# ZJU-DAILY/HC-SpMM

Measured on AMD Instinct MI355X. Metric: GNN-aggregation SpMM edges*dim/s (A*X, fp32), higher is better.
Workload: dtype f32

## Files before the change

### hc-spmm_amd/csrc/capi.hip

```cpp
#include <hip/hip_runtime.h>
#include <stdint.h>
#include <stdlib.h>

#include "fingerprint.h"
#include "hcspmm.h"
#include "spmm_kernels.h"

namespace {
thread_local int g_last_hip_error = 0;

int fail_hip(hipError_t e) {
  g_last_hip_error = (int)e;
  return HCSPMM_EHIP;
}

inline bool aligned(const void* p, size_t a) { return (reinterpret_cast<uintptr_t>(p) & (a - 1)) == 0; }

constexpr int kDtypeF8 = HCSPMM_DTYPE_BF16 + 1;

inline int elem_bytes(int dtype) { return dtype == HCSPMM_DTYPE_F32 ? 4 : dtype == kDtypeF8 ? 1 : 2; }

int pick_vec(int dtype, int D, int64_t ldx, int64_t ldz, const void* X, const void* Z, const void* ws) {
  if (dtype == HCSPMM_DTYPE_F32) return D >= 4 ? 4 : D >= 2 ? 2 : 1;
  const bool dword_rows = ((D | ldx | ldz) & 1) == 0 && aligned(X, 4) && aligned(Z, 4) && (!ws || aligned(ws, 4));
// ... 69 lines not shown
  }
  int n_wide = 0;
  return wide_choice(h, D, dtype, &n_wide);
}

extern "C" int32_t hcspmm_wide_threshold_fp8(const hcspmm_plan_header* h, int D) {
  if (D <= 0 || D % 4 != 0) return INT32_MAX;
  if (!h) return (D + nominal_vec(kDtypeF8, D) - 1) / nominal_vec(kDtypeF8, D) > 32 ? INT32_MAX : 64;
  int n_wide = 0;
  return wide_choice(h, D, kDtypeF8, &n_wide);
}

extern "C" int32_t hcspmm_wide_threshold(const hcspmm_plan_header* h, int D) {
  return hcspmm_wide_threshold_typed(h, D, HCSPMM_DTYPE_F32);
}

extern "C" int32_t hcspmm_own_tiny_launch(const hcspmm_plan_header* h, int fused) {
  return h && hcspmm::plan_own_tiny_launch(h->n_tiny, fused) ? 1 : 0;
}

extern "C" int hcspmm_abi_version(void) { return HCSPMM_ABI_VERSION; }

namespace {
__global__ __launch_bounds__(256) void fingerprint_kernel(const int32_t* __restrict__ rowptr, const int32_t* __restrict__ col,
                                                          long long N, long long E, unsigned long long* out) {
  const long long stride = (long long)gridDim.x * blockDim.x;
  const long long i0 = (long long)blockIdx.x * blockDim.x + threadIdx.x;
  unsigned long long acc = (i0 == 0) ? hcspmm::fp_seed(N, E) : 0ull;
  for (long long r = i0; r <= N; r += stride) acc += hcspmm::fp_term_rowptr((uint64_t)r, rowptr[r]);
  for (long long e = i0; e < E; e += stride) acc += hcspmm::fp_term_col((uint64_t)e, col[e]);
  for (int off = 32; off > 0; off >>= 1) acc += __shfl_xor(acc, off, 64);
  if ((threadIdx.x & 63) == 0) atomicAdd(out, acc);
}
}

namespace {
__global__ __launch_bounds__(256) void edge_to_row_kernel(const int32_t* __restrict__ rowptr, int N, long long E,
                                                          int32_t* __restrict__ e2r) {
  const long long stride = (long long)gridDim.x * blockDim.x;
  for (long long e = (long long)blockIdx.x * blockDim.x + threadIdx.x; e < E; e += stride) {
    int lo = 0, hi = N;
    while (hi - lo > 1) {
      const int mid = lo + ((hi - lo) >> 1);
      if ((long long)rowptr[mid] <= e) lo = mid;
      else hi = mid;
    }
    e2r[e] = lo;
  }
}
}

extern "C" int hcspmm_edge_to_row_device(const int32_t* rowptr, int64_t N, int64_t E, int32_t* e2r, void* stream_v) {
  if (N < 0 || E < 0 || !rowptr || (E > 0 && !e2r)) return HCSPMM_EINVAL;
  if (N > INT32_MAX - 16 || E > INT32_MAX) return HCSPMM_ERANGE;
  if (E == 0) return HCSPMM_OK;
  long long blocks = (E + 255) / 256;
  if (blocks > 65536) blocks = 65536;
  hipLaunchKernelGGL(edge_to_row_kernel, dim3((unsigned)blocks), dim3(256), 0, reinterpret_cast<hipStream_t>(stream_v), rowptr,
                     (int)N, (long long)E, e2r);
  const hipError_t e = hipGetLastError();
  return e == hipSuccess ? HCSPMM_OK : fail_hip(e);
}

extern "C" int hcspmm_graph_fingerprint_device(const int32_t* rowptr, const int32_t* col, int64_t N, int64_t E,
                                               uint64_t* out_d, void* stream_v) {
  if (!rowptr || !out_d || N < 0 || E < 0 || (E > 0 && !col)) return HCSPMM_EINVAL;
  if (N > INT32_MAX - 16 || E > INT32_MAX) return HCSPMM_ERANGE;
  hipStream_t stream = reinterpret_cast<hipStream_t>(stream_v);
  hipError_t e = hipMemsetAsync(out_d, 0, sizeof(uint64_t), stream);
  if (e != hipSuccess) return fail_hip(e);
  long long blocks = (N + 1 + E + 256 * 16 - 1) / (256 * 16);
  if (blocks < 1) blocks = 1;
  if (blocks > 4096) blocks = 4096;
  hipLaunchKernelGGL(fingerprint_kernel, dim3((unsigned)blocks), dim3(256), 0, stream, rowptr, col, (long long)N, (long long)E,
                     reinterpret_cast<unsigned long long*>(out_d));
  e = hipGetLastError();
  return e == hipSuccess ? HCSPMM_OK : fail_hip(e);
}
extern "C" int hcspmm_last_hip_error(void) { return g_last_hip_error; }

namespace {
struct FusedOperands {
  const float* W;
  long long ldr, ldc;
  float* out;
  int H;
  int mode;
};

void fill_plan_args(hcspmm::PlanArgs& a, const int32_t* plan_d, const hcspmm_plan_header* ph, int64_t N, int D, int dtype) {
  a = hcspmm::PlanArgs{};
  a.plan = plan_d;
  a.off_tasks = ph->off_tasks;
  a.n_tasks = ph->n_tasks;
  a.n_tiny = ph->n_tiny;
  a.off_slice_table = ph->off_slice_table;
  a.off_slice_tasks = ph->off_slice_tasks;
  a.n_slices = ph->n_slices;
  a.slice_xcd_tasks = ph->slice_xcd_tasks;
  a.off_dense_index = ph->off_dense_index;
  a.off_dense_pack = ph->off_dense_pack;
  a.n_dense = ph->n_dense;
  a.off_dense_compact = ph->off_dense_compact;
  a.n_dense_compact = ph->n_dense_compact;
  a.off_dense_compact2 = ph->off_dense_compact2;
  a.n_dense_compact2 = ph->n_dense_compact2;
  a.off_fixups = ph->off_fixups;
  a.n_split_rows = ph->n_split_rows;
  wide_choice(ph, D, dtype, &a.n_wide, &a.panel_cols);
  a.N = (int)N;
  a.D = D;
}

int forward_impl(const void* X, int64_t x_rows, int64_t ldx, void* Z, int64_t ldz, int dtype, const int32_t* rowptr,
                 const int32_t* col, const int32_t* blockPartition, const int32_t* edgeToColumn,
                 const int32_t* edgeToRow, const int32_t* hybrid_type, const int32_t* plan_d,
                 const hcspmm_plan_header* ph, int64_t N, int64_t E, int D, void* workspace,
                 size_t workspace_bytes, void* stream_v, const FusedOperands* fused, const float* values = nullptr,
                 int heads = 0, const int32_t* vindex = nullptr, int64_t num_values = 0) {
  if (dtype < HCSPMM_DTYPE_F32 || dtype > HCSPMM_DTYPE_BF16) return HCSPMM_EINVAL;
  if (N < 0 || E < 0 || D <= 0 || ldx < D || ldz < D) return HCSPMM_EINVAL;
  if (heads > 0 && (dtype != HCSPMM_DTYPE_F32 || !values || fused || D % heads != 0 ||
                    ((D / heads) % 4 != 0 && !(vindex && heads == 1))))
    return HCSPMM_EINVAL;
  if (N == 0) return HCSPMM_OK;
  if (!X || !Z || !rowptr || (E > 0 && !col)) return HCSPMM_EINVAL;
  if (N > INT32_MAX - 16 || E > INT32_MAX) return HCSPMM_ERANGE;
  hipStream_t stream = reinterpret_cast<hipStream_t>(stream_v);
  hipError_t e;
  if (plan_d && ph) {
    const int rc = hcspmm_plan_check(ph, N, E, 0);
    if (rc != HCSPMM_OK) return rc;
    if (x_rows < ph->num_columns) return HCSPMM_EINVAL;
    const size_t need = hcspmm_workspace_bytes(ph, D);
    if (need > 0 && (!workspace || workspace_bytes < need)) return HCSPMM_EWORKSPACE;
    hcspmm::PlanArgs a;
    fill_plan_args(a, plan_d, ph, N, D, dtype);
    a.X = X;
    a.Z = Z;
    a.ldx = (size_t)ldx;
    a.ldz = (size_t)ldz;
    a.partial = need ? reinterpret_cast<float*>(workspace) : nullptr;
    a.col = col;
    if (fused) {
      a.fused = fused->mode;
      a.H = fused->H;
      a.W = fused->W;
      a.w_ldr = fused->ldr;
      a.w_ldc = fused->ldc;
      a.out = fused->out;
    }
    const int vec = pick_vec(dtype, D, ldx, ldz, X, Z, need ? workspace : nullptr);
    if (fused && (vec != 4 || dtype != HCSPMM_DTYPE_F32)) return HCSPMM_EINVAL;
    if (fused && (fused->mode & 2)) {
      e = hcspmm::launch_fused_tiles(a, stream);
      if (e != hipSuccess) return fail_hip(e);
    }
    if (values) {
      if (fused) return HCSPMM_EINVAL;
      const hcspmm::WPlanArgs wa{a, values, rowptr, ph->segment_len};
      if (vindex) e = hcspmm::launch_plan_wi_f32(hcspmm::WHPlanArgs{wa, (long long)num_values, D / heads, vindex}, vec, stream);
      else if (heads > 0) e = hcspmm::launch_plan_wh_f32(hcspmm::WHPlanArgs{wa, (long long)E, D / heads, nullptr}, vec, stream);
      else e = dtype == HCSPMM_DTYPE_F32 ? hcspmm::launch_plan_w_f32(wa, vec, stream)
          : dtype == HCSPMM_DTYPE_F16 ? hcspmm::launch_plan_w_f16(wa, vec, stream)
                                      : hcspmm::launch_plan_w_bf16(wa, vec, stream);
    } else {
      e = dtype == HCSPMM_DTYPE_F32 ? hcspmm::launch_plan_f32(a, vec, stream)
          : dtype == HCSPMM_DTYPE_F16 ? hcspmm::launch_plan_f16(a, vec, stream)
                                      : hcspmm::launch_plan_bf16(a, vec, stream);
    }
  } else {
    if (fused) return HCSPMM_EINVAL;
    if (plan_d || ph) return HCSPMM_EINVAL;
    if (!blockPartition || !hybrid_type || (E > 0 && (!edgeToColumn || !edgeToRow))) return HCSPMM_EINVAL;
    hcspmm::WindowArgs a;
    a.X = X;
    a.Z = Z;
    a.ldx = (size_t)ldx;
    a.ldz = (size_t)ldz;
    a.rowptr = rowptr;
    a.col = col;
    a.blockPartition = blockPartition;
    a.edgeToColumn = edgeToColumn;
    a.edgeToRow = edgeToRow;
    a.hybrid_type = hybrid_type;
    a.N = (int)N;
    a.D = D;
    const int vec = pick_vec(dtype, D, ldx, ldz, X, Z, nullptr);
    if (values) {
      const hcspmm::WWindowArgs wa{a, values};
      if (vindex) e = hcspmm::launch_window_wi_f32(hcspmm::WHWindowArgs{wa, (long long)num_values, D / heads, vindex}, vec, stream);
      else if (heads > 0) e = hcspmm::launch_window_wh_f32(hcspmm::WHWindowArgs{wa, (long long)E, D / heads, nullptr}, vec, stream);
      else e = dtype == HCSPMM_DTYPE_F32 ? hcspmm::launch_window_w_f32(wa, vec, stream)
          : dtype == HCSPMM_DTYPE_F16 ? hcspmm::launch_window_w_f16(wa, vec, stream)
                                      : hcspmm::launch_window_w_bf16(wa, vec, stream);
    } else {
      e = dtype == HCSPMM_DTYPE_F32 ? hcspmm::launch_window_f32(a, vec, stream)
          : dtype == HCSPMM_DTYPE_F16 ? hcspmm::launch_window_f16(a, vec, stream)
                                      : hcspmm::launch_window_bf16(a, vec, stream);
    }
  }
  return e == hipSuccess ? HCSPMM_OK : fail_hip(e);
}
}

extern "C" int hcspmm_forward_typed(const void* X, int64_t x_rows, int64_t ldx, void* Z, int64_t ldz, int dtype, const int32_t* rowptr,
                                    const int32_t* col, const int32_t* blockPartition, const int32_t* edgeToColumn,
                                    const int32_t* edgeToRow, const int32_t* hybrid_type, const int32_t* plan_d,
                                    const hcspmm_plan_header* ph, int64_t N, int64_t E, int D, void* workspace,
                                    size_t workspace_bytes, void* stream_v) {
  return forward_impl(X, x_rows, ldx, Z, ldz, dtype, rowptr, col, blockPartition, edgeToColumn, edgeToRow, hybrid_type,
                      plan_d, ph, N, E, D, workspace, workspace_bytes, stream_v, nullptr);
}

extern "C" int hcspmm_forward_weighted(const void* X, int64_t x_rows, int64_t ldx, void* Z, int64_t ldz, int dtype,
                                       const int32_t* rowptr, const int32_t* col, const int32_t* blockPartition,
                                       const int32_t* edgeToColumn, const int32_t* edgeToRow, const int32_t* hybrid_type,
                                       const int32_t* plan_d, const hcspmm_plan_header* ph, int64_t N, int64_t E, int D,
                                       void* workspace, size_t workspace_bytes, void* stream_v, const float* values) {
  if (!values) return HCSPMM_EINVAL;
  return forward_impl(X, x_rows, ldx, Z, ldz, dtype, rowptr, col, blockPartition, edgeToColumn, edgeToRow, hybrid_type,
                      plan_d, ph, N, E, D, workspace, workspace_bytes, stream_v, nullptr, values);
}

extern "C" int hcspmm_forward_weighted_heads(const void* X, int64_t x_rows, int64_t ldx, void* Z, int64_t ldz, int dtype,
                                             const int32_t* rowptr, const int32_t* col, const int32_t* blockPartition,
                                             const int32_t* edgeToColumn, const int32_t* edgeToRow, const int32_t* hybrid_type,
                                             const int32_t* plan_d, const hcspmm_plan_header* ph, int64_t N, int64_t E, int D,
                                             void* workspace, size_t workspace_bytes, void* stream_v, const float* values,
                                             int heads) {
  if (!values || heads <= 0) return HCSPMM_EINVAL;
  if ((long long)E * heads > INT64_MAX / 4) return HCSPMM_ERANGE;
  return forward_impl(X, x_rows, ldx, Z, ldz, dtype, rowptr, col, blockPartition, edgeToColumn, edgeToRow, hybrid_type,
                      plan_d, ph, N, E, D, workspace, workspace_bytes, stream_v, nullptr, values, heads);
}

extern "C" int hcspmm_forward_weighted_indexed(const void* X, int64_t x_rows, int64_t ldx, void* Z, int64_t ldz, int dtype,
                                               const int32_t* rowptr, const int32_t* col, const int32_t* blockPartition,
                                               const int32_t* edgeToColumn, const int32_t* edgeToRow, const int32_t* hybrid_type,
                                               const int32_t* plan_d, const hcspmm_plan_header* ph, int64_t N, int64_t E, int D,
                                               void* workspace, size_t workspace_bytes, void* stream_v, const float* values,
                                               int heads, const int32_t* value_index, int64_t num_values) {
  if (!values || heads <= 0 || num_values < 0 || (E > 0 && (!value_index || num_values == 0))) return HCSPMM_EINVAL;
  if (num_values > INT32_MAX || num_values > INT64_MAX / 4 / heads) return HCSPMM_ERANGE;
  static const int32_t no_entries = 0;
  return forward_impl(X, x_rows, ldx, Z, ldz, dtype, rowptr, col, blockPartition, edgeToColumn, edgeToRow, hybrid_type, plan_d,
                      ph, N, E, D, workspace, workspace_bytes, stream_v, nullptr, values, heads,
                      value_index ? value_index : &no_entries, num_values);
}

extern "C" int hcspmm_quantize_fp8(const float* X, int64_t rows, int64_t ldx, int D, int format, const float* scale_in, void* Xq,
                                   int64_t ldq, float* scale_out, void* stream_v) {
  if (format != HCSPMM_FP8_E4M3) return HCSPMM_EINVAL;
  if (rows < 0 || D <= 0 || D % 4 != 0 || ldx < D || ldq < D || ldq % 4 != 0) return HCSPMM_EINVAL;
  if (rows == 0) return HCSPMM_OK;
  if (!X || !Xq || (!scale_out && !scale_in) || !aligned(Xq, 4)) return HCSPMM_EINVAL;
  const hipError_t e = hcspmm::launch_quantize_fp8(X, (long long)rows, (long long)ldx, D, scale_in, reinterpret_cast<unsigned char*>(Xq),
                                                   (long long)ldq, scale_out, reinterpret_cast<hipStream_t>(stream_v));
  return e == hipSuccess ? HCSPMM_OK : fail_hip(e);
}

extern "C" int hcspmm_forward_fp8(const void* Xq, int64_t x_rows, int64_t ldx, int format, const float* row_scale,
                                  const float* values, float* Z, int64_t ldz, const int32_t* rowptr, const int32_t* col,
                                  const int32_t* blockPartition, const int32_t* edgeToColumn, const int32_t* edgeToRow,
                                  const int32_t* hybrid_type, const int32_t* plan_d, const hcspmm_plan_header* ph, int64_t N,
                                  int64_t E, int D, void* workspace, size_t workspace_bytes, void* stream_v) {
  if (format != HCSPMM_FP8_E4M3) return HCSPMM_EINVAL;
  if (N < 0 || E < 0 || x_rows < 0 || D <= 0 || ldx < D || ldz < D) return HCSPMM_EINVAL;
  if (D % 4 != 0 || ldx % 4 != 0) return HCSPMM_EINVAL;
  if (N == 0) return HCSPMM_OK;
  if (!Xq || !Z || !rowptr || (E > 0 && !col) || !aligned(Xq, 4) || !aligned(Z, 4)) return HCSPMM_EINVAL;
  if (N > INT32_MAX - 16 || E > INT32_MAX) return HCSPMM_ERANGE;
  hipStream_t stream = reinterpret_cast<hipStream_t>(stream_v);
  const int vec = nominal_vec(kDtypeF8, D);
  const bool binary = !values && !row_scale;
  hipError_t e;
  if (plan_d && ph) {
    const int rc = hcspmm_plan_check(ph, N, E, 0);
    if (rc != HCSPMM_OK) return rc;
    if (x_rows < ph->num_columns) return HCSPMM_EINVAL;
    const size_t need = hcspmm_workspace_bytes(ph, D);
    if (need > 0 && (!workspace || workspace_bytes < need)) return HCSPMM_EWORKSPACE;
    if (need > 0 && !aligned(workspace, 4)) return HCSPMM_EINVAL;
    hcspmm::PlanArgs a;
    fill_plan_args(a, plan_d, ph, N, D, kDtypeF8);
    a.X = Xq;
    a.Z = Z;
    a.ldx = (size_t)ldx;
    a.ldz = (size_t)ldz;
    a.partial = need ? reinterpret_cast<float*>(workspace) : nullptr;
    a.col = col;
    if (binary) {
      e = hcspmm::launch_plan_f8(a, vec, stream);
    } else {
      a.row_scale = row_scale;
      e = hcspmm::launch_plan_w_f8(hcspmm::WPlanArgs{a, values, rowptr, ph->segment_len}, vec, stream);
    }
  } else {
    if (plan_d || ph) return HCSPMM_EINVAL;
    if (!blockPartition || !hybrid_type || (E > 0 && (!edgeToColumn || !edgeToRow))) return HCSPMM_EINVAL;
    hcspmm::WindowArgs a;
    a.X = Xq;
    a.Z = Z;
    a.ldx = (size_t)ldx;
    a.ldz = (size_t)ldz;
    a.rowptr = rowptr;
// ... 475 lines not shown
```

### hc-spmm_amd/csrc/plan_host.cpp

```cpp
#include <algorithm>
#include <atomic>
#include <chrono>
#include <condition_variable>
#include <cstdint>
#include <cstdio>
#include <cstdlib>
#include <cstring>
#include <mutex>
#include <thread>
#include <vector>

#include "fingerprint.h"
#include "hcspmm.h"
#include "host_util.h"

namespace {

constexpr int kSliceAuto = 0, kSliceOn = 1, kSliceOff = -1;
constexpr int32_t kSliceAutoThreshold = 256;
constexpr int64_t kSliceAutoMinColumns = 65536;
constexpr int64_t kSliceAutoAlwaysColumns = 250000;
constexpr int64_t kSliceAutoMinEntries = 3000000;
constexpr int kSliceSample = 4;
constexpr int kSlicePad = 64;

struct Resolved {
  int32_t split_threshold, segment_len, fuse_in_launch;
  int32_t slice_mode, slice_threshold, n_slices, panel_cols;
};

int env_int(const char* name, int dflt) {
  const char* e = std::getenv(name);
  return e && *e ? std::atoi(e) : dflt;
}

Resolved resolve(const hcspmm_plan_params* p) {
  Resolved r{512, 256, 0, kSliceAuto, kSliceAutoThreshold, 8, 0};
  if (p) {
    if (p->split_threshold > 0) r.split_threshold = p->split_threshold;
    if (p->segment_len > 0) r.segment_len = p->segment_len;
    r.fuse_in_launch = p->fuse_in_launch < 0 ? -1 : (p->fuse_in_launch > 2 ? 2 : p->fuse_in_launch);
  }
  if (r.segment_len > r.split_threshold) r.segment_len = r.split_threshold;
  int thr = p ? p->slice_threshold : 0, ns = p ? p->n_slices : 0;
  if (thr == 0) thr = env_int("HCSPMM_SLICE_THRESHOLD", 0);
  if (ns == 0) ns = env_int("HCSPMM_SLICES", 0);
  if (thr > 0) { r.slice_mode = kSliceOn; r.slice_threshold = thr; }
  else if (thr < 0) r.slice_mode = kSliceOff;
  if (ns > 0) r.n_slices = std::min(64, (ns + 7) / 8 * 8);
  if (p && p->panel_cols != 0) r.panel_cols = p->panel_cols < 0 ? -1 : std::min(1 << 20, (p->panel_cols + 15) / 16 * 16);
  return r;
}

inline int64_t pieces_bound(int64_t d, const Resolved& rp) {
  return std::min<int64_t>(d, rp.n_slices - 1 + (d + rp.segment_len - 1) / rp.segment_len);
}

inline void slice_cuts(const int32_t* col, int32_t e0, int64_t d, const int32_t* bounds, int S, int32_t* cuts) {
  const int32_t* first = col + e0;
  int64_t lo = 0;
  cuts[0] = 0;
  for (int s = 0; s < S; ++s) {
    const int64_t hi = (s == S - 1) ? d : std::lower_bound(first + lo, first + d, bounds[s]) - first;
    cuts[s + 1] = (int32_t)hi;
    lo = hi;
  }
}

template <typename F>
inline void for_each_piece(const int32_t* cuts, int32_t e0, int S, int32_t seg, F fn) {
  for (int s = 0; s < S; ++s)
    for (int64_t b = cuts[s]; b < cuts[s + 1]; b += seg) fn(s, (int32_t)(e0 + b), (int32_t)std::min<int64_t>(seg, cuts[s + 1] - b));
}

inline int64_t align4(int64_t x) { return (x + 3) & ~int64_t(3); }

struct Layout {
  int64_t n_tasks = 0, n_dense = 0, n_compact = 0, n_compact2 = 0, n_split_rows = 0, n_partials = 0;
  int64_t dense_pack_words = 0;
  int64_t nnz_sparse = 0, nnz_dense = 0, dense_k_sum = 0;
  int32_t max_dense_k = 0;
  int64_t n_sparse_windows = 0;
  int64_t n_slice_tasks = 0, n_sliced_rows = 0, nnz_sliced = 0;
  int64_t off_tasks = 0, off_dense_index = 0, off_dense_pack = 0, off_compact2 = 0, off_compact = 0, off_fixups = 0,
          off_sparse_windows = 0, off_slice_table = 0, off_slice_tasks = 0, total = 0;
};

class PassPool {
 public:
  explicit PassPool(int T) : T_(T) {
    for (int t = 1; t < T_; ++t) th_.emplace_back([this, t] { work(t); });
  }
  ~PassPool() {
    fn_ = nullptr;
    post();
    for (auto& x : th_) x.join();
  }
  int size() const { return T_; }
  template <typename F> void run(F& fn) {
    fn_ = [](void* f, int t) { (*static_cast<F*>(f))(t); };
    arg_ = &fn;
    done_.store(0, std::memory_order_relaxed);
    post();
    fn(0);
    for (int spin = 0; done_.load(std::memory_order_acquire) != T_ - 1; ++spin)
      if (spin > 256) std::this_thread::yield();
  }

 private:
  void post() {
    {
      std::lock_guard<std::mutex> lk(m_);
      gen_.fetch_add(1, std::memory_order_release);
    }
    cv_.notify_all();
  }
  void work(int t) {
    uint64_t seen = 0;
    for (;;) {
      for (int spin = 0; spin < 4000 && gen_.load(std::memory_order_acquire) == seen; ++spin) {
      }
      if (gen_.load(std::memory_order_acquire) == seen) {
        std::unique_lock<std::mutex> lk(m_);
        cv_.wait(lk, [&] { return gen_.load(std::memory_order_acquire) != seen; });
      }
      ++seen;
      if (!fn_) return;
      fn_(arg_, t);
      done_.fetch_add(1, std::memory_order_release);
    }
  }
  const int T_;
  std::vector<std::thread> th_;
  void (*fn_)(void*, int) = nullptr;
  void* arg_ = nullptr;
  std::atomic<uint64_t> gen_{0};
  std::atomic<int> done_{0};
  std::mutex m_;
  std::condition_variable cv_;
};
thread_local PassPool* tl_pool = nullptr;
struct PoolScope {
  PassPool pool;
  explicit PoolScope(int T) : pool(T) { tl_pool = T > 1 ? &pool : nullptr; }
  ~PoolScope() { tl_pool = nullptr; }
};

template <typename F> void parallel_for(int T, F fn) {
  if (T <= 1) { fn(0); return; }
  if (tl_pool && tl_pool->size() == T) { tl_pool->run(fn); return; }
  std::vector<std::thread> th;
  th.reserve((size_t)T);
  for (int t = 0; t < T; ++t) th.emplace_back(fn, t);
  for (auto& x : th) x.join();
}

int plan_threads(int64_t W) { return W < 4096 ? 1 : std::min(hcspmm::host_threads(), 16); }

int compute_layout(const int32_t* rowptr, int64_t N, const int32_t* bp, const int32_t* ht, const Resolved& rp,
                   bool slicing, Layout* out) {
  const int64_t W = (N + HCSPMM_BLK_H - 1) / HCSPMM_BLK_H;
  const int T = plan_threads(W);
  std::vector<Layout> part((size_t)T);
  std::vector<int> bad((size_t)T, 0);
  parallel_for(T, [&](int t) {
    Layout L;
    for (int64_t w = W * t / T; w < W * (t + 1) / T; ++w) {
      const int64_t r0 = w * HCSPMM_BLK_H, r1 = std::min<int64_t>(r0 + HCSPMM_BLK_H, N);
      const int64_t nnz = (int64_t)rowptr[r1] - rowptr[r0];
      if (ht[w] != 0 && nnz > 0) {
        if (bp[w] <= 0) { bad[(size_t)t] = 1; return; }
        L.n_dense++;
        const int64_t K = (int64_t)bp[w] * HCSPMM_BLK_W;
        if (K <= HCSPMM_COMPACT_K) L.n_compact++;
        else if (K <= HCSPMM_COMPACT2_K) L.n_compact2++;
        else L.dense_pack_words += K + (K / 4) * 2;
        L.nnz_dense += nnz;
        L.dense_k_sum += K;
        L.max_dense_k = std::max<int32_t>(L.max_dense_k, (int32_t)K);
      } else {
        L.n_sparse_windows++;
        for (int64_t r = r0; r < r1; ++r) {
          const int64_t d = (int64_t)rowptr[r + 1] - rowptr[r];
          if (slicing && d > rp.slice_threshold) {
            const int64_t pcs = pieces_bound(d, rp);
            L.n_slice_tasks += pcs;
            L.n_partials += pcs;
            L.n_split_rows++;
            L.n_sliced_rows++;
            L.nnz_sliced += d;
          } else if (d > rp.split_threshold) {
            const int64_t segs = (d + rp.segment_len - 1) / rp.segment_len;
            L.n_tasks += segs;
            L.n_partials += segs;
            L.n_split_rows++;
          } else {
            L.n_tasks++;
          }
        }
        L.nnz_sparse += nnz;
      }
    }
    part[(size_t)t] = L;
  });
  Layout L;
  for (int t = 0; t < T; ++t) {
    if (bad[(size_t)t]) return HCSPMM_EINVAL;
    const Layout& p = part[(size_t)t];
    L.n_tasks += p.n_tasks; L.n_dense += p.n_dense; L.n_compact += p.n_compact; L.n_compact2 += p.n_compact2;
    L.n_split_rows += p.n_split_rows; L.n_partials += p.n_partials; L.dense_pack_words += p.dense_pack_words;
    L.nnz_sparse += p.nnz_sparse; L.nnz_dense += p.nnz_dense; L.dense_k_sum += p.dense_k_sum;
    L.n_sparse_windows += p.n_sparse_windows;
    L.n_slice_tasks += p.n_slice_tasks; L.n_sliced_rows += p.n_sliced_rows; L.nnz_sliced += p.nnz_sliced;
    L.max_dense_k = std::max(L.max_dense_k, p.max_dense_k);
  }
  if (slicing) L.n_slice_tasks += (int64_t)kSlicePad * rp.n_slices;
  L.off_tasks = HCSPMM_PLAN_HEADER_WORDS;
  L.off_dense_index = align4(L.off_tasks + 4 * L.n_tasks);
  L.off_dense_pack = align4(L.off_dense_index + 4 * L.n_dense);
  L.off_compact2 = (L.off_dense_pack + L.dense_pack_words + 63) & ~int64_t(63);
  L.off_compact = L.off_compact2 + HCSPMM_COMPACT2_WORDS * L.n_compact2;
  L.off_fixups = align4(L.off_compact + HCSPMM_COMPACT_WORDS * L.n_compact);
  L.off_sparse_windows = align4(L.off_fixups + 4 * L.n_split_rows);
  L.off_slice_table = align4(L.off_sparse_windows + L.n_sparse_windows);
  L.off_slice_tasks = slicing ? align4(L.off_slice_table + rp.n_slices + 1) : L.off_slice_table;
  L.total = align4(L.off_slice_tasks + 4 * (slicing ? L.n_slice_tasks : 0));
  if (L.total > INT32_MAX) return HCSPMM_ERANGE;
  *out = L;
  return HCSPMM_OK;
}

}

extern "C" int hcspmm_plan_words(const int32_t* rowptr, int64_t N, int64_t E, const int32_t* bp, const int32_t* ht,
                                 const hcspmm_plan_params* params, int64_t* words_out) {
  if (!rowptr || !words_out || N < 0 || E < 0) return HCSPMM_EINVAL;
  if (N > 0 && (!bp || !ht)) return HCSPMM_EINVAL;
  const Resolved rp = resolve(params);
  PoolScope scope(plan_threads((N + HCSPMM_BLK_H - 1) / HCSPMM_BLK_H));
  Layout L, Ls;
  int rc = HCSPMM_OK;
  int64_t total = 0;
  if (rp.slice_mode != kSliceOn) {
    rc = compute_layout(rowptr, N, bp, ht, rp, false, &L);
    if (rc != HCSPMM_OK) return rc;
    total = L.total;
  }
  if (rp.slice_mode != kSliceOff) {
    rc = compute_layout(rowptr, N, bp, ht, rp, true, &Ls);
    if (rc != HCSPMM_OK) return rc;
    total = std::max(total, Ls.total);
  }
  *words_out = total;
  return HCSPMM_OK;
}

static inline int length_class(int32_t len) { return len <= 1 ? (len > 0 ? 1 : 0) : 33 - __builtin_clz((uint32_t)len - 1u); }

static int fingerprint_and_check(const int32_t* rowptr, const int32_t* col, int64_t N, int64_t E, int64_t M, uint64_t* out) {
  if (rowptr[0] != 0 || rowptr[N] != E) return HCSPMM_EINVAL;
  const int T = (N + E < (1 << 18)) ? 1 : plan_threads(1 << 20);
  std::vector<uint64_t> part((size_t)T, 0);
  std::vector<int> bad((size_t)T, 0);
  parallel_for(T, [&](int t) {
    uint64_t acc = 0;
    uint32_t over = 0;
    for (int64_t r = (N + 1) * t / T; r < (N + 1) * (t + 1) / T; ++r) acc += hcspmm::fp_term_rowptr((uint64_t)r, rowptr[r]);
    for (int64_t r = std::max<int64_t>(1, (N + 1) * t / T); r < (N + 1) * (t + 1) / T; ++r) over |= (uint32_t)(rowptr[r] < rowptr[r - 1]);
    for (int64_t e = E * t / T; e < E * (t + 1) / T; ++e) {
      acc += hcspmm::fp_term_col((uint64_t)e, col[e]);
      over |= (uint32_t)((uint32_t)col[e] >= (uint32_t)M);
    }
    part[(size_t)t] = acc;
    bad[(size_t)t] = over != 0;
  });
  uint64_t f = hcspmm::fp_seed(N, E);
  for (int t = 0; t < T; ++t) {
    if (bad[(size_t)t]) return HCSPMM_EINVAL;
    f += part[(size_t)t];
  }
  *out = f;
  return HCSPMM_OK;
}

extern "C" int hcspmm_graph_fingerprint_host(const int32_t* rowptr, const int32_t* col, int64_t N, int64_t E, uint64_t* out) {
  if (!rowptr || !out || N < 0 || E < 0 || (E > 0 && !col)) return HCSPMM_EINVAL;
  if (N > INT32_MAX - 16 || E > INT32_MAX) return HCSPMM_ERANGE;
  return fingerprint_and_check(rowptr, col, N, E, (int64_t)INT32_MAX + 1, out);
}

extern "C" int hcspmm_plan_build(const int32_t* rowptr, const int32_t* col, int64_t N, int64_t E, int64_t M,
                                 const int32_t* bp, const int32_t* e2c, const int32_t* ht,
                                 const hcspmm_plan_params* params, int32_t* plan, int64_t words) {
  if (!rowptr || !plan || N < 0 || E < 0) return HCSPMM_EINVAL;
  if (N > 0 && (!bp || !ht)) return HCSPMM_EINVAL;
  if (E > 0 && (!col || !e2c)) return HCSPMM_EINVAL;
  if (N > INT32_MAX - 16 || E > INT32_MAX) return HCSPMM_ERANGE;
  if (M <= 0) M = N;
  if (M > INT32_MAX) return HCSPMM_ERANGE;
  PoolScope scope(plan_threads((N + HCSPMM_BLK_H - 1) / HCSPMM_BLK_H));
  static const bool dbg = std::getenv("HCSPMM_PLAN_DEBUG") != nullptr;
  auto now = [] { return std::chrono::duration<double, std::milli>(std::chrono::steady_clock::now().time_since_epoch()).count(); };
  double tp[8] = {now(), 0, 0, 0, 0, 0, 0, 0};
  uint64_t fingerprint = 0;
  {
    const int frc = fingerprint_and_check(rowptr, col, N, E, M, &fingerprint);
    if (frc != HCSPMM_OK) return frc;
  }
  tp[1] = now();
  const Resolved rp = resolve(params);
  Layout L;
  int rc = HCSPMM_OK;
  bool slicing = rp.slice_mode == kSliceOn;
  if (rp.slice_mode != kSliceOff) {
    rc = compute_layout(rowptr, N, bp, ht, rp, true, &L);
    if (rc != HCSPMM_OK) return rc;
    if (rp.slice_mode == kSliceAuto)
      slicing = M >= kSliceAutoMinColumns && L.nnz_sliced * 20 >= L.nnz_sparse && L.nnz_sliced > 0 &&
                (M >= kSliceAutoAlwaysColumns || L.nnz_sparse >= kSliceAutoMinEntries);
    if (L.n_sliced_rows == 0) slicing = false;
  }
  if (!slicing) {
    rc = compute_layout(rowptr, N, bp, ht, rp, false, &L);
    if (rc != HCSPMM_OK) return rc;
  }
  if (words < L.total) return HCSPMM_EINVAL;
  const int64_t W = (N + HCSPMM_BLK_H - 1) / HCSPMM_BLK_H;
  const int S = slicing ? rp.n_slices : 0;
  tp[2] = now();

  const int T = plan_threads(W);
  std::vector<int64_t> cut((size_t)T + 1);
  for (int t = 0; t <= T; ++t) cut[(size_t)t] = W * t / T;
  {
    const int64_t z0 = L.off_dense_index, zn = L.total - z0;
    std::vector<int64_t> zc((size_t)T + 1);
    for (int t = 0; t <= T; ++t) zc[(size_t)t] = z0 + zn * t / T;
    parallel_for(T, [&](int t) {
      std::memset(plan + zc[(size_t)t], 0, sizeof(int32_t) * (size_t)(zc[(size_t)t + 1] - zc[(size_t)t]));
    });
  }

  std::vector<int32_t> bounds((size_t)std::max(S - 1, 0), 0);
  if (slicing) {
    int shift = 0;
    while (((M - 1) >> shift) >= 65536) ++shift;
    const int64_t nb = ((M - 1) >> shift) + 1;
    std::vector<std::vector<int64_t>> hist((size_t)T, std::vector<int64_t>((size_t)nb, 0));
    parallel_for(T, [&](int t) {
      int64_t* h = hist[(size_t)t].data();
      for (int64_t w = cut[(size_t)t]; w < cut[(size_t)t + 1]; ++w) {
        const int64_t r0 = w * HCSPMM_BLK_H, r1 = std::min<int64_t>(r0 + HCSPMM_BLK_H, N);
        if (ht[w] != 0 && rowptr[r1] > rowptr[r0]) continue;
        for (int64_t r = r0; r < r1; ++r) {
          if ((int64_t)rowptr[r + 1] - rowptr[r] <= rp.slice_threshold) continue;
          for (int64_t e = rowptr[r]; e < rowptr[r + 1]; e += kSliceSample) h[col[e] >> shift]++;
        }
      }
    });
    int64_t total = 0;
    for (int64_t b = 0; b < nb; ++b) {
      for (int t = 1; t < T; ++t) hist[0][(size_t)b] += hist[(size_t)t][(size_t)b];
      total += hist[0][(size_t)b];
    }
    int64_t run = 0, b = 0;
    for (int sidx = 0; sidx < S - 1; ++sidx) {
      const int64_t want = (total * (sidx + 1) + S - 1) / S;
      while (b < nb && run + hist[0][(size_t)b] <= want) run += hist[0][(size_t)b++];
      bounds[(size_t)sidx] = (int32_t)std::min<int64_t>(M, b << shift);
    }
  }

  tp[3] = now();
  const int n_cls = length_class(rp.split_threshold) + 1;
  struct Counts {
    std::vector<int64_t> cls;
    std::vector<int64_t> slice_cls;
    std::vector<int32_t> cuts;
    int64_t n_fix = 0, n_slots = 0, n_dense = 0, n_sparse_w = 0;
  };
  std::vector<Counts> cnt((size_t)T);
  auto walk = [&](int t, bool first_pass, auto&& on_task, auto&& on_fix, auto&& on_dense, auto&& on_sparse_window, auto&& on_piece) {
    std::vector<int32_t>& row_cuts = cnt[(size_t)t].cuts;
    if (first_pass) row_cuts.clear();
    size_t next_cuts = 0;
    for (int64_t w = cut[(size_t)t]; w < cut[(size_t)t + 1]; ++w) {
      const int64_t r0 = w * HCSPMM_BLK_H, r1 = std::min<int64_t>(r0 + HCSPMM_BLK_H, N);
      const int64_t nnz = (int64_t)rowptr[r1] - rowptr[r0];
      if (ht[w] != 0 && nnz > 0) {
        on_dense(w);
        continue;
      }
      on_sparse_window(w);
      for (int64_t r = r0; r < r1; ++r) {
        const int32_t e0 = rowptr[r];
        const int64_t d = (int64_t)rowptr[r + 1] - e0;
        if (slicing && d > rp.slice_threshold) {
          if (first_pass) {
            row_cuts.resize(next_cuts + (size_t)S + 1);
            slice_cuts(col, e0, d, bounds.data(), S, row_cuts.data() + next_cuts);
          }
          const int32_t* cuts = row_cuts.data() + next_cuts;
          next_cuts += (size_t)S + 1;
          int64_t pcs = 0, k = 0;
          for (int sl = 0; sl < S; ++sl) pcs += ((int64_t)cuts[sl + 1] - cuts[sl] + rp.segment_len - 1) / rp.segment_len;
          const int64_t slot0 = pcs > 1 ? on_fix(r, pcs) : -1;
          for_each_piece(cuts, e0, S, rp.segment_len, [&](int sl, int32_t first, int32_t len) {
            on_piece(sl, (int32_t)r, first, len, (int32_t)(pcs > 1 ? slot0 + k : -1));
            ++k;
          });
        } else if (d > rp.split_threshold) {
          const int64_t segs = (d + rp.segment_len - 1) / rp.segment_len;
          const int64_t slot0 = on_fix(r, segs);
          for (int64_t sgm = 0; sgm < segs; ++sgm) {
            const int64_t b = sgm * rp.segment_len;
            on_task((int32_t)r, (int32_t)(e0 + b), (int32_t)std::min<int64_t>(rp.segment_len, d - b), (int32_t)(slot0 + sgm));
          }
        } else {
          on_task((int32_t)r, e0, (int32_t)d, -1);
        }
      }
    }
  };
  parallel_for(T, [&](int t) {
    std::vector<int64_t> cls((size_t)n_cls, 0), slice_cls((size_t)S * (size_t)n_cls, 0);
    int64_t n_fix = 0, n_slots = 0, n_dense = 0, n_sparse_w = 0;
    walk(t, true, [&](int32_t, int32_t, int32_t len, int32_t) { cls[(size_t)length_class(len)]++; },
         [&](int64_t, int64_t segs) { n_fix++; n_slots += segs; return (int64_t)0; },
         [&](int64_t) { n_dense++; }, [&](int64_t) { n_sparse_w++; },
         [&](int sl, int32_t, int32_t, int32_t len, int32_t) { slice_cls[(size_t)sl * (size_t)n_cls + (size_t)length_class(len)]++; });
    Counts& c = cnt[(size_t)t];
    c.cls.swap(cls);
    c.slice_cls.swap(slice_cls);
    c.n_fix = n_fix;
    c.n_slots = n_slots;
    c.n_dense = n_dense;
    c.n_sparse_w = n_sparse_w;
  });
  std::vector<int64_t> start((size_t)n_cls + 1, 0);
  for (int c = 0; c < n_cls; ++c) {
    int64_t tot = 0;
    for (int t = 0; t < T; ++t) tot += cnt[(size_t)t].cls[(size_t)c];
    start[(size_t)(n_cls - 1 - c) + 1] = tot;
  }
  for (size_t i = 1; i < start.size(); ++i) start[i] += start[i - 1];
  int32_t len_gt[5] = {0, 0, 0, 0, 0};
  for (int b = 0; b < 5; ++b) {
    const int c = length_class((16 << b) + 1);
    len_gt[b] = c >= n_cls ? 0 : (int32_t)start[(size_t)(n_cls - c)];
  }
  int64_t n_tiny = 0;
  for (int c = 0; c <= length_class(HCSPMM_TINY_LEN) && c < n_cls; ++c)
    for (int t = 0; t < T; ++t) n_tiny += cnt[(size_t)t].cls[(size_t)c];
  std::vector<std::vector<int64_t>> pos((size_t)T, std::vector<int64_t>((size_t)n_cls));
  std::vector<int64_t> fix_at((size_t)T + 1, 0), slot_at((size_t)T + 1, 0), dense_at((size_t)T + 1, 0), sparse_w_at((size_t)T + 1, 0);
  {
    std::vector<int64_t> run(start.begin(), start.end() - 1);
    for (int t = 0; t < T; ++t) {
      for (int c = 0; c < n_cls; ++c) {
        pos[(size_t)t][(size_t)c] = run[(size_t)(n_cls - 1 - c)];
        run[(size_t)(n_cls - 1 - c)] += cnt[(size_t)t].cls[(size_t)c];
      }
      fix_at[(size_t)t + 1] = fix_at[(size_t)t] + cnt[(size_t)t].n_fix;
      slot_at[(size_t)t + 1] = slot_at[(size_t)t] + cnt[(size_t)t].n_slots;
      dense_at[(size_t)t + 1] = dense_at[(size_t)t] + cnt[(size_t)t].n_dense;
      sparse_w_at[(size_t)t + 1] = sparse_w_at[(size_t)t] + cnt[(size_t)t].n_sparse_w;
    }
  }
  if (slicing ? (fix_at[(size_t)T] > L.n_split_rows || slot_at[(size_t)T] > L.n_partials)
              : (fix_at[(size_t)T] != L.n_split_rows || slot_at[(size_t)T] != L.n_partials))
    return HCSPMM_EINVAL;
  if (dense_at[(size_t)T] != L.n_dense || start.back() != L.n_tasks || sparse_w_at[(size_t)T] != L.n_sparse_windows)
    return HCSPMM_EINVAL;
  std::vector<int64_t> table((size_t)S + 1, 0);
  std::vector<std::vector<int64_t>> spos((size_t)T, std::vector<int64_t>((size_t)S * (size_t)n_cls, 0));
  int64_t slice_xcd_tasks = 0;
  if (slicing) {
    int64_t xcd[8] = {0, 0, 0, 0, 0, 0, 0, 0};
    for (int sl = 0; sl < S; ++sl) {
      int64_t run = table[(size_t)sl];
      for (int c = n_cls - 1; c >= 0; --c)
        for (int t = 0; t < T; ++t) {
          spos[(size_t)t][(size_t)sl * (size_t)n_cls + (size_t)c] = run;
          run += cnt[(size_t)t].slice_cls[(size_t)sl * (size_t)n_cls + (size_t)c];
        }
      const int64_t padded = (run - table[(size_t)sl] + kSlicePad - 1) / kSlicePad * kSlicePad;
      int32_t* pad = plan + L.off_slice_tasks;
      for (int64_t q = run; q < table[(size_t)sl] + padded; ++q) {
        if (q >= L.n_slice_tasks) return HCSPMM_EINVAL;
        pad[4 * q + 0] = -1; pad[4 * q + 1] = 0; pad[4 * q + 2] = 0; pad[4 * q + 3] = -1;
      }
      table[(size_t)sl + 1] = table[(size_t)sl] + padded;
      xcd[sl & 7] += padded;
    }
    if (table[(size_t)S] > L.n_slice_tasks) return HCSPMM_EINVAL;
    for (int x = 0; x < 8; ++x) slice_xcd_tasks = std::max(slice_xcd_tasks, xcd[x]);
    for (int sl = 0; sl <= S; ++sl) plan[L.off_slice_table + sl] = (int32_t)table[(size_t)sl];
  }
  tp[4] = now();
  struct DenseRef { int32_t w, K; };
  std::vector<DenseRef> dense((size_t)L.n_dense);
  int32_t* out = plan + L.off_tasks;
  int32_t* fix = plan + L.off_fixups;
  int32_t* sparse_w = plan + L.off_sparse_windows;
  int32_t* sout = plan + L.off_slice_tasks;
  parallel_for(T, [&](int t) {
    std::vector<int64_t> p = pos[(size_t)t];
    std::vector<int64_t> sp = spos[(size_t)t];
    int64_t n_fix = fix_at[(size_t)t], slot = slot_at[(size_t)t], nd = dense_at[(size_t)t], nsw = sparse_w_at[(size_t)t];
    walk(t, false,
         [&](int32_t row, int32_t e0, int32_t len, int32_t slot_id) {
           const int64_t q = p[(size_t)length_class(len)]++;
           if (len <= HCSPMM_TINY_LEN) {
             out[4 * q + 0] = slot_id < 0 ? row : -(slot_id + 1);
             out[4 * q + 1] = len >= 1 ? col[e0] : -1;
             out[4 * q + 2] = len;
             out[4 * q + 3] = len >= 2 ? col[e0 + 1] : -1;
           } else {
             out[4 * q + 0] = row;
             out[4 * q + 1] = e0;
             out[4 * q + 2] = len;
             out[4 * q + 3] = slot_id;
           }
         },
         [&](int64_t r, int64_t segs) {
           fix[4 * n_fix + 0] = (int32_t)r;
           fix[4 * n_fix + 1] = (int32_t)slot;
           fix[4 * n_fix + 2] = (int32_t)segs;
           ++n_fix;
           const int64_t s0 = slot;
           slot += segs;
           return s0;
         },
         [&](int64_t w) { dense[(size_t)nd++] = DenseRef{(int32_t)w, bp[w] * HCSPMM_BLK_W}; },
         [&](int64_t w) { sparse_w[nsw++] = (int32_t)w; },
         [&](int sl, int32_t row, int32_t first, int32_t len, int32_t slot_id) {
           const int64_t q = sp[(size_t)sl * (size_t)n_cls + (size_t)length_class(len)]++;
           sout[4 * q + 0] = row;
           sout[4 * q + 1] = first;
           sout[4 * q + 2] = len;
           sout[4 * q + 3] = slot_id;
         });
  });

  tp[5] = now();
  std::stable_sort(dense.begin(), dense.end(), [](const DenseRef& a, const DenseRef& b) { return a.K > b.K; });
  int32_t* dindex = plan + L.off_dense_index;
  int32_t* dpack = plan + L.off_dense_pack;
  const int64_t n_reg = L.n_dense - L.n_compact - L.n_compact2, n_c2 = L.n_compact2;
  std::vector<int64_t> pack_at((size_t)n_reg + 1, 0);
  for (int64_t i = 0; i < n_reg; ++i) pack_at[(size_t)i + 1] = pack_at[(size_t)i] + dense[(size_t)i].K + (dense[(size_t)i].K / 4) * 2;
  std::vector<int64_t> uniq_part((size_t)T, 0);
  std::vector<int> bad((size_t)T, 0);
  parallel_for(T, [&](int t) {
    int64_t uniq_total = 0;
    for (int64_t i = L.n_dense * t / T; i < L.n_dense * (t + 1) / T; ++i) {
      const int64_t w = dense[(size_t)i].w;
      const int32_t K = dense[(size_t)i].K, K4 = K / 4;
      const int64_t r0 = w * HCSPMM_BLK_H, r1 = std::min<int64_t>(r0 + HCSPMM_BLK_H, N);
      const int kind = i < n_reg ? 0 : (i < n_reg + n_c2 ? 2 : 1);
      if (kind != (K <= HCSPMM_COMPACT_K ? 1 : (K <= HCSPMM_COMPACT2_K ? 2 : 0))) { bad[(size_t)t] = 1; return; }
      const int32_t kmax = kind == 1 ? HCSPMM_COMPACT_K : (kind == 2 ? HCSPMM_COMPACT2_K : K);
      const int64_t off = kind == 1 ? HCSPMM_COMPACT_WORDS * (i - n_reg - n_c2)
                                    : (kind == 2 ? HCSPMM_COMPACT2_WORDS * (i - n_reg) : pack_at[(size_t)i]);
      int32_t* rec = plan + (kind == 1 ? L.off_compact : L.off_compact2) + off;
      int32_t* U = kind ? rec + 2 : dpack + off;
      uint32_t* masks = reinterpret_cast<uint32_t*>(U + kmax);
      if (kind) {
        rec[0] = (int32_t)w;
        rec[1] = K4;
      }
      for (int32_t k = 0; k < kmax; ++k) U[k] = -1;
      for (int64_t r = r0; r < r1; ++r) {
        for (int64_t e = rowptr[r]; e < rowptr[r + 1]; ++e) {
          const int32_t c = e2c[e];
          if (c < 0 || c >= K) { bad[(size_t)t] = 1; return; }
          U[c] = col[e];
          const int lane = 16 * (c & 3) + (int)(r - r0);
          masks[(c >> 2) * 2 + (lane >> 5)] |= 1u << (lane & 31);
        }
      }
      for (int32_t k = 0; k < K; ++k) uniq_total += U[k] >= 0;
      dindex[4 * i + 0] = (int32_t)w;
      dindex[4 * i + 1] = (int32_t)off;
      dindex[4 * i + 2] = K4;
      dindex[4 * i + 3] = kind;
    }
    uniq_part[(size_t)t] = uniq_total;
  });
  int64_t uniq_total = 0;
  for (int t = 0; t < T; ++t) {
    if (bad[(size_t)t]) return HCSPMM_EINVAL;
    uniq_total += uniq_part[(size_t)t];
  }

  hcspmm_plan_header h;
  std::memset(&h, 0, sizeof(h));
  h.magic = HCSPMM_PLAN_MAGIC;
  h.version = HCSPMM_PLAN_VERSION;
  h.total_words = (int32_t)L.total;
  h.num_nodes = (int32_t)N;
  h.num_edges = (int32_t)E;
  h.num_windows = (int32_t)W;
  h.split_threshold = rp.split_threshold;
  h.segment_len = rp.segment_len;
  h.n_tasks = (int32_t)L.n_tasks;
  h.n_dense = (int32_t)L.n_dense;
  h.n_split_rows = (int32_t)fix_at[(size_t)T];
  h.n_partials = (int32_t)slot_at[(size_t)T];
  h.off_tasks = (int32_t)L.off_tasks;
  h.off_dense_index = (int32_t)L.off_dense_index;
  h.off_dense_pack = (int32_t)L.off_dense_pack;
  h.off_fixups = (int32_t)L.off_fixups;
  h.nnz_sparse = (int32_t)L.nnz_sparse;
  h.nnz_dense = (int32_t)L.nnz_dense;
  h.uniq_dense = (int32_t)uniq_total;
  h.max_dense_k = L.max_dense_k;
  for (int b = 0; b < 5; ++b) h.n_len_gt[b] = len_gt[b];
  h.n_tiny = (int32_t)n_tiny;
  h.n_dense_compact = (int32_t)L.n_compact;
  h.off_dense_compact = (int32_t)L.off_compact;
  h.n_dense_compact2 = (int32_t)L.n_compact2;
  h.off_dense_compact2 = (int32_t)L.off_compact2;
  h.num_columns = (int32_t)M;
  h.n_sparse_windows = (int32_t)L.n_sparse_windows;
  h.off_sparse_windows = (int32_t)L.off_sparse_windows;
  h.fingerprint_lo = (uint32_t)(fingerprint & 0xffffffffull);
  h.fingerprint_hi = (uint32_t)(fingerprint >> 32);
  h.dense_k_sum = (int32_t)std::min<int64_t>(L.dense_k_sum, INT32_MAX);
  h.flags = rp.fuse_in_launch < 0 ? HCSPMM_PLAN_FUSE_NEVER : (rp.fuse_in_launch >= 2 ? HCSPMM_PLAN_FUSE_ROWS : (rp.fuse_in_launch == 1 ? HCSPMM_PLAN_FUSE_IN_LAUNCH : 0));
  h.n_slices = S;
  h.slice_threshold = slicing ? rp.slice_threshold : 0;
  h.off_slice_table = (int32_t)L.off_slice_table;
  h.off_slice_tasks = (int32_t)L.off_slice_tasks;
  h.n_slice_tasks = slicing ? (int32_t)table[(size_t)S] : 0;
  h.slice_xcd_tasks = (int32_t)slice_xcd_tasks;
  h.nnz_sliced = slicing ? (int32_t)L.nnz_sliced : 0;
  h.n_sliced_rows = slicing ? (int32_t)L.n_sliced_rows : 0;
  h.panel_cols = rp.panel_cols;
  static_assert(sizeof(hcspmm_plan_header) == HCSPMM_PLAN_HEADER_WORDS * 4, "header size");
  std::memcpy(plan, &h, sizeof(h));
  if (dbg) {
    tp[6] = now();
    std::fprintf(stderr, "plan_build: T=%d: fingerprint + range check %.2f | layout %.2f | clear + slice boundaries %.2f | task pass 1 (count) %.2f | "
                         "task pass 2 (write) %.2f | dense packs %.2f | total %.2f ms\n",
                 T, tp[1] - tp[0], tp[2] - tp[1], tp[3] - tp[2], tp[4] - tp[3], tp[5] - tp[4], tp[6] - tp[5], tp[6] - tp[0]);
  }
  return HCSPMM_OK;
}

extern "C" int hcspmm_plan_check(const hcspmm_plan_header* h, int64_t N, int64_t E, int64_t words_available) {
  if (!h) return HCSPMM_EINVAL;
  if (h->magic != HCSPMM_PLAN_MAGIC || h->version != HCSPMM_PLAN_VERSION) return HCSPMM_EPLAN;
  if (h->num_nodes != N || h->num_edges != E) return HCSPMM_EPLAN;
  if (h->num_windows != (N + HCSPMM_BLK_H - 1) / HCSPMM_BLK_H) return HCSPMM_EPLAN;
  if (h->num_columns < 0 || (h->num_columns == 0 && N > 0)) return HCSPMM_EPLAN;
  if (h->n_tasks < 0 || h->n_dense < 0 || h->n_split_rows < 0 || h->n_partials < 0) return HCSPMM_EPLAN;
  if (h->n_tiny < 0 || h->n_tiny > h->n_tasks) return HCSPMM_EPLAN;
  if (h->n_dense_compact < 0 || h->n_dense_compact2 < 0 ||
      (int64_t)h->n_dense_compact + h->n_dense_compact2 > h->n_dense)
    return HCSPMM_EPLAN;
  if (h->n_sparse_windows < 0 || (int64_t)h->n_sparse_windows + h->n_dense != h->num_windows) return HCSPMM_EPLAN;
  if (h->n_partials < 2 * (int64_t)h->n_split_rows || h->split_threshold <= 0 || h->segment_len <= 0) return HCSPMM_EPLAN;
  for (int b = 0; b < 5; ++b) {
    if (h->n_len_gt[b] < 0 || h->n_len_gt[b] > h->n_tasks - h->n_tiny) return HCSPMM_EPLAN;
    if (b > 0 && h->n_len_gt[b] > h->n_len_gt[b - 1]) return HCSPMM_EPLAN;
  }
  const int64_t n_reg = (int64_t)h->n_dense - h->n_dense_compact - h->n_dense_compact2;
  if (h->off_tasks != HCSPMM_PLAN_HEADER_WORDS) return HCSPMM_EPLAN;
  if (h->off_dense_index < h->off_tasks + 4 * (int64_t)h->n_tasks || (h->off_dense_index & 3)) return HCSPMM_EPLAN;
  if (h->off_dense_pack < h->off_dense_index + 4 * (int64_t)h->n_dense || (h->off_dense_pack & 3)) return HCSPMM_EPLAN;
  if (h->off_dense_compact2 < h->off_dense_pack + 132 * n_reg || (h->off_dense_compact2 & 63)) return HCSPMM_EPLAN;
  if (h->off_dense_compact != h->off_dense_compact2 + (int64_t)HCSPMM_COMPACT2_WORDS * h->n_dense_compact2) return HCSPMM_EPLAN;
  if (h->off_fixups < h->off_dense_compact + (int64_t)HCSPMM_COMPACT_WORDS * h->n_dense_compact || (h->off_fixups & 3))
    return HCSPMM_EPLAN;
  if (h->off_sparse_windows < h->off_fixups + 4 * (int64_t)h->n_split_rows || (h->off_sparse_windows & 3)) return HCSPMM_EPLAN;
  if (h->total_words < h->off_sparse_windows + (int64_t)h->n_sparse_windows) return HCSPMM_EPLAN;
  if (h->n_slices < 0 || h->n_slices > 64 || (h->n_slices & 7) || h->n_slice_tasks < 0 || h->slice_xcd_tasks < 0) return HCSPMM_EPLAN;
  if (h->n_slices > 0) {
    if (h->slice_threshold <= 0 || (h->n_slice_tasks % 64) || (h->slice_xcd_tasks % 64) || h->slice_xcd_tasks > h->n_slice_tasks)
      return HCSPMM_EPLAN;
    if (h->off_slice_table < h->off_sparse_windows + (int64_t)h->n_sparse_windows || (h->off_slice_table & 3)) return HCSPMM_EPLAN;
    if (h->off_slice_tasks < h->off_slice_table + (int64_t)h->n_slices + 1 || (h->off_slice_tasks & 3)) return HCSPMM_EPLAN;
    if (h->total_words < h->off_slice_tasks + 4 * (int64_t)h->n_slice_tasks) return HCSPMM_EPLAN;
    if (h->nnz_sliced < 0 || h->nnz_sliced > h->nnz_sparse) return HCSPMM_EPLAN;
  } else if (h->n_slice_tasks != 0 || h->slice_xcd_tasks != 0) {
    return HCSPMM_EPLAN;
  }
  if (words_available > 0 && h->total_words > words_available) return HCSPMM_EPLAN;
  if ((int64_t)h->nnz_sparse + h->nnz_dense != E) return HCSPMM_EPLAN;
  return HCSPMM_OK;
}

extern "C" size_t hcspmm_workspace_bytes(const hcspmm_plan_header* h, int D) {
  if (!h || D <= 0) return 0;
  return (size_t)h->n_partials * (size_t)D * sizeof(float);
}
```

### hc-spmm_amd/csrc/spmm_impl.h

```cpp
#pragma once
#include <hip/hip_runtime.h>
#include <stdint.h>
#include <stdlib.h>

#include "hcspmm.h"
#include "spmm_kernels.h"
#include "plan_layout.h"

namespace hcspmm {

struct F32 { typedef float T; typedef float Z; };
struct F16 { typedef unsigned short T; typedef unsigned short Z; };
struct BF16 { typedef unsigned short T; typedef unsigned short Z; };
struct F8 { typedef unsigned char T; typedef float Z; };

typedef float f32x4 __attribute__((ext_vector_type(4)));
typedef unsigned int u32x4 __attribute__((ext_vector_type(4)));
typedef unsigned int u32x2 __attribute__((ext_vector_type(2)));

template <int VEC> struct AccT { typedef float type __attribute__((ext_vector_type(VEC))); };
template <> struct AccT<1> { typedef float type; };
__device__ __forceinline__ float aget(const float& v, int) { return v; }
__device__ __forceinline__ void aset(float& v, int, float x) { v = x; }
template <typename V> __device__ __forceinline__ float aget(const V& v, int i) { return v[i]; }
template <typename V> __device__ __forceinline__ void aset(V& v, int i, float x) { v[i] = x; }
template <int VEC> __device__ __forceinline__ typename AccT<VEC>::type azero() {
  typename AccT<VEC>::type z;
#pragma unroll
  for (int q = 0; q < VEC; ++q) aset(z, q, 0.f);
  return z;
}

template <typename E, int VEC> struct RawT { typedef typename AccT<VEC>::type type; };
template <> struct RawT<F16, 8> { typedef u32x4 type; };
template <> struct RawT<F16, 4> { typedef u32x2 type; };
template <> struct RawT<F16, 2> { typedef unsigned int type; };
template <> struct RawT<F16, 1> { typedef unsigned short type; };
template <> struct RawT<BF16, 8> { typedef u32x4 type; };
template <> struct RawT<BF16, 4> { typedef u32x2 type; };
template <> struct RawT<BF16, 2> { typedef unsigned int type; };
template <> struct RawT<BF16, 1> { typedef unsigned short type; };
template <> struct RawT<F8, 8> { typedef u32x2 type; };
template <> struct RawT<F8, 4> { typedef unsigned int type; };
template <> struct RawT<F8, 2> { typedef unsigned short type; };
template <> struct RawT<F8, 1> { typedef unsigned char type; };

template <typename E> __device__ __forceinline__ float widen(unsigned short h);
template <> __device__ __forceinline__ float widen<F16>(unsigned short h) { return (float)__builtin_bit_cast(_Float16, h); }
template <> __device__ __forceinline__ float widen<BF16>(unsigned short h) { return __uint_as_float((unsigned)h << 16); }
template <typename E> __device__ __forceinline__ unsigned short narrow(float f);
template <> __device__ __forceinline__ unsigned short narrow<F16>(float f) { return __builtin_bit_cast(unsigned short, (_Float16)f); }
template <> __device__ __forceinline__ unsigned short narrow<BF16>(float f) {
  unsigned u = __float_as_uint(f);
  if ((u & 0x7fffffffu) > 0x7f800000u) return (unsigned short)((u >> 16) | 0x40u);
  u += 0x7fffu + ((u >> 16) & 1u);
  return (unsigned short)(u >> 16);
}

__device__ __forceinline__ unsigned rword(const u32x4& v, int i) { return v[i]; }
__device__ __forceinline__ unsigned rword(const u32x2& v, int i) { return v[i]; }
__device__ __forceinline__ unsigned rword(const unsigned& v, int) { return v; }
__device__ __forceinline__ unsigned rword(const unsigned short& v, int) { return v; }
__device__ __forceinline__ unsigned rword(const unsigned char& v, int) { return v; }
__device__ __forceinline__ float widen_f8(unsigned w, int q) {
  typedef float f32x2 __attribute__((ext_vector_type(2)));
  const f32x2 lo = __builtin_amdgcn_cvt_pk_f32_fp8((int)w, false), hi = __builtin_amdgcn_cvt_pk_f32_fp8((int)w, true);
  return (q & 2) ? hi[q & 1] : lo[q & 1];
}
__device__ __forceinline__ void rset(u32x4& v, int i, unsigned w) { v[i] = w; }
__device__ __forceinline__ void rset(u32x2& v, int i, unsigned w) { v[i] = w; }
__device__ __forceinline__ void rset(unsigned& v, int, unsigned w) { v = w; }

template <int VEC> struct MemF32 { typedef float type __attribute__((ext_vector_type(VEC), aligned(4))); };
template <> struct MemF32<1> { typedef float type; };

template <int WORDS> struct MemU32 { typedef unsigned int type __attribute__((ext_vector_type(WORDS), aligned(4))); };
template <> struct MemU32<1> { typedef unsigned int type; };


template <int VEC> __device__ __forceinline__ int lane_col(int c, int cend) { return VEC == 1 ? c : min(c, cend - VEC); }

template <typename E, int VEC> struct Lane {
  typedef typename E::T T;
  typedef typename E::Z ZT;
  typedef typename RawT<E, VEC>::type raw_t;
  typedef typename AccT<VEC>::type acc_t;
  static __device__ __forceinline__ raw_t zero() {
    raw_t z;
    __builtin_memset(&z, 0, sizeof(z));
    return z;
  }
  static __device__ __forceinline__ raw_t load(const T* p) {
    if constexpr (sizeof(T) == 4) return *reinterpret_cast<const typename MemF32<VEC>::type*>(p);
    else if constexpr (sizeof(T) == 1 && VEC >= 4) return *reinterpret_cast<const typename MemU32<VEC / 4>::type*>(p);
    else if constexpr (sizeof(T) == 1) return *reinterpret_cast<const raw_t*>(p);
    else if constexpr (VEC >= 2) return *reinterpret_cast<const typename MemU32<VEC / 2>::type*>(p);
    else return *reinterpret_cast<const raw_t*>(p);
  }
  static __device__ __forceinline__ acc_t load_partial(const float* p) { return *reinterpret_cast<const typename MemF32<VEC>::type*>(p); }
  static __device__ __forceinline__ float elem(const raw_t& v, int q) {
    if constexpr (sizeof(T) == 4) return aget(v, q);
    else if constexpr (sizeof(T) == 1) return widen_f8(rword(v, q >> 2), q & 3);
    else if constexpr (VEC == 1) return widen<E>(v);
    else {
      const unsigned w = rword(v, q >> 1);
      return widen<E>((unsigned short)((q & 1) ? (w >> 16) : (w & 0xffffu)));
    }
  }
  static __device__ __forceinline__ void add(acc_t& acc, const raw_t& v) {
    if constexpr (sizeof(T) == 4) acc += v;
    else {
#pragma unroll
      for (int q = 0; q < VEC; ++q) aset(acc, q, aget(acc, q) + elem(v, q));
    }
  }
  static __device__ __forceinline__ raw_t pack(const acc_t& acc) {
    if constexpr (sizeof(T) == 4) return acc;
    else if constexpr (VEC == 1) return narrow<E>(acc);
    else {
      raw_t r;
#pragma unroll
      for (int w = 0; w < VEC / 2; ++w)
        rset(r, w, (unsigned)narrow<E>(aget(acc, 2 * w)) | ((unsigned)narrow<E>(aget(acc, 2 * w + 1)) << 16));
      return r;
    }
  }
  static __device__ __forceinline__ void store(ZT* p, const acc_t& acc) {
    if constexpr (sizeof(T) == 1) store_partial(p, acc);
    else if constexpr (sizeof(T) == 4) __builtin_nontemporal_store(pack(acc), reinterpret_cast<typename MemF32<VEC>::type*>(p));
    else if constexpr (VEC >= 2) __builtin_nontemporal_store(pack(acc), reinterpret_cast<typename MemU32<VEC / 2>::type*>(p));
    else __builtin_nontemporal_store(pack(acc), reinterpret_cast<raw_t*>(p));
  }
  static __device__ __forceinline__ void store_partial(float* p, const acc_t& acc) {
    __builtin_nontemporal_store(acc, reinterpret_cast<typename MemF32<VEC>::type*>(p));
  }
};

#define HCSPMM_CONST_AS __attribute__((address_space(4)))
typedef const HCSPMM_CONST_AS int* cint_p;
typedef const HCSPMM_CONST_AS unsigned long long* cu64_p;

#ifndef HCSPMM_SPARSE_U
#define HCSPMM_SPARSE_U 8
#endif
#ifndef HCSPMM_DENSE_B
#define HCSPMM_DENSE_B 8
#endif
#ifndef HCSPMM_TINY_PER_WAVE
#define HCSPMM_TINY_PER_WAVE 8
#endif
template <int L> struct TinyT {
  static constexpr int per_group = HCSPMM_TINY_PER_WAVE / (64 / L);
  static constexpr int value = per_group < 2 ? 2 : (per_group > 4 ? 4 : per_group);
};
#ifndef HCSPMM_MIN_WAVES_H16
#define HCSPMM_MIN_WAVES_H16 4
// ... 554 lines not shown
  const int lane = threadIdx.x & 63;
  const int fi = (int)blockIdx.x * kWaves + (threadIdx.x >> 6);
  if (fi >= a.n_split_rows) return;
  const int4 f = reinterpret_cast<const int4*>(a.plan + a.off_fixups)[fi];
  const int row = f.x, s0 = f.y, ns = f.z;
  const int slots = (a.D + VEC - 1) / VEC;
  int L = 1;
  while (L < slots && L < 64) L <<= 1;
  const int R = 64 / L, g = lane / L, sl = lane & (L - 1);
  for (int c0 = 0; c0 < a.D; c0 += L * VEC) {
    const bool cok = c0 + sl * VEC < a.D;
    const int c = cok ? lane_col<VEC>(c0 + sl * VEC, a.D) : 0;
    const float* p = a.partial + (size_t)s0 * (size_t)a.D + c;
    acc_t acc = azero<VEC>();
    int s = g;
    for (; s + 7 * R < ns; s += 8 * R) {
      acc_t v[8];
#pragma unroll
      for (int u = 0; u < 8; ++u) v[u] = Lane<F32, VEC>::load_partial(p + (size_t)(s + u * R) * (size_t)a.D);
#pragma unroll
      for (int u = 0; u < 8; ++u) acc += v[u];
    }
    for (; s < ns; s += R) acc += Lane<F32, VEC>::load_partial(p + (size_t)s * (size_t)a.D);
    for (int off = L; off < 64; off <<= 1) {
#pragma unroll
      for (int q = 0; q < VEC; ++q) aset(acc, q, aget(acc, q) + __shfl_xor(aget(acc, q), off, 64));
    }
    if (cok && g == 0) Ln::store(Z + (size_t)row * a.ldz + c, acc);
  }
}

constexpr int kChunkK = 512;
constexpr int kPlanFreeWide = 64;

template <typename E, int L, int VEC>
__global__ __launch_bounds__(kThreads) void hybrid_window_kernel(WindowArgs a) {
  typedef Lane<E, VEC> Ln;
  typedef typename E::T elem_t;
  const elem_t* X = reinterpret_cast<const elem_t*>(a.X);
  typename E::Z* Z = reinterpret_cast<typename E::Z*>(a.Z);
  __shared__ int s_U[kChunkK];
  __shared__ unsigned int s_mask[kChunkK / 4 * 2];
  const int lane = threadIdx.x & 63;
  const int wave = __builtin_amdgcn_readfirstlane(threadIdx.x >> 6);
  const int nthreads = (int)blockDim.x, nwaves = nthreads >> 6;
  const int w = blockIdx.x;
  const int r0 = w * 16, r1 = min(r0 + 16, a.N);
  if (a.hybrid_type[w] == 0) {
    constexpr int R = 64 / L;
    const int G = R * nwaves;
    const int gi = wave * R + lane / L;
    for (int rb = r0; rb < r1; rb += G) {
      const int r = rb + gi;
      int e0 = 0, n = 0;
      typename E::Z* dst = nullptr;
      if (r < r1) {
        e0 = a.rowptr[r];
        n = a.rowptr[r + 1] - e0;
        dst = Z + (size_t)r * a.ldz;
        if (R > 1 && n > kPlanFreeWide) {
          n = 0;
          dst = nullptr;
        }
      }
      sparse_task<E, L, VEC, false>(X, dst, nullptr, a.col, e0, n, a.ldx, 0, a.D, lane);
    }
    if (R > 1) {
      int k = 0;
      for (int r = r0; r < r1; ++r) {
        const int e0 = a.rowptr[r];
        const int n = a.rowptr[r + 1] - e0;
        if (n > kPlanFreeWide) {
          if (k % nwaves == wave)
            sparse_task<E, L, VEC, true>(X, Z + (size_t)r * a.ldz, nullptr, a.col, e0, n, a.ldx, 0, a.D, lane);
          ++k;
        }
      }
    }
    return;
  }
  const int lo = a.rowptr[r0], hi = a.rowptr[r1];
  const int K = a.blockPartition[w] * 8;
  const int n_panels = (a.D + 16 * VEC - 1) / (16 * VEC);
  const int kq = lane >> 4, j = lane & 15;
  for (int pb = 0; pb < n_panels; pb += nwaves) {
    const int panel = pb + wave;
    const bool cok = panel < n_panels && panel * 16 * VEC + j * VEC < a.D;
    const int c = cok ? lane_col<VEC>(panel * 16 * VEC + j * VEC, a.D) : 0;
    f32x4 acc[VEC];
#pragma unroll
    for (int q = 0; q < VEC; ++q) acc[q] = f32x4{0.f, 0.f, 0.f, 0.f};
    for (int k0 = 0; k0 < K; k0 += kChunkK) {
      const int kc = min(kChunkK, K - k0);
      __syncthreads();
      for (int i = threadIdx.x; i < kChunkK; i += nthreads) s_U[i] = -1;
      for (int i = threadIdx.x; i < kChunkK / 2; i += nthreads) s_mask[i] = 0u;
      __syncthreads();
      for (int e = lo + (int)threadIdx.x; e < hi; e += nthreads) {
        const int cc = a.edgeToColumn[e] - k0;
        if (cc >= 0 && cc < kc) {
          const int rl = a.edgeToRow[e] - r0;
          const int bit = 16 * (cc & 3) + rl;
          atomicOr(&s_mask[(cc >> 2) * 2 + (bit >> 5)], 1u << (bit & 31));
          s_U[cc] = a.col[e];
        }
      }
      __syncthreads();
      const int steps = (kc + 3) / 4;
      for (int t0 = 0; t0 < steps; t0 += 4) {
        typename Ln::raw_t x[4];
        float av[4];
#pragma unroll
        for (int u = 0; u < 4; ++u) {
          const int t = t0 + u;
          const bool tv = t < steps;
          const int idx = tv ? s_U[min(4 * t + kq, kChunkK - 1)] : -1;
          const unsigned int mw = tv ? s_mask[t * 2 + (lane >> 5)] : 0u;
          av[u] = ((mw >> (lane & 31)) & 1u) ? 1.0f : 0.0f;
          x[u] = Ln::zero();
          if (cok && idx >= 0) x[u] = Ln::load(X + (size_t)idx * a.ldx + c);
        }
#pragma unroll
        for (int u = 0; u < 4; ++u) {
#pragma unroll
          for (int q = 0; q < VEC; ++q)
            acc[q] = __builtin_amdgcn_mfma_f32_16x16x4f32(av[u], Ln::elem(x[u], q), acc[q], 0, 0, 0);
        }
      }
    }
    if (cok) dense_store<E, VEC>(Z, acc, w, kq, c, a.N, a.ldz);
  }
}

template <typename E, int L, int VEC>
static hipError_t launch_plan_LV(const PlanArgs& a, hipStream_t stream) {
  PlanArgs b = a;
  const bool dense_fused = (a.fused & 1) != 0;
  const int n_col_panels =
      plan_launch_layout(b, L, VEC, DenseV<VEC>::mid, TinyT<L>::value, own_tiny_launch(a.n_tiny, a.fused), a.fused);
  constexpr bool kCanFuse = sizeof(typename E::T) == 4 && VEC == 4;
  constexpr int kMinWaves = sizeof(typename E::T) == 4 ? HCSPMM_MIN_WAVES_PER_SIMD : HCSPMM_MIN_WAVES_H16;
  if (dense_fused && !kCanFuse) return hipErrorInvalidValue;
  const long long dense_units = (long long)b.n_dense * (dense_fused ? 1 : b.n_panels);
  long long dense_wgs = (dense_units + kWaves - 1) / kWaves;
  if (dense_fused) {
    static const long long cap = [] {
      const char* e = getenv("HCSPMM_FUSED_DENSE_WGS");
      const long long v = e ? atoll(e) : 0;
      return v > 0 ? v : 2048LL;
    }();
    if (dense_wgs > cap) dense_wgs = cap;
  }
  b.fused_dense_wgs = (int)dense_wgs;
  const long long grid = (long long)b.sparse_wgs + dense_wgs;
  if (grid > 0x7fffffffLL) return hipErrorInvalidValue;
  if (grid > 0) {
    if constexpr (kCanFuse) {
      if (dense_fused) {
        const size_t lds = (size_t)b.n_panels * 16 * b.dense_vec * fused_row_stride(a.H, b.dense_vec) * sizeof(float);
        hipLaunchKernelGGL((hybrid_plan_kernel<E, L, VEC, HCSPMM_SPARSE_U, HCSPMM_FUSED_MIN_WAVES, true>),
                           dim3((unsigned)grid), dim3(kThreads), lds, stream, b);
      } else {
        hipLaunchKernelGGL((hybrid_plan_kernel<E, L, VEC, HCSPMM_SPARSE_U, kMinWaves>), dim3((unsigned)grid),
                           dim3(kThreads), 0, stream, b);
      }
    } else {
      hipLaunchKernelGGL((hybrid_plan_kernel<E, L, VEC, HCSPMM_SPARSE_U, kMinWaves>), dim3((unsigned)grid),
                         dim3(kThreads), 0, stream, b);
    }
  }
  hipError_t e = hipGetLastError();
  if (e != hipSuccess) return e;
  if (b.tiny_kernel_wgs > 0) {
    hipLaunchKernelGGL((tiny_kernel<E, L, VEC>), dim3((unsigned)(b.tiny_kernel_wgs * n_col_panels)), dim3(kThreads), 0, stream, b);
    e = hipGetLastError();
    if (e != hipSuccess) return e;
  }
  if (a.n_split_rows > 0) {
    const int fg = (a.n_split_rows + kWaves - 1) / kWaves;
    hipLaunchKernelGGL((fixup_kernel<E, VEC>), dim3(fg), dim3(kThreads), 0, stream, b);
    e = hipGetLastError();
  }
  return e;
}

template <typename E, int L, int VEC>
static hipError_t launch_window_LV(const WindowArgs& a, hipStream_t stream) {
  const int W = (a.N + 15) / 16;
  const int n_panels = (a.D + 16 * VEC - 1) / (16 * VEC);
  int waves = (16 * L + 63) / 64;
  if (n_panels > waves) waves = n_panels;
  if (waves > kWaves) waves = kWaves;
  if (W > 0) hipLaunchKernelGGL((hybrid_window_kernel<E, L, VEC>), dim3(W), dim3(waves * 64), 0, stream, a);
  return hipGetLastError();
}

static inline int pick_L(int D, int VEC) {
  const int slots = (D + VEC - 1) / VEC;
  int L = 4;
  while (L < slots && L < 64) L <<= 1;
  return L;
}

#define HCSPMM_DISPATCH_L(FN, E, VEC, WIDTH, ARGS, STREAM)  \
  switch (pick_L((WIDTH), VEC)) {                           \
    case 4:  return FN<E, 4, VEC>(ARGS, STREAM);            \
    case 8:  return FN<E, 8, VEC>(ARGS, STREAM);            \
    case 16: return FN<E, 16, VEC>(ARGS, STREAM);           \
    case 32: return FN<E, 32, VEC>(ARGS, STREAM);           \
    default: return FN<E, 64, VEC>(ARGS, STREAM);           \
  }

}
```

### hc-spmm_amd/csrc/spmm_kernels.h

```cpp
#pragma once
#include <hip/hip_runtime.h>
#include <stdint.h>

namespace hcspmm {

struct PlanArgs {
  const void* X;
  void* Z;
  float* partial;
  const int* col;
  const int* plan;
  size_t ldx, ldz;
  int off_tasks, n_tasks;
  int off_dense_index, off_dense_pack, n_dense;
  int off_dense_compact, n_dense_compact;
  int off_dense_compact2, n_dense_compact2;
  int off_fixups, n_split_rows;
  int N, D;
  int n_wide;
  int n_tiny;
  int panel_cols;
  int sparse_wgs_pp, dense_vec;
  int wide_wgs, sparse_wgs, n_panels;
  int tiny_wgs;
  int tiny_kernel_wgs;
  int off_slice_table, off_slice_tasks, n_slices, slice_xcd_tasks;
  int slice_wgs;
  int free_wgs_pp;
  int fused, H;
  int fused_dense_wgs;
  union {
    const float* W;
    const float* row_scale;
  };
  long long w_ldr, w_ldc;
  float* out;
};

struct TilesArgs {
  PlanArgs p;
  int n_ord_tiles, n_tiny_tiles;
  int chunk, tile_stride;
};

struct WindowArgs {
  const void* X;
  void* Z;
  const int* rowptr;
  const int* col;
  const int* blockPartition;
  const int* edgeToColumn;
  const int* edgeToRow;
  const int* hybrid_type;
  size_t ldx, ldz;
  int N, D;
};

struct WPlanArgs {
  PlanArgs p;
  const float* values;
  const int* rowptr;
  int segment_len;
};
struct WWindowArgs {
  WindowArgs w;
  const float* values;
  const float* row_scale;
};

hipError_t launch_plan_f32(const PlanArgs& a, int vec, hipStream_t stream);
bool plan_own_tiny_launch(int n_tiny, int fused);
hipError_t launch_window_f32(const WindowArgs& a, int vec, hipStream_t stream);
hipError_t launch_plan_f16(const PlanArgs& a, int vec, hipStream_t stream);
hipError_t launch_window_f16(const WindowArgs& a, int vec, hipStream_t stream);
hipError_t launch_plan_bf16(const PlanArgs& a, int vec, hipStream_t stream);
hipError_t launch_window_bf16(const WindowArgs& a, int vec, hipStream_t stream);
hipError_t launch_plan_w_f32(const WPlanArgs& a, int vec, hipStream_t stream);
hipError_t launch_window_w_f32(const WWindowArgs& a, int vec, hipStream_t stream);
hipError_t launch_plan_w_f16(const WPlanArgs& a, int vec, hipStream_t stream);
hipError_t launch_window_w_f16(const WWindowArgs& a, int vec, hipStream_t stream);
hipError_t launch_plan_w_bf16(const WPlanArgs& a, int vec, hipStream_t stream);
hipError_t launch_window_w_bf16(const WWindowArgs& a, int vec, hipStream_t stream);
hipError_t launch_plan_f8(const PlanArgs& a, int vec, hipStream_t stream);
hipError_t launch_window_f8(const WindowArgs& a, int vec, hipStream_t stream);
hipError_t launch_plan_w_f8(const WPlanArgs& a, int vec, hipStream_t stream);
hipError_t launch_window_w_f8(const WWindowArgs& a, int vec, hipStream_t stream);
hipError_t launch_quantize_fp8(const float* X, long long rows, long long ldx, int D, const float* scale_in, unsigned char* Xq,
                               long long ldq, float* scale_out, hipStream_t stream);
struct WHPlanArgs {
  WPlanArgs w;
  long long E;
  int dh;
  const int* vindex;
};
struct WHWindowArgs {
  WWindowArgs w;
  long long E;
  int dh;
  const int* vindex;
};
hipError_t launch_plan_wh_f32(const WHPlanArgs& a, int vec, hipStream_t stream);
hipError_t launch_window_wh_f32(const WHWindowArgs& a, int vec, hipStream_t stream);
hipError_t launch_plan_wi_f32(const WHPlanArgs& a, int vec, hipStream_t stream);
hipError_t launch_window_wi_f32(const WHWindowArgs& a, int vec, hipStream_t stream);
hipError_t launch_edge_norm(const int* rowptr, const int* col, int N, long long E, int kind, float* values, hipStream_t stream);

bool weight_grad_supported(int D, int H);
int weight_grad_groups(long long N);
hipError_t launch_weight_grad(const float* A, long long lda, const float* B, long long ldb, float* out, float* partial,
                              long long N, int D, int H, hipStream_t stream);

hipError_t launch_dense_update(const float* in, const float* W, long long ldr, long long ldc, float* out, int N,
                               int D, int H, const int* tile_list, int n_tiles, hipStream_t stream);
bool fused_tiles_supported(int D, int H);
hipError_t launch_fused_tiles(const PlanArgs& a, hipStream_t stream);
hipError_t launch_dense_update_leftover(const float* in, const float* W, long long ldr, long long ldc, float* out, int N,
                                        int D, int H, const int* plan, int off_tasks, int n_wide, int off_fixups,
                                        int n_split_rows, int off_slice_tasks, int n_slice_tasks, hipStream_t stream);
bool dense_update_streams(const float* in, const float* out, int D, int H);

struct SddmmArgs {
  const void* A;
  const void* B;
  size_t lda, ldb;
  const int* rowptr;
  const int* col;
  float* out;
  int N, D;
  long long E;
};
hipError_t launch_sddmm_f32(const SddmmArgs& a, int vec, hipStream_t stream);
hipError_t launch_sddmm_f16(const SddmmArgs& a, int vec, hipStream_t stream);
hipError_t launch_sddmm_bf16(const SddmmArgs& a, int vec, hipStream_t stream);
hipError_t launch_sddmm_heads_f32(const SddmmArgs& a, int heads, int vec, hipStream_t stream);
struct SoftmaxArgs {
  const float* x;
  const float* y;
  float* out;
  const int* rowptr;
  int N, heads;
  long long E;
};
hipError_t launch_edge_softmax(const SoftmaxArgs& a, bool backward, hipStream_t stream);

struct GatArgs {
  const float* s_dst;
  const float* s_src;
  const float* alpha;
  const float* grad_alpha;
  const int* rowptr;
  const int* col;
  const int* perm;
  float* out;
  float* grad_s_dst;
  float* grad_s_src;
  float slope;
  int N, heads;
  long long E;
  const int* rowptr_t;
  int n_t;
};
hipError_t launch_gat_attention(const GatArgs& a, hipStream_t stream);
hipError_t launch_gat_attention_backward(const GatArgs& a, hipStream_t stream);

struct Gatv2Args {
  const float* H_dst;
  const float* H_src;
  const float* att;
  const float* g;
  const int* rowptr;
  const int* col;
  const int* perm;
  float* out;
  float* grad_dst;
  float* grad_src;
  float* grad_att;
  float* partial;
  size_t ld_dst, ld_src, ld_gdst, ld_gsrc;
  float slope;
  int N, D, heads;
  long long E;
  const int* rowptr_t;
  const int* col_t;
  int n_t;
};
long long gatv2_grad_blocks(long long N, int D);
hipError_t launch_gatv2_scores(const Gatv2Args& a, hipStream_t stream);
hipError_t launch_gatv2_backward(const Gatv2Args& a, hipStream_t stream);

struct XArgs {
  PlanArgs p;
  const int* rowptr;
  int segment_len;
  unsigned flip;
  int* arg;
  int* ppos;
  const int* garg;
  const int* perm;
  size_t ldarg;
};
hipError_t launch_extremum_f32(const XArgs& a, int vec, hipStream_t stream);
hipError_t launch_extremum_backward_f32(const XArgs& a, int vec, hipStream_t stream);

struct EdgeMsgArgs {
  PlanArgs p;
  const int* rowptr;
  int segment_len;
  int op;
  const float* F;
  size_t ldf;
  const int* findex;
};
hipError_t launch_edge_messages_f32(const EdgeMsgArgs& a, int vec, hipStream_t stream);
struct EdgeMsgGradArgs {
  const float* gZ;
  const float* X;
  const float* F;
  float* gF;
  size_t ldg, ldx, ldf, ldgf;
  const int* rowptr;
  const int* col;
  int N, D, op;
  long long E;
// ... 6 lines not shown
```

### hc-spmm_amd/hcspmm/__init__.py

```python
import collections
import ctypes
import os
import threading
import weakref

import torch

from .capi import (EPLAN, Header, PlanParams, RULE_AS_SHIPPED, RULE_INTENDED, RULE_INTENDED_GUARD, RULE_MI355X,
                   RULE_MI355X_WIDE, check, lib)

__all__ = [
    "preprocess", "forward", "forward_more", "forward_fixed32", "forward_fixed64", "forward_fixed32_fused",
    "forward_fixed64_fused", "forward_final_fused", "forward_final_fused_64", "forward_GIN_final_fused", "backward",
    "backward_fixed32", "backward_fixed32_fused", "backward_final_fused", "backward_fixed64",
    "backward_fixed64_fused", "backward_final_fused_64", "backward_GIN_final_fused", "loi_reorder",
    "apply_permutation", "weight_grad", "update", "plan_header", "forward_rect", "forward_into", "sddmm", "edge_softmax", "edge_softmax_backward",
    "gat_attention", "gat_attention_backward", "forward_weighted_heads", "sddmm_heads",
    "gatv2_scores", "gatv2_scores_backward",
    "transpose_graph", "forward_weighted_indexed", "gat_attention_backward_directed", "gatv2_scores_backward_directed",
    "forward_max", "forward_min", "forward_extremum_backward",
    "forward_edge_messages", "edge_messages_grad", "EDGE_OPS",
    "quantize_fp8", "forward_fp8", "forward_weighted_fp8", "wide_threshold_fp8",
    "wide_threshold", "workspace_bytes", "fused_in_launch", "own_tiny_launch", "build_plan", "set_default_rule", "default_rule", "RULE_INTENDED", "RULE_INTENDED_GUARD",
    "RULE_AS_SHIPPED", "RULE_MI355X", "RULE_MI355X_WIDE", "mi355x_rule", "tune_plan",
# ... 50 lines not shown
    return e


def _entry(row_nzr, num_nodes=None, num_edges=None):
    if row_nzr is None or row_nzr.numel() < Header.WORDS or row_nzr.dtype != torch.int32:
        return None
    key = row_nzr.data_ptr()
    with _REG_LOCK:
        e = _REG.get(key)
        if e is not None:
            if e.ref() is not None:
                _REG.move_to_end(key)
                return e
            del _REG[key]
    host = row_nzr[:Header.WORDS].cpu().contiguous()
    h = Header.from_buffer_copy(host.numpy().tobytes())
    if h.magic != Header.MAGIC:
        return None
    if num_nodes is not None and check(lib().hcspmm_plan_check(ctypes.byref(h), num_nodes, num_edges, row_nzr.numel()),
                                       soft=True) != 0:
        return None
    return _register(row_nzr, h)


def plan_header(row_nzr, num_nodes=None, num_edges=None):
    e = _entry(row_nzr, num_nodes, num_edges)
    return e.header if e is not None else None


def _verify_graph(e, row_pointers, column_index):
    key = (row_pointers.data_ptr(), column_index.data_ptr())
    hit = e.graphs.get(key)
    if hit is not None and hit[0]() is not None and hit[1]() is not None:
        return
    L = lib()
    out = torch.empty(1, dtype=torch.int64, device=row_pointers.device)
    stream = torch.cuda.current_stream(row_pointers.device)
    with torch.cuda.device(row_pointers.device):
        check(L.hcspmm_graph_fingerprint_device(_ptr(row_pointers), _ptr(column_index), row_pointers.numel() - 1,
                                                column_index.numel(), _ptr(out), ctypes.c_void_p(stream.cuda_stream)))
    got = int(out.item()) & 0xFFFFFFFFFFFFFFFF
    if got != e.header.fingerprint:
        raise RuntimeError("hcspmm: plan does not match this graph (row_pointers / column_index differ from the ones "
                           "the plan was built from) [code %d]" % EPLAN)
    while len(e.graphs) >= _GRAPHS_MAX:
        e.graphs.popitem(last=False)
    e.graphs[key] = (weakref.ref(row_pointers), weakref.ref(column_index))


def wide_threshold(row_nzr, embedding_dim, dtype=torch.float32):
    h = plan_header(row_nzr)
    return int(lib().hcspmm_wide_threshold_typed(ctypes.byref(h) if h is not None else None, int(embedding_dim),
                                                 _DTYPES[dtype]))


def wide_threshold_fp8(row_nzr, embedding_dim):
    h = plan_header(row_nzr)
    return int(lib().hcspmm_wide_threshold_fp8(ctypes.byref(h) if h is not None else None, int(embedding_dim)))


def workspace_bytes(row_nzr, embedding_dim):
    h = plan_header(row_nzr)
    return int(lib().hcspmm_workspace_bytes(ctypes.byref(h), int(embedding_dim))) if h is not None else 0


def fused_in_launch(row_nzr, embedding_dim, hidden_dim):
    h = plan_header(row_nzr)
    return int(lib().hcspmm_fused_in_launch(ctypes.byref(h), int(embedding_dim), int(hidden_dim))) if h is not None else 0


def own_tiny_launch(row_nzr, fused=False):
    h = plan_header(row_nzr)
    return bool(lib().hcspmm_own_tiny_launch(ctypes.byref(h), int(bool(fused)))) if h is not None else False


def _ptr(t):
    return ctypes.c_void_p(t.data_ptr() if t is not None and t.numel() > 0 else 0)


class _on_device:
    __slots__ = ("ctx",)

    def __init__(self, device):
        self.ctx = None if device.index is None or device.index == torch.cuda.current_device() else torch.cuda.device(device)

    def __enter__(self):
        if self.ctx is not None:
            self.ctx.__enter__()

    def __exit__(self, *a):
        if self.ctx is not None:
            self.ctx.__exit__(*a)


def _i32_host(t):
    t = t.detach()
    if t.is_cuda and t.dtype == torch.int32 and t.is_contiguous() and t.numel() > (1 << 16):
        host = torch.empty(t.shape, dtype=torch.int32, pin_memory=True)
        host.copy_(t, non_blocking=True)
        torch.cuda.current_stream(t.device).synchronize()
        return host
    return t.to(device="cpu", dtype=torch.int32).contiguous()


def preprocess(column_index, row_pointers, num_nodes, num_edges, num_row_windows, rule=None, dim=None, num_columns=None):
    L = lib()
    dev = column_index.device
    col_h = _i32_host(column_index)
    rp_h = _i32_host(row_pointers)
    N = int(rp_h.numel()) - 1
    E = int(col_h.numel())
    if int(num_nodes) != N:
        raise RuntimeError("preprocess: num_nodes (%d) != row_pointers.size(0)-1 (%d)" % (num_nodes, N))
    W = (N + 15) // 16
    if int(num_row_windows) != W:
        raise RuntimeError("preprocess: num_row_windows (%d) != ceil(N/16) (%d)" % (num_row_windows, W))
    on_gpu = dev.type == "cuda"
    bp = torch.empty(W, dtype=torch.int32, pin_memory=on_gpu)
    ht = torch.empty(W, dtype=torch.int32, pin_memory=on_gpu)
    e2c = torch.empty(E, dtype=torch.int32, pin_memory=on_gpu)
    e2r = None
    if on_gpu:
        e2r = torch.empty(E, dtype=torch.int32, device=dev)
        rp_dev = row_pointers.to(device=dev, dtype=torch.int32).contiguous()
        with torch.cuda.device(dev):
            check(L.hcspmm_edge_to_row_device(_ptr(rp_dev), N, E, _ptr(e2r),
                                              ctypes.c_void_p(torch.cuda.current_stream(dev).cuda_stream)))
    e2r_h = None if on_gpu else torch.empty(E, dtype=torch.int32)
    if rule == "mi355x":
        if dim is None:
            raise RuntimeError('preprocess: rule="mi355x" needs dim= (the embedding width)')
        rule = mi355x_rule(dim)
    r = _DEFAULT_RULE if rule is None else int(rule)
    M = N if num_columns is None else int(num_columns)
    check(L.hcspmm_preprocess_host(_ptr(rp_h), _ptr(col_h), N, E, M, r, 0, _ptr(bp), _ptr(e2c), _ptr(e2r_h), _ptr(ht)))
    if not on_gpu:
        e2r = e2r_h
    up = [t.to(dev, non_blocking=True) for t in (bp, e2c, e2r, ht)]
    words = ctypes.c_int64(0)
    check(L.hcspmm_plan_words(_ptr(rp_h), N, E, _ptr(bp), _ptr(ht), ctypes.byref(_PLAN_PARAMS), ctypes.byref(words)))
    plan = torch.empty(max(int(words.value), Header.WORDS), dtype=torch.int32, pin_memory=on_gpu)
    check(L.hcspmm_plan_build(_ptr(rp_h), _ptr(col_h), N, E, M, _ptr(bp), _ptr(e2c), _ptr(ht),
                              ctypes.byref(_PLAN_PARAMS), _ptr(plan), plan.numel()))
    h = Header.from_buffer_copy(plan[:Header.WORDS].numpy().tobytes())
    plan = plan[:h.total_words]
    outs = up + [plan.to(dev, non_blocking=True)]
    _register(outs[4], h, row_pointers, column_index)
    col_nzr = torch.zeros(1, dtype=torch.int32, device=dev)
    return [outs[0], outs[1], outs[2], outs[3], outs[4], col_nzr]


def build_plan(row_pointers, column_index, blockPartition, edgeToColumn, hybrid_type, device=None,
               split_threshold=0, segment_len=0, num_columns=None, fuse_in_launch=False, slice_threshold=0, n_slices=0,
               panel_cols=0):
    L = lib()
    rp_h, col_h = _i32_host(row_pointers), _i32_host(column_index)
    bp_h, e2c_h, ht_h = _i32_host(blockPartition), _i32_host(edgeToColumn), _i32_host(hybrid_type)
    N, E = rp_h.numel() - 1, col_h.numel()
    params = PlanParams(int(split_threshold), int(segment_len), int(fuse_in_launch), int(slice_threshold), int(n_slices),
                        int(panel_cols)) \
        if (split_threshold or segment_len or fuse_in_launch or slice_threshold or n_slices or panel_cols) else _PLAN_PARAMS
    words = ctypes.c_int64(0)
    check(L.hcspmm_plan_words(_ptr(rp_h), N, E, _ptr(bp_h), _ptr(ht_h), ctypes.byref(params), ctypes.byref(words)))
    plan = torch.empty(max(int(words.value), Header.WORDS), dtype=torch.int32)
    check(L.hcspmm_plan_build(_ptr(rp_h), _ptr(col_h), N, E, N if num_columns is None else int(num_columns), _ptr(bp_h),
                              _ptr(e2c_h), _ptr(ht_h), ctypes.byref(params), _ptr(plan), plan.numel()))
    h = Header.from_buffer_copy(plan[:Header.WORDS].numpy().tobytes())
    plan = plan[:h.total_words]
    dev = torch.device(device) if device is not None else row_pointers.device
    plan_d = plan.to(dev)
    _register(plan_d, h, row_pointers, column_index)
    return plan_d


def tune_plan(row_pointers, column_index, blockPartition, edgeToColumn, edgeToRow, hybrid_type, embedding_dim,
              dtype=torch.float32, num_columns=None, candidates=None, steps=20, fuse_in_launch=False):
    dev = row_pointers.device
    if not row_pointers.is_cuda:
        raise RuntimeError("tune_plan measures on the GPU: graph tensors must be CUDA tensors")
    D = int(embedding_dim)
    N = row_pointers.size(0) - 1
    M = N if num_columns is None else int(num_columns)
    if candidates is None:
        panels = [0, 32, 64, -1] if D >= 64 else [0]
        candidates = [dict(slice_threshold=s, panel_cols=p) for s in (0, -1, 256) for p in panels]
    X = torch.randn(M, D, device=dev).to(dtype)
    Z = torch.empty(N, D, dtype=dtype, device=dev)
    col_nzr = torch.zeros(1, dtype=torch.int32, device=dev)
    report, best, seen = [], None, set()
    for kw in candidates:
        plan = build_plan(row_pointers, column_index, blockPartition, edgeToColumn, hybrid_type, num_columns=M,
                          fuse_in_launch=fuse_in_launch, **kw)
        h = plan_header(plan)
        key = (h.n_slices, h.slice_threshold, h.panel_cols, h.n_slice_tasks)
        if key in seen:
            continue
        seen.add(key)
        ws = torch.empty(max(workspace_bytes(plan, D) // 4, 1), dtype=torch.float32, device=dev)
        a = (row_pointers, column_index, blockPartition, edgeToColumn, edgeToRow, hybrid_type, plan, col_nzr)
        for _ in range(3):
            forward_into(X, Z, *a, workspace=ws)
        s, e = torch.cuda.Event(enable_timing=True), torch.cuda.Event(enable_timing=True)
        s.record()
        for _ in range(steps):
            forward_into(X, Z, *a, workspace=ws)
        e.record()
        e.synchronize()
        ms = s.elapsed_time(e) / steps
        report.append(dict(kw, ms=ms, n_slices=h.n_slices))
        if best is None or ms < best[0]:
            best = (ms, plan)
    return best[1], sorted(report, key=lambda r: r["ms"])


def _check_input(t, name):
    if not t.is_cuda:
        raise RuntimeError("%s must be a CUDA tensor" % name)
    if not t.is_contiguous():
        raise RuntimeError("%s must be contiguous" % name)


_DTYPES = {torch.float32: 0, torch.float16: 1, torch.bfloat16: 2}


def _graph_args(X, row_pointers, column_index, blockPartition, edgeToColumn, edgeToRow, hybrid_type, row_nzr,
                rect=False, dtypes=(torch.float32,)):
    for t, n in ((X, "input"), (row_pointers, "nodePointer"), (column_index, "edgeList"),
                 (blockPartition, "blockPartition"), (edgeToColumn, "edgeToColumn"), (edgeToRow, "edgeToRow")):
        _check_input(t, n)
    if X.dtype not in dtypes or X.dim() != 2:
        raise RuntimeError("input must be a 2-D %s tensor" % " / ".join(str(d).replace("torch.", "") for d in dtypes))
    N = row_pointers.size(0) - 1
    E = column_index.size(0)
    D = X.size(1)
    if X.size(0) != N and not rect:
        raise RuntimeError("input has %d rows but the graph has %d nodes" % (X.size(0), N))
    h = _checked_header(row_nzr, row_pointers, column_index, N, E, X.size(0))
    return N, E, D, h


def _checked_header(row_nzr, row_pointers, column_index, N, E, x_rows):
    e = _entry(row_nzr, N, E) if (row_nzr is not None and row_nzr.is_cuda) else None
    if e is None:
        return None
    if e.checked != (N, E, row_nzr.numel()):
        check(lib().hcspmm_plan_check(ctypes.byref(e.header), N, E, row_nzr.numel()))
        e.checked = (N, E, row_nzr.numel())
    if x_rows < e.header.num_columns:
        raise RuntimeError("input has %d rows but the plan gathers from %d" % (x_rows, e.header.num_columns))
    _verify_graph(e, row_pointers, column_index)
    return e.header


def _spmm(X, row_pointers, column_index, blockPartition, edgeToColumn, edgeToRow, hybrid_type, row_nzr, col_nzr,
          Z=None, rect=False):
    L = lib()
    N, E, D, h = _graph_args(X, row_pointers, column_index, blockPartition, edgeToColumn, edgeToRow, hybrid_type,
                             row_nzr, rect, dtypes=tuple(_DTYPES))
    if Z is None:
        Z = torch.empty((N, D), dtype=X.dtype, device=X.device)
    ws, ws_bytes = None, 0
    if h is not None:
        ws_bytes = int(L.hcspmm_workspace_bytes(ctypes.byref(h), D))
        if ws_bytes:
            ws = torch.empty(ws_bytes // 4, dtype=torch.float32, device=X.device)
    stream = ctypes.c_void_p(torch.cuda.current_stream(X.device).cuda_stream)
    with _on_device(X.device):
        check(L.hcspmm_forward_typed(_ptr(X), X.size(0), D, _ptr(Z), D, _DTYPES[X.dtype], _ptr(row_pointers), _ptr(column_index),
                                     _ptr(blockPartition), _ptr(edgeToColumn), _ptr(edgeToRow), _ptr(hybrid_type),
                                     _ptr(row_nzr) if h is not None else ctypes.c_void_p(0),
                                     ctypes.byref(h) if h is not None else None, N, E, D, _ptr(ws), ws_bytes, stream))
    return Z


def forward(X, row_pointers, column_index, blockPartition, edgeToColumn, edgeToRow, hybrid_type, row_nzr, col_nzr):
    return [_spmm(X, row_pointers, column_index, blockPartition, edgeToColumn, edgeToRow, hybrid_type, row_nzr, col_nzr)]


def forward_rect(X_full, row_pointers, column_index, blockPartition, edgeToColumn, edgeToRow, hybrid_type, row_nzr,
                 col_nzr):
    return [_spmm(X_full, row_pointers, column_index, blockPartition, edgeToColumn, edgeToRow, hybrid_type, row_nzr,
                  col_nzr, rect=True)]


def forward_into(X, Z, row_pointers, column_index, blockPartition, edgeToColumn, edgeToRow, hybrid_type, row_nzr,
                 col_nzr, workspace=None):
    L = lib()
    for t, n in ((row_pointers, "nodePointer"), (column_index, "edgeList"), (blockPartition, "blockPartition"),
                 (edgeToColumn, "edgeToColumn"), (edgeToRow, "edgeToRow")):
        _check_input(t, n)
    for t, n in ((X, "input"), (Z, "output")):
        if not t.is_cuda:
            raise RuntimeError("%s must be a CUDA tensor" % n)
        if t.dtype not in _DTYPES or t.dtype != X.dtype or t.dim() != 2 or t.stride(1) != 1 or t.stride(0) < t.size(1):
            raise RuntimeError("%s must be a 2-D float32 / float16 / bfloat16 view with unit inner stride" % n)
    N, E, D = row_pointers.size(0) - 1, column_index.size(0), X.size(1)
    if Z.size(0) != N or Z.size(1) != D:
        raise RuntimeError("output must be [num_nodes, embedding_dim]")
    h = _checked_header(row_nzr, row_pointers, column_index, N, E, X.size(0))
    ws, ws_bytes = None, 0
    if h is not None:
        ws_bytes = int(L.hcspmm_workspace_bytes(ctypes.byref(h), D))
        if ws_bytes:
            if workspace is not None and workspace.numel() * workspace.element_size() >= ws_bytes:
                ws = workspace
            else:
                ws = torch.empty(ws_bytes // 4, dtype=torch.float32, device=X.device)
    stream = ctypes.c_void_p(torch.cuda.current_stream(X.device).cuda_stream)
    with _on_device(X.device):
        check(L.hcspmm_forward_typed(_ptr(X), X.size(0), X.stride(0), _ptr(Z), Z.stride(0), _DTYPES[X.dtype], _ptr(row_pointers),
                                     _ptr(column_index), _ptr(blockPartition), _ptr(edgeToColumn), _ptr(edgeToRow),
                                     _ptr(hybrid_type), _ptr(row_nzr) if h is not None else ctypes.c_void_p(0),
                                     ctypes.byref(h) if h is not None else None, N, E, D, _ptr(ws), ws_bytes, stream))
    return Z
# ... 790 lines not shown
```

### hc-spmm_amd/hcspmm/capi.py

```python
import ctypes
import os

_HERE = os.path.dirname(os.path.abspath(__file__))
LIB_PATH = os.environ.get("HCSPMM_LIB") or os.path.normpath(os.path.join(_HERE, "..", "csrc", "libhcspmm.so"))

RULE_INTENDED = 0
RULE_INTENDED_GUARD = 1
RULE_AS_SHIPPED = 2
RULE_MI355X = 3
RULE_MI355X_WIDE = 4

OK, EINVAL, ENOMEM, EPLAN, EHIP, EWORKSPACE, ERANGE = 0, -1, -2, -3, -4, -5, -6


class Header(ctypes.Structure):
    WORDS = 64
    MAGIC = 0x48435350
    _fields_ = [(n, ctypes.c_int32) for n in (
        "magic", "version", "total_words", "num_nodes", "num_edges", "num_windows", "split_threshold", "segment_len",
        "n_tasks", "n_dense", "n_split_rows", "n_partials", "off_tasks", "off_dense_index", "off_dense_pack",
        "off_fixups", "nnz_sparse", "nnz_dense", "uniq_dense", "max_dense_k")] + [("n_len_gt", ctypes.c_int32 * 5),
                                                                                  ("n_tiny", ctypes.c_int32), ("n_dense_compact", ctypes.c_int32),
                                                                                  ("off_dense_compact", ctypes.c_int32), ("n_dense_compact2", ctypes.c_int32),
                                                                                  ("off_dense_compact2", ctypes.c_int32), ("num_columns", ctypes.c_int32),
                                                                                  ("n_sparse_windows", ctypes.c_int32), ("off_sparse_windows", ctypes.c_int32),
                                                                                  ("fingerprint_lo", ctypes.c_uint32), ("fingerprint_hi", ctypes.c_uint32),
                                                                                  ("dense_k_sum", ctypes.c_int32), ("flags", ctypes.c_int32),
                                                                                  ("n_slices", ctypes.c_int32), ("slice_threshold", ctypes.c_int32),
                                                                                  ("off_slice_table", ctypes.c_int32), ("off_slice_tasks", ctypes.c_int32),
                                                                                  ("n_slice_tasks", ctypes.c_int32), ("slice_xcd_tasks", ctypes.c_int32),
                                                                                  ("nnz_sliced", ctypes.c_int32), ("n_sliced_rows", ctypes.c_int32),
                                                                                  ("panel_cols", ctypes.c_int32), ("reserved", ctypes.c_int32 * 18)]

    @property
    def fingerprint(self):
        return (int(self.fingerprint_hi) << 32) | int(self.fingerprint_lo)


class PlanParams(ctypes.Structure):
    _fields_ = [("split_threshold", ctypes.c_int32), ("segment_len", ctypes.c_int32), ("fuse_in_launch", ctypes.c_int32),
                ("slice_threshold", ctypes.c_int32), ("n_slices", ctypes.c_int32), ("panel_cols", ctypes.c_int32)]


_vp, _i64, _int, _sz = ctypes.c_void_p, ctypes.c_int64, ctypes.c_int, ctypes.c_size_t
_hp, _pp = ctypes.POINTER(Header), ctypes.POINTER(PlanParams)
SYMBOLS = {
    "hcspmm_strerror": (ctypes.c_char_p, [_int]),
    "hcspmm_abi_version": (_int, []),
    "hcspmm_last_hip_error": (_int, []),
    "hcspmm_preprocess_host": (_int, [_vp, _vp, _i64, _i64, _i64, _int, _int, _vp, _vp, _vp, _vp]),
    "hcspmm_edge_to_row_device": (_int, [_vp, _i64, _i64, _vp, _vp]),
    "hcspmm_plan_words": (_int, [_vp, _i64, _i64, _vp, _vp, _pp, ctypes.POINTER(_i64)]),
    "hcspmm_plan_build": (_int, [_vp, _vp, _i64, _i64, _i64, _vp, _vp, _vp, _pp, _vp, _i64]),
    "hcspmm_plan_check": (_int, [_hp, _i64, _i64, _i64]),
    "hcspmm_graph_fingerprint_host": (_int, [_vp, _vp, _i64, _i64, ctypes.POINTER(ctypes.c_uint64)]),
    "hcspmm_graph_fingerprint_device": (_int, [_vp, _vp, _i64, _i64, _vp, _vp]),
    "hcspmm_workspace_bytes": (_sz, [_hp, _int]),
    "hcspmm_wide_threshold": (ctypes.c_int32, [_hp, _int]),
    "hcspmm_wide_threshold_typed": (ctypes.c_int32, [_hp, _int, _int]),
    "hcspmm_own_tiny_launch": (ctypes.c_int32, [_hp, _int]),
    "hcspmm_wide_threshold_fp8": (ctypes.c_int32, [_hp, _int]),
    "hcspmm_quantize_fp8": (_int, [_vp, _i64, _i64, _int, _int, _vp, _vp, _i64, _vp, _vp]),
    "hcspmm_forward_fp8": (_int, [_vp, _i64, _i64, _int, _vp, _vp, _vp, _i64, _vp, _vp, _vp, _vp, _vp, _vp, _vp, _hp, _i64, _i64,
                                  _int, _vp, _sz, _vp]),
    "hcspmm_forward_typed": (_int, [_vp, _i64, _i64, _vp, _i64, _int, _vp, _vp, _vp, _vp, _vp, _vp, _vp, _hp, _i64, _i64, _int, _vp,
                                    _sz, _vp]),
    "hcspmm_forward_weighted": (_int, [_vp, _i64, _i64, _vp, _i64, _int, _vp, _vp, _vp, _vp, _vp, _vp, _vp, _hp, _i64, _i64, _int,
                                       _vp, _sz, _vp, _vp]),
    "hcspmm_forward_weighted_heads": (_int, [_vp, _i64, _i64, _vp, _i64, _int, _vp, _vp, _vp, _vp, _vp, _vp, _vp, _hp, _i64, _i64,
                                             _int, _vp, _sz, _vp, _vp, _int]),
    "hcspmm_forward_weighted_indexed": (_int, [_vp, _i64, _i64, _vp, _i64, _int, _vp, _vp, _vp, _vp, _vp, _vp, _vp, _hp, _i64, _i64,
                                               _int, _vp, _sz, _vp, _vp, _int, _vp, _i64]),
    "hcspmm_extremum_workspace_bytes": (_sz, [_hp, _int]),
    "hcspmm_forward_extremum": (_int, [_vp, _i64, _i64, _vp, _i64, _int, _vp, _vp, _vp, _vp, _vp, _vp, _vp, _hp, _i64, _i64, _int,
                                       _vp, _sz, _vp, _int, _vp, _i64]),
    "hcspmm_forward_extremum_backward": (_int, [_vp, _i64, _vp, _i64, _vp, _i64, _vp, _vp, _vp, _vp, _vp, _vp, _vp, _hp, _i64, _i64,
                                                _int, _vp, _vp, _sz, _vp]),
    "hcspmm_forward_edge_messages": (_int, [_vp, _i64, _i64, _vp, _i64, _i64, _vp, _int, _vp, _i64, _vp, _vp, _vp, _vp, _vp, _vp, _vp,
                                            _hp, _i64, _i64, _int, _vp, _sz, _vp]),
    "hcspmm_edge_messages_grad": (_int, [_vp, _i64, _vp, _i64, _i64, _vp, _i64, _vp, _i64, _int, _vp, _vp, _i64, _i64, _int, _vp]),
    "hcspmm_edge_norm_device": (_int, [_vp, _vp, _i64, _i64, _int, _vp, _vp]),
    "hcspmm_transpose_permutation": (_int, [_vp, _vp, _i64, _i64, _vp]),
    "hcspmm_transpose_graph": (_int, [_vp, _vp, _i64, _i64, _i64, _vp, _vp, _vp]),
    "hcspmm_sddmm": (_int, [_vp, _i64, _vp, _i64, _i64, _int, _vp, _vp, _vp, _vp, _hp, _i64, _i64, _int, _vp]),
    "hcspmm_sddmm_heads": (_int, [_vp, _i64, _vp, _i64, _i64, _int, _vp, _vp, _vp, _vp, _hp, _i64, _i64, _int, _vp, _int]),
    "hcspmm_edge_softmax": (_int, [_vp, _vp, _vp, _i64, _i64, _int, _vp]),
    "hcspmm_edge_softmax_backward": (_int, [_vp, _vp, _vp, _vp, _i64, _i64, _int, _vp]),
    "hcspmm_gat_attention": (_int, [_vp, _vp, _i64, ctypes.c_float, _vp, _vp, _vp, _i64, _i64, _int, _vp]),
    "hcspmm_gat_attention_backward": (_int, [_vp, _vp, _vp, _vp, ctypes.c_float, _vp, _vp, _vp, _i64, _i64, _int, _vp, _vp, _vp,
                                             _vp]),
    "hcspmm_gat_attention_backward_directed": (_int, [_vp, _vp, _vp, _vp, ctypes.c_float, _vp, _vp, _vp, _vp, _i64, _i64, _i64, _int,
                                                      _vp, _vp, _vp, _vp]),
    "hcspmm_gatv2_scores": (_int, [_vp, _i64, _vp, _i64, _i64, _vp, ctypes.c_float, _vp, _vp, _vp, _i64, _i64, _int, _int, _vp]),
    "hcspmm_gatv2_backward_workspace_bytes": (_sz, [_i64, _i64, _int, _int]),
    "hcspmm_gatv2_scores_backward": (_int, [_vp, _vp, _i64, _vp, _i64, _vp, ctypes.c_float, _vp, _vp, _vp, _i64, _i64, _int, _int,
                                            _vp, _i64, _vp, _i64, _vp, _vp, _sz, _vp]),
    "hcspmm_gatv2_scores_backward_directed": (_int, [_vp, _vp, _i64, _vp, _i64, _vp, ctypes.c_float, _vp, _vp, _vp, _vp, _vp, _i64,
                                                     _i64, _i64, _int, _int, _vp, _i64, _vp, _i64, _vp, _vp, _sz, _vp]),
    "hcspmm_forward": (_int, [_vp, _vp, _vp, _vp, _vp, _vp, _vp, _vp, _vp, _hp, _i64, _i64, _int, _vp, _sz, _vp]),
    "hcspmm_forward_strided": (_int, [_vp, _i64, _i64, _vp, _i64, _vp, _vp, _vp, _vp, _vp, _vp, _vp, _hp, _i64, _i64, _int, _vp, _sz,
                                      _vp]),
    "hcspmm_forward_fused": (_int, [_vp, _vp, _vp, _vp, _i64, _i64, _int, _vp, _vp, _vp, _vp, _vp, _vp, _vp, _hp,
                                    _i64, _i64, _int, _vp, _sz, _vp]),
    "hcspmm_fused_in_launch": (_int, [_hp, _int, _int]),
    "hcspmm_dense_update": (_int, [_vp, _vp, _i64, _i64, _vp, _i64, _int, _int, _vp]),
    "hcspmm_weight_grad_workspace": (_sz, [_i64, _int, _int]),
    "hcspmm_weight_grad": (_int, [_vp, _i64, _vp, _i64, _vp, _i64, _int, _int, _vp, _sz, _vp]),
    "hcspmm_loi_reorder": (_int, [_vp, _vp, _i64, _i64, _vp, _vp, ctypes.POINTER(_i64)]),
    "hcspmm_loi_reorder_variant": (_int, [_vp, _vp, _i64, _i64, _int, _vp, _vp, ctypes.POINTER(_i64)]),
    "hcspmm_loi_reorder_fast": (_int, [_vp, _vp, _i64, _i64, _vp, _vp, _vp, ctypes.POINTER(_i64)]),
    "hcspmm_apply_permutation": (_int, [_vp, _vp, _i64, _i64, _vp, _vp, _vp]),
}

_LIB = None


def lib():
    global _LIB
    if _LIB is None:
        if not os.path.exists(LIB_PATH):
            raise RuntimeError("libhcspmm.so not found at %s -- run `python -c 'import __graft_entry__ as g; "
                               "g.build()'` (or make -C hc-spmm_amd/csrc); no fallback path exists" % LIB_PATH)
        L = ctypes.CDLL(LIB_PATH)
        for name, (res, args) in SYMBOLS.items():
            fn = getattr(L, name)
            fn.restype = res
            fn.argtypes = args
        _LIB = L
    return _LIB


def check(rc, soft=False):
    if rc != 0 and not soft:
        L = lib()
        msg = L.hcspmm_strerror(rc).decode()
        if rc == EHIP:
            msg += " (hipError_t %d)" % L.hcspmm_last_hip_error()
        raise RuntimeError("hcspmm: %s [code %d]" % (msg, rc))
    return rc
```

### hc-spmm_amd/hybrid_kernel/hybrid_all.cpp

```cpp
#include <torch/extension.h>

#include <c10/hip/HIPStream.h>

#include <cstring>
#include <mutex>
#include <unordered_map>
#include <vector>

#include "hcspmm.h"

namespace {

#define CHECK_CUDA(x) TORCH_CHECK(x.is_cuda(), #x " must be a CUDA tensor")
#define CHECK_CONTIGUOUS(x) TORCH_CHECK(x.is_contiguous(), #x " must be contiguous")
#define CHECK_INPUT(x) \
  CHECK_CUDA(x);       \
  CHECK_CONTIGUOUS(x)

int g_rule = HCSPMM_RULE_MI355X;
hcspmm_plan_params g_params = {0, 0, 0, 0, 0, 0};

void check_rc(int rc, const char* what) {
  TORCH_CHECK(rc == HCSPMM_OK, "HCSPMM.", what, ": ", hcspmm_strerror(rc), " [code ", rc, ", hipError_t ",
              hcspmm_last_hip_error(), "]");
}

typedef c10::weak_intrusive_ptr<c10::TensorImpl> WeakTensor;
WeakTensor weak_of(const torch::Tensor& t) { return WeakTensor(t.getIntrusivePtr()); }

struct GraphSeen {
  const void *rp, *col;
  WeakTensor rp_ref, col_ref;
};
struct PlanEntry {
  WeakTensor plan;
  hcspmm_plan_header header;
  std::vector<GraphSeen> graphs;
  uint64_t tick;
};
std::mutex g_mu;
std::unordered_map<const void*, PlanEntry> g_plans;
uint64_t g_tick = 0;
constexpr size_t kMaxPlans = 256, kMaxGraphsPerPlan = 8;

void remember(const torch::Tensor& plan, const hcspmm_plan_header& h, const torch::Tensor* rp, const torch::Tensor* col) {
  std::lock_guard<std::mutex> lk(g_mu);
  for (auto it = g_plans.begin(); it != g_plans.end();) it = it->second.plan.expired() ? g_plans.erase(it) : std::next(it);
  while (g_plans.size() >= kMaxPlans) {
    auto lru = g_plans.begin();
    for (auto it = g_plans.begin(); it != g_plans.end(); ++it)
      if (it->second.tick < lru->second.tick) lru = it;
    g_plans.erase(lru);
  }
  PlanEntry e{weak_of(plan), h, {}, ++g_tick};
  if (rp && col && rp->is_cuda()) e.graphs.push_back(GraphSeen{rp->data_ptr(), col->data_ptr(), weak_of(*rp), weak_of(*col)});
  g_plans.insert_or_assign(plan.data_ptr(), std::move(e));
}

bool lookup(const torch::Tensor& row_nzr, const torch::Tensor& nodePointer, const torch::Tensor& edgeList, int64_t N,
            int64_t E, hcspmm_plan_header* h) {
  if (!row_nzr.defined() || !row_nzr.is_cuda() || row_nzr.scalar_type() != torch::kInt ||
      row_nzr.numel() < HCSPMM_PLAN_HEADER_WORDS || !row_nzr.is_contiguous())
    return false;
  bool known = false, graph_ok = false;
  {
    std::lock_guard<std::mutex> lk(g_mu);
    auto it = g_plans.find(row_nzr.data_ptr());
    if (it != g_plans.end() && it->second.plan.expired()) {
      g_plans.erase(it);
      it = g_plans.end();
    }
    if (it != g_plans.end()) {
      known = true;
      it->second.tick = ++g_tick;
      *h = it->second.header;
      for (const GraphSeen& g : it->second.graphs)
        if (g.rp == nodePointer.data_ptr() && g.col == edgeList.data_ptr() && !g.rp_ref.expired() && !g.col_ref.expired())
          graph_ok = true;
    }
  }
  if (!known) {
    auto host = row_nzr.slice(0, 0, HCSPMM_PLAN_HEADER_WORDS).cpu().contiguous();
    std::memcpy(h, host.data_ptr<int>(), sizeof(*h));
    if (h->magic != HCSPMM_PLAN_MAGIC) return false;
  }
  check_rc(hcspmm_plan_check(h, N, E, row_nzr.numel()), "forward(plan check)");
  if (!graph_ok) {
    auto fp = torch::empty({1}, row_nzr.options().dtype(torch::kLong));
    const c10::DeviceGuard guard(row_nzr.device());
    check_rc(hcspmm_graph_fingerprint_device(nodePointer.data_ptr<int>(), edgeList.numel() ? edgeList.data_ptr<int>() : nullptr, N,
                                             E, reinterpret_cast<uint64_t*>(fp.data_ptr<int64_t>()),
                                             (void*)c10::hip::getCurrentHIPStream(row_nzr.device().index()).stream()),
             "forward(graph fingerprint)");
    const uint64_t got = (uint64_t)fp.item<int64_t>();
    const uint64_t want = ((uint64_t)h->fingerprint_hi << 32) | h->fingerprint_lo;
    TORCH_CHECK(got == want, "HCSPMM.forward: plan does not match this graph (nodePointer / edgeList differ from the ones "
                "the plan was built from) [code ", HCSPMM_EPLAN, "]");
    if (!known) remember(row_nzr, *h, &nodePointer, &edgeList);
    else {
      std::lock_guard<std::mutex> lk(g_mu);
      auto it = g_plans.find(row_nzr.data_ptr());
      if (it != g_plans.end()) {
        if (it->second.graphs.size() >= kMaxGraphsPerPlan) it->second.graphs.erase(it->second.graphs.begin());
        it->second.graphs.push_back(GraphSeen{nodePointer.data_ptr(), edgeList.data_ptr(), weak_of(nodePointer), weak_of(edgeList)});
      }
    }
  }
  return true;
}

struct Call {
  int64_t N, E;
  int D;
  bool has_plan;
  hcspmm_plan_header header;
  torch::Tensor workspace;
  void* stream;
};

int feature_dtype(const torch::Tensor& t) {
  switch (t.scalar_type()) {
    case torch::kFloat: return HCSPMM_DTYPE_F32;
    case torch::kHalf: return HCSPMM_DTYPE_F16;
    case torch::kBFloat16: return HCSPMM_DTYPE_BF16;
    default: return -1;
  }
}

Call prepare(const torch::Tensor& input, const torch::Tensor& nodePointer, const torch::Tensor& edgeList,
             const torch::Tensor& blockPartition, const torch::Tensor& edgeToColumn, const torch::Tensor& edgeToRow,
             const torch::Tensor& row_nzr, bool allow_16bit = false, bool rect = false, bool strided = false,
             const torch::Tensor* workspace = nullptr, bool fp8 = false) {
  if (strided) {
    CHECK_CUDA(input);
  } else {
    CHECK_INPUT(input);
  }
  CHECK_INPUT(nodePointer);
  CHECK_INPUT(edgeList);
  CHECK_INPUT(blockPartition);
  CHECK_INPUT(edgeToColumn);
  CHECK_INPUT(edgeToRow);
  if (fp8) {
    TORCH_CHECK(input.dim() == 2 && (input.scalar_type() == torch::kFloat8_e4m3fn || input.scalar_type() == torch::kByte),
                "input must be a 2-D float8_e4m3fn (or uint8) tensor");
  } else {
    TORCH_CHECK(input.dim() == 2 && (allow_16bit ? feature_dtype(input) >= 0 : input.scalar_type() == torch::kFloat),
                allow_16bit ? "input must be a 2-D float32 / float16 / bfloat16 tensor" : "input must be a 2-D float32 tensor");
  }
  TORCH_CHECK(nodePointer.scalar_type() == torch::kInt && edgeList.scalar_type() == torch::kInt,
              "nodePointer / edgeList must be int32");
  Call c;
  c.N = nodePointer.size(0) - 1;
  c.E = edgeList.size(0);
  c.D = (int)input.size(1);
  TORCH_CHECK(rect || input.size(0) == c.N, "input has ", input.size(0), " rows but the graph has ", c.N, " nodes");
  c.has_plan = lookup(row_nzr, nodePointer, edgeList, c.N, c.E, &c.header);
  if (c.has_plan) {
    TORCH_CHECK(input.size(0) >= c.header.num_columns, "input has ", input.size(0), " rows but the plan gathers from ",
                c.header.num_columns);
    const size_t need = hcspmm_workspace_bytes(&c.header, c.D);
    if (need) {
      if (workspace && workspace->defined() && workspace->is_cuda() && (size_t)workspace->nbytes() >= need)
        c.workspace = *workspace;
      else
        c.workspace = torch::empty({(int64_t)(need / 4)}, input.options().dtype(torch::kFloat));
    }
  }
  c.stream = (void*)c10::hip::getCurrentHIPStream(input.device().index()).stream();
  return c;
}

const int* iptr(const torch::Tensor& t) { return (t.defined() && t.numel() > 0) ? t.data_ptr<int>() : nullptr; }
// ... 564 lines not shown
                                                   (void*)c10::hip::getCurrentHIPStream(H_dst.device().index()).stream()),
             "gatv2_scores_backward_directed");
    return {grad_dst, grad_src, grad_att};
  }
  check_rc(hcspmm_gatv2_scores_backward(fptr(grad_logits), fptr(H_dst), H_dst.stride(0), fptr(H_src), H_src.stride(0), fptr(att),
                                        (float)negative_slope, iptr(nodePointer), iptr(edgeList), iptr(perm32), N, E, (int)D,
                                        (int)heads, mfptr(grad_dst), D, mfptr(grad_src), D, mfptr(grad_att), mfptr(ws), ws_bytes,
                                        (void*)c10::hip::getCurrentHIPStream(H_dst.device().index()).stream()),
           "gatv2_scores_backward");
  return {grad_dst, grad_src, grad_att};
}

std::vector<torch::Tensor> gatv2_scores_backward(torch::Tensor grad_logits, torch::Tensor H_dst, torch::Tensor H_src,
                                                 torch::Tensor att, torch::Tensor nodePointer, torch::Tensor edgeList,
                                                 torch::Tensor perm, double negative_slope) {
  return gatv2_scores_backward_any(grad_logits, H_dst, H_src, att, nodePointer, edgeList, torch::Tensor(), torch::Tensor(), perm,
                                   negative_slope);
}

std::vector<torch::Tensor> run_fused(const torch::Tensor& input, const torch::Tensor& nodePointer,
                                     const torch::Tensor& edgeList, const torch::Tensor& blockPartition,
                                     const torch::Tensor& edgeToColumn, const torch::Tensor& edgeToRow,
                                     const torch::Tensor& hybrid_type, const torch::Tensor& row_nzr,
                                     const torch::Tensor& weights, torch::Tensor output) {
  Call c = prepare(input, nodePointer, edgeList, blockPartition, edgeToColumn, edgeToRow, row_nzr);
  TORCH_CHECK(weights.is_cuda() && weights.scalar_type() == torch::kFloat && weights.dim() == 2 &&
                  weights.size(0) == c.D,
              "weights must be a CUDA float32 tensor of shape [embedding_dim, hidden_dim]");
  const int H = (int)weights.size(1);
  if (!output.defined()) {
    output = torch::empty({c.N, (int64_t)H}, input.options());
  } else {
    CHECK_INPUT(output);
    TORCH_CHECK(output.scalar_type() == torch::kFloat && output.numel() == c.N * H,
                "output must be float32 with num_nodes*hidden_dim elements");
  }
  auto output2 = torch::empty({c.N, (int64_t)c.D}, input.options());
  const c10::DeviceGuard guard(input.device());
  const int rc = hcspmm_forward_fused(
      input.data_ptr<float>(), output.data_ptr<float>(), output2.data_ptr<float>(), weights.data_ptr<float>(),
      weights.stride(0), weights.stride(1), H, iptr(nodePointer), iptr(edgeList), iptr(blockPartition),
      iptr(edgeToColumn), iptr(edgeToRow), iptr(hybrid_type), c.has_plan ? iptr(row_nzr) : nullptr,
      c.has_plan ? &c.header : nullptr, c.N, c.E, c.D, c.workspace.defined() ? c.workspace.data_ptr() : nullptr,
      c.workspace.defined() ? (size_t)c.workspace.nbytes() : 0, c.stream);
  check_rc(rc, "forward_fused");
  return {output, output2};
}

torch::Tensor to_host_i32(const torch::Tensor& t) {
  if (t.is_cuda() && t.scalar_type() == torch::kInt && t.is_contiguous() && t.numel() > (1 << 16)) {
    auto host = torch::empty(t.sizes(), torch::TensorOptions().dtype(torch::kInt).pinned_memory(true));
    host.copy_(t, true);
    c10::hip::getCurrentHIPStream(t.device().index()).synchronize();
    return host;
  }
  return t.to(torch::kCPU, torch::kInt).contiguous();
}

}

std::vector<torch::Tensor> preprocess(torch::Tensor edgeList_tensor, torch::Tensor nodePointer_tensor, int num_nodes,
                                      int edge_num, int block_num, int64_t num_columns) {
  (void)edge_num;
  auto dev = edgeList_tensor.device();
  auto col = to_host_i32(edgeList_tensor);
  auto rp = to_host_i32(nodePointer_tensor);
  const int64_t N = rp.numel() - 1, E = col.numel(), W = (N + HCSPMM_BLK_H - 1) / HCSPMM_BLK_H;
  TORCH_CHECK(num_nodes == N, "preprocess: num_nodes (", num_nodes, ") != row_pointers.size(0)-1 (", N, ")");
  TORCH_CHECK(block_num == W, "preprocess: num_row_windows (", block_num, ") != ceil(N/16) (", W, ")");
  const int64_t M = num_columns > 0 ? num_columns : N;
  auto opts = torch::TensorOptions().dtype(torch::kInt);
  auto hopts = opts.pinned_memory(dev.is_cuda());
  auto bp = torch::empty({W}, hopts), ht = torch::empty({W}, hopts), e2c = torch::empty({E}, hopts);
  torch::Tensor e2r;
  if (dev.is_cuda()) {
    e2r = torch::empty({E}, opts.device(dev));
    auto rp_dev = nodePointer_tensor.to(dev, torch::kInt).contiguous();
    const c10::DeviceGuard guard(dev);
    check_rc(hcspmm_edge_to_row_device(rp_dev.data_ptr<int>(), N, E, mptr(e2r),
                                       (void*)c10::hip::getCurrentHIPStream(dev.index()).stream()),
             "preprocess(edgeToRow)");
  } else {
    e2r = torch::empty({E}, opts);
  }
  check_rc(hcspmm_preprocess_host(rp.data_ptr<int>(), iptr(col), N, E, M, g_rule, 0, mptr(bp), mptr(e2c),
                                  dev.is_cuda() ? nullptr : mptr(e2r), mptr(ht)),
           "preprocess");
  auto bp_d = bp.to(dev, true), e2c_d = e2c.to(dev, true), ht_d = ht.to(dev, true);
  int64_t words = 0;
  check_rc(hcspmm_plan_words(rp.data_ptr<int>(), N, E, iptr(bp), iptr(ht), &g_params, &words), "preprocess(plan size)");
  auto plan = torch::empty({std::max<int64_t>(words, HCSPMM_PLAN_HEADER_WORDS)}, hopts);
  check_rc(hcspmm_plan_build(rp.data_ptr<int>(), iptr(col), N, E, M, iptr(bp), iptr(e2c), iptr(ht), &g_params,
                             plan.data_ptr<int>(), plan.numel()),
           "preprocess(plan build)");
  hcspmm_plan_header h;
  std::memcpy(&h, plan.data_ptr<int>(), sizeof(h));
  plan = plan.narrow(0, 0, h.total_words);
  auto plan_d = plan.to(dev, true);
  if (plan_d.is_cuda()) remember(plan_d, h, &nodePointer_tensor, &edgeList_tensor);
  auto col_nzr = torch::zeros({1}, opts).to(dev);
  return {bp_d, e2c_d, e2r.to(dev), ht_d, plan_d, col_nzr};
}

#define HCSPMM_GRAPH_PARAMS                                                                                   \
  torch::Tensor input, torch::Tensor nodePointer, torch::Tensor edgeList, torch::Tensor blockPartition,       \
      torch::Tensor edgeToColumn, torch::Tensor edgeToRow, torch::Tensor hybrid_type, torch::Tensor row_nzr,  \
      torch::Tensor col_nzr

std::vector<torch::Tensor> spmm_forward(HCSPMM_GRAPH_PARAMS) {
  return {run_spmm(input, nodePointer, edgeList, blockPartition, edgeToColumn, edgeToRow, hybrid_type, row_nzr)};
}

std::vector<torch::Tensor> spmm_forward_fused(HCSPMM_GRAPH_PARAMS, torch::Tensor weights) {
  return run_fused(input, nodePointer, edgeList, blockPartition, edgeToColumn, edgeToRow, hybrid_type, row_nzr,
                   weights, torch::Tensor());
}

std::vector<torch::Tensor> spmm_forward_final_fused(HCSPMM_GRAPH_PARAMS, torch::Tensor weights,
                                                    torch::Tensor output) {
  return run_fused(input, nodePointer, edgeList, blockPartition, edgeToColumn, edgeToRow, hybrid_type, row_nzr,
                   weights, output);
}

std::vector<torch::Tensor> spmm_forward_rect(HCSPMM_GRAPH_PARAMS) {
  return {run_spmm(input, nodePointer, edgeList, blockPartition, edgeToColumn, edgeToRow, hybrid_type, row_nzr, true)};
}

torch::Tensor spmm_forward_into(torch::Tensor input, torch::Tensor output, torch::Tensor nodePointer, torch::Tensor edgeList,
                                torch::Tensor blockPartition, torch::Tensor edgeToColumn, torch::Tensor edgeToRow,
                                torch::Tensor hybrid_type, torch::Tensor row_nzr, torch::Tensor col_nzr,
                                c10::optional<torch::Tensor> workspace) {
  (void)col_nzr;
  for (const torch::Tensor* t : {&input, &output}) {
    TORCH_CHECK(t->is_cuda() && feature_dtype(*t) >= 0 && t->scalar_type() == input.scalar_type() && t->dim() == 2 &&
                    t->stride(1) == 1 && t->stride(0) >= t->size(1),
                t == &input ? "input" : "output", " must be a 2-D float32 / float16 / bfloat16 view with unit inner stride");
  }
  torch::Tensor ws = workspace.has_value() ? *workspace : torch::Tensor();
  Call c = prepare(input, nodePointer, edgeList, blockPartition, edgeToColumn, edgeToRow, row_nzr, true, true, true, &ws);
  TORCH_CHECK(output.size(0) == c.N && output.size(1) == c.D, "output must be [num_nodes, embedding_dim]");
  const c10::DeviceGuard guard(input.device());
  const int rc = hcspmm_forward_typed(
      input.data_ptr(), input.size(0), input.stride(0), output.data_ptr(), output.stride(0), feature_dtype(input),
      iptr(nodePointer), iptr(edgeList), iptr(blockPartition), iptr(edgeToColumn), iptr(edgeToRow), iptr(hybrid_type),
      c.has_plan ? iptr(row_nzr) : nullptr, c.has_plan ? &c.header : nullptr, c.N, c.E, c.D,
      c.workspace.defined() ? c.workspace.data_ptr() : nullptr, c.workspace.defined() ? (size_t)c.workspace.nbytes() : 0,
      c.stream);
  check_rc(rc, "forward_into");
  return output;
}

torch::Tensor build_plan(torch::Tensor row_pointers, torch::Tensor column_index, torch::Tensor blockPartition,
                         torch::Tensor edgeToColumn, torch::Tensor hybrid_type, int split_threshold, int segment_len,
                         int64_t num_columns, int fuse_in_launch, int slice_threshold, int n_slices, int panel_cols) {
  auto rp = to_host_i32(row_pointers), col = to_host_i32(column_index), bp = to_host_i32(blockPartition),
       e2c = to_host_i32(edgeToColumn), ht = to_host_i32(hybrid_type);
  const int64_t N = rp.numel() - 1, E = col.numel();
  hcspmm_plan_params pp = (split_threshold || segment_len || fuse_in_launch || slice_threshold || n_slices || panel_cols)
                              ? hcspmm_plan_params{split_threshold, segment_len, fuse_in_launch, slice_threshold, n_slices, panel_cols}
                              : g_params;
  int64_t words = 0;
  check_rc(hcspmm_plan_words(rp.data_ptr<int>(), N, E, iptr(bp), iptr(ht), &pp, &words), "build_plan(plan size)");
  auto plan = torch::empty({std::max<int64_t>(words, HCSPMM_PLAN_HEADER_WORDS)}, torch::TensorOptions().dtype(torch::kInt));
  check_rc(hcspmm_plan_build(rp.data_ptr<int>(), iptr(col), N, E, num_columns > 0 ? num_columns : N, iptr(bp), iptr(e2c),
                             iptr(ht), &pp, plan.data_ptr<int>(), plan.numel()),
           "build_plan");
  hcspmm_plan_header h;
  std::memcpy(&h, plan.data_ptr<int>(), sizeof(h));
  plan = plan.narrow(0, 0, h.total_words);
  auto plan_d = plan.to(row_pointers.device());
  if (plan_d.is_cuda()) remember(plan_d, h, &row_pointers, &column_index);
  return plan_d;
}

PYBIND11_MODULE(TORCH_EXTENSION_NAME, m) {
  m.def("preprocess", &preprocess, "Preprocess step: window condensing + classifier + MI355X launch plan (host)",
        pybind11::arg("column_index"), pybind11::arg("row_pointers"), pybind11::arg("num_nodes"), pybind11::arg("num_edges"),
        pybind11::arg("num_row_windows"), pybind11::arg("num_columns") = -1);
  m.def("forward", &spmm_forward, "HCSPMM SPMM forward (gfx950)");
  m.def("forward_more", &spmm_forward, "HCSPMM SPMM forward more (gfx950)");
  m.def("forward_fixed32", &spmm_forward, "HCSPMM SPMM forward fixed32 (gfx950)");
  m.def("forward_fixed32_fused", &spmm_forward_fused, "HCSPMM SPMM forward fixed32 fused (gfx950)");
  m.def("forward_final_fused", &spmm_forward_final_fused, "HCSPMM SPMM forward final fused (gfx950)");
  m.def("forward_fixed64", &spmm_forward, "HCSPMM SPMM forward fixed64 (gfx950)");
  m.def("forward_fixed64_fused", &spmm_forward_fused, "HCSPMM SPMM forward fixed64 fused (gfx950)");
  m.def("forward_final_fused_64", &spmm_forward_final_fused, "HCSPMM SPMM forward final fused 64 (gfx950)");
  m.def("forward_GIN_final_fused", &spmm_forward_fused, "HCSPMM SPMM forward for GIN final fused (gfx950)");
  m.def("backward", &spmm_forward, "HCSPMM SPMM backward (gfx950)");
  m.def("backward_fixed32", &spmm_forward, "HCSPMM SPMM backward fixed32 (gfx950)");
  m.def("backward_fixed32_fused", &spmm_forward_fused, "HCSPMM SPMM backward fixed32 fused (gfx950)");
  m.def("backward_final_fused", &spmm_forward_final_fused, "HCSPMM SPMM backward final fused (gfx950)");
  m.def("backward_fixed64", &spmm_forward, "HCSPMM SPMM backward fixed 64 (gfx950)");
  m.def("backward_fixed64_fused", &spmm_forward_fused, "HCSPMM SPMM backward fixed 64 fused (gfx950)");
  m.def("backward_final_fused_64", &spmm_forward_final_fused, "HCSPMM SPMM backward final fused 64 (gfx950)");
  m.def("backward_GIN_final_fused", &spmm_forward_fused, "HCSPMM SPMM backward for GIN final fused (gfx950)");
  m.def("forward_rect", &spmm_forward_rect, "A (n x M row block) * X_full (M x D) -> [Z (n x D)]");
  m.def("forward_into", &spmm_forward_into, "Z_view[:, :] = A @ X_view on strided column panels",
        pybind11::arg("input"), pybind11::arg("output"), pybind11::arg("nodePointer"), pybind11::arg("edgeList"),
        pybind11::arg("blockPartition"), pybind11::arg("edgeToColumn"), pybind11::arg("edgeToRow"),
        pybind11::arg("hybrid_type"), pybind11::arg("row_nzr"), pybind11::arg("col_nzr"),
        pybind11::arg("workspace") = pybind11::none());
  m.def("build_plan", &build_plan, "launch plan (row_nzr) for a caller-supplied window classification",
        pybind11::arg("row_pointers"), pybind11::arg("column_index"), pybind11::arg("blockPartition"),
        pybind11::arg("edgeToColumn"), pybind11::arg("hybrid_type"), pybind11::arg("split_threshold") = 0,
        pybind11::arg("segment_len") = 0, pybind11::arg("num_columns") = -1, pybind11::arg("fuse_in_launch") = 0,
        pybind11::arg("slice_threshold") = 0, pybind11::arg("n_slices") = 0, pybind11::arg("panel_cols") = 0);
  m.def("wide_threshold", [](torch::Tensor row_nzr, int embedding_dim, int dtype) {
    hcspmm_plan_header h;
    bool has = false;
    if (row_nzr.defined() && row_nzr.numel() >= HCSPMM_PLAN_HEADER_WORDS && row_nzr.scalar_type() == torch::kInt) {
      auto host = row_nzr.slice(0, 0, HCSPMM_PLAN_HEADER_WORDS).cpu().contiguous();
      std::memcpy(&h, host.data_ptr<int>(), sizeof(h));
      has = h.magic == HCSPMM_PLAN_MAGIC;
    }
    return (int64_t)hcspmm_wide_threshold_typed(has ? &h : nullptr, embedding_dim, dtype);
  }, "rows with more entries than this are summed by a whole wave (hcspmm.h hcspmm_wide_threshold_typed)",
        pybind11::arg("row_nzr"), pybind11::arg("embedding_dim"), pybind11::arg("dtype") = 0);
  m.def("set_rule", [](int rule) {
    TORCH_CHECK(rule >= HCSPMM_RULE_INTENDED && rule <= HCSPMM_RULE_MI355X_WIDE, "unknown rule");
    g_rule = rule;
  }, "3 = MI355X refit, narrow / width-agnostic (default), 4 = MI355X refit for embedding widths of 64 columns and more; the reference's: "
     "0 = intended classifier (hybrid_all_kernel.cu:261), 1 = with the size>32 guard, 2 = as shipped (:262, every window on the sparse-row path)");
  m.def("get_rule", []() { return g_rule; });
  m.def("set_plan_params", [](int split_threshold, int segment_len, int fuse_in_launch, int slice_threshold, int n_slices, int panel_cols) {
    g_params.split_threshold = split_threshold;
    g_params.segment_len = segment_len;
    g_params.fuse_in_launch = fuse_in_launch;
    g_params.slice_threshold = slice_threshold;
    g_params.n_slices = n_slices;
    g_params.panel_cols = panel_cols;
  }, "rows longer than split_threshold are cut into segments of segment_len entries (0 = defaults); fuse_in_launch: 1 = the fused "
     "operators update dense-tile windows inside the hybrid launch, 2 = sparse rows as well (row-tile form); slice_threshold / n_slices: XCD-affine column slices "
     "(hcspmm.h hcspmm_plan_params: 0 = automatic, < 0 = off)",
        pybind11::arg("split_threshold"), pybind11::arg("segment_len"), pybind11::arg("fuse_in_launch") = 0,
        pybind11::arg("slice_threshold") = 0, pybind11::arg("n_slices") = 0, pybind11::arg("panel_cols") = 0);
  m.def("fused_in_launch", [](torch::Tensor row_nzr, int embedding_dim, int hidden_dim) {
    hcspmm_plan_header h;
    if (!row_nzr.defined() || row_nzr.numel() < HCSPMM_PLAN_HEADER_WORDS || row_nzr.scalar_type() != torch::kInt) return 0;
    auto host = row_nzr.slice(0, 0, HCSPMM_PLAN_HEADER_WORDS).cpu().contiguous();
    std::memcpy(&h, host.data_ptr<int>(), sizeof(h));
    return h.magic == HCSPMM_PLAN_MAGIC ? hcspmm_fused_in_launch(&h, embedding_dim, hidden_dim) : 0;
  }, "form forward_*_fused takes with this plan and shape: 0 = two launches, 1 = dense-tile windows update inside the hybrid "
     "launch, 2 = the sparse-row path as well (row-tile form)");
  m.def("forward_weighted", &spmm_forward_weighted, "edge-weighted aggregation [A_w * X] (gfx950)");
  m.def("quantize_fp8", &quantize_fp8,
        "per-row quantiser: float32 [rows, D] -> (float8_e4m3fn codes [rows, D], float32 scale [rows]), code = rne(clamp(x / scale, "
        "-448, 448)), scale = amax / 448 unless given (gfx950)",
        pybind11::arg("input"), pybind11::arg("scale") = c10::optional<torch::Tensor>());
  m.def("forward_fp8", [](torch::Tensor input, c10::optional<torch::Tensor> scale, torch::Tensor nodePointer, torch::Tensor edgeList,
                          torch::Tensor blockPartition, torch::Tensor edgeToColumn, torch::Tensor edgeToRow,
                          torch::Tensor hybrid_type, torch::Tensor row_nzr, torch::Tensor col_nzr) {
    return std::vector<torch::Tensor>{run_spmm_fp8(input, scale, nullptr, nodePointer, edgeList, blockPartition, edgeToColumn,
                                                   edgeToRow, hybrid_type, row_nzr)};
  }, "aggregation of 8-bit features: float32 [A * (scale[:, None] * Xq)], scale float32 [N] or None (gfx950)");
  m.def("forward_weighted_fp8", [](torch::Tensor input, c10::optional<torch::Tensor> scale, torch::Tensor values,
                                   torch::Tensor nodePointer, torch::Tensor edgeList, torch::Tensor blockPartition,
                                   torch::Tensor edgeToColumn, torch::Tensor edgeToRow, torch::Tensor hybrid_type,
                                   torch::Tensor row_nzr, torch::Tensor col_nzr) {
    return std::vector<torch::Tensor>{run_spmm_fp8(input, scale, &values, nodePointer, edgeList, blockPartition, edgeToColumn,
                                                   edgeToRow, hybrid_type, row_nzr)};
  }, "edge-weighted aggregation of 8-bit features: float32 [A_w * (scale[:, None] * Xq)] (gfx950)");
  m.def("wide_threshold_fp8", [](torch::Tensor row_nzr, int embedding_dim) {
    hcspmm_plan_header h;
    bool has = false;
    if (row_nzr.defined() && row_nzr.numel() >= HCSPMM_PLAN_HEADER_WORDS && row_nzr.scalar_type() == torch::kInt) {
      auto host = row_nzr.slice(0, 0, HCSPMM_PLAN_HEADER_WORDS).cpu().contiguous();
      std::memcpy(&h, host.data_ptr<int>(), sizeof(h));
      has = h.magic == HCSPMM_PLAN_MAGIC;
    }
    return (int64_t)hcspmm_wide_threshold_fp8(has ? &h : nullptr, embedding_dim);
  }, "wide_threshold for forward_fp8 / forward_weighted_fp8 (hcspmm.h hcspmm_wide_threshold_fp8)");
  m.def("edge_norm", [](torch::Tensor row_pointers, torch::Tensor column_index, std::string kind) {
    TORCH_CHECK(kind == "sym" || kind == "mean", "kind must be 'sym' or 'mean', got '", kind, "'");
    CHECK_INPUT(row_pointers);
    CHECK_INPUT(column_index);
    TORCH_CHECK(row_pointers.scalar_type() == torch::kInt && column_index.scalar_type() == torch::kInt,
                "nodePointer / edgeList must be int32");
    const int64_t N = row_pointers.numel() - 1, E = column_index.numel();
    auto out = torch::empty({E}, row_pointers.options().dtype(torch::kFloat));
    const c10::DeviceGuard guard(row_pointers.device());
    check_rc(hcspmm_edge_norm_device(iptr(row_pointers), iptr(column_index), N, E, kind == "sym" ? HCSPMM_NORM_SYM : HCSPMM_NORM_MEAN,
                                     E ? out.data_ptr<float>() : nullptr,
                                     (void*)c10::hip::getCurrentHIPStream(row_pointers.device().index()).stream()),
             "edge_norm");
    return out;
  }, "edge values of the 'sym' (1/sqrt(deg_r deg_c)) or 'mean' (1/deg_r) normalisation, on the device");
  m.def("transpose_permutation", [](torch::Tensor row_pointers, torch::Tensor column_index) {
    auto rp = row_pointers.to(torch::kCPU, torch::kInt).contiguous();
    auto col = column_index.to(torch::kCPU, torch::kInt).contiguous();
    const int64_t N = rp.numel() - 1, E = col.numel();
    auto perm = torch::empty({E}, rp.options());
    check_rc(hcspmm_transpose_permutation(rp.data_ptr<int>(), E ? col.data_ptr<int>() : nullptr, N, E,
                                          E ? perm.data_ptr<int>() : nullptr),
             "transpose_permutation");
    return perm.to(row_pointers.device(), torch::kLong);
  }, "perm with values[perm] = the values of A_w^T in A's CSR order (pattern-symmetric graphs)");
  m.def("transpose_graph", [](torch::Tensor row_pointers, torch::Tensor column_index, c10::optional<int64_t> num_cols) {
    auto rp = row_pointers.to(torch::kCPU, torch::kInt).contiguous();
    auto col = column_index.to(torch::kCPU, torch::kInt).contiguous();
    TORCH_CHECK(rp.dim() == 1 && rp.numel() >= 1 && col.dim() == 1, "row_pointers [N + 1] and column_index [E] must be 1-D");
    const int64_t N = rp.numel() - 1, E = col.numel(), M = num_cols.has_value() ? *num_cols : N;
    TORCH_CHECK(M >= 0, "num_cols must not be negative, got ", M);
    auto rp_t = torch::empty({M + 1}, rp.options()), col_t = torch::empty({E}, rp.options()), eid_t = torch::empty({E}, rp.options());
    check_rc(hcspmm_transpose_graph(rp.data_ptr<int>(), E ? col.data_ptr<int>() : nullptr, N, M, E, rp_t.data_ptr<int>(),
                                    E ? col_t.data_ptr<int>() : nullptr, E ? eid_t.data_ptr<int>() : nullptr),
             "transpose_graph");
    const auto dev = row_pointers.device();
    return std::vector<torch::Tensor>{rp_t.to(dev), col_t.to(dev), eid_t.to(dev)};
  }, "A^T of any CSR graph (host counting sort) -> [row_pointers_t, column_index_t, entry_index_t], int32 on the inputs' device; "
     "entry_index_t[e_t] = the CSR position in A of A^T's entry e_t",
        pybind11::arg("row_pointers"), pybind11::arg("column_index"), pybind11::arg("num_cols") = pybind11::none());
  m.def("forward_weighted_indexed", &spmm_forward_weighted_indexed,
        "multi-head edge-weighted aggregation with indexed values [Z]: entry e of head h weighs values[h][value_index[e]]; the "
        "bits of forward_weighted_heads(X, values[:, value_index]) without the gathered copy (gfx950)");
  m.def("gat_attention_backward_directed",
        [](torch::Tensor alpha, torch::Tensor grad_alpha, torch::Tensor s_dst, torch::Tensor s_src, torch::Tensor row_pointers,
           torch::Tensor column_index, torch::Tensor row_pointers_t, torch::Tensor entry_index_t, double negative_slope) {
          TORCH_CHECK(row_pointers_t.defined(), "row_pointers_t is required");
          return gat_attention_backward_any(alpha, grad_alpha, s_dst, s_src, row_pointers, column_index, row_pointers_t,
                                            entry_index_t, negative_slope);
        },
        "backward of gat_attention on any square graph; (row_pointers_t, entry_index_t) from transpose_graph -> [grad_s_dst, "
        "grad_s_src, grad_scores] (gfx950)",
        pybind11::arg("alpha"), pybind11::arg("grad_alpha"), pybind11::arg("s_dst"), pybind11::arg("s_src"),
        pybind11::arg("row_pointers"), pybind11::arg("column_index"), pybind11::arg("row_pointers_t"),
        pybind11::arg("entry_index_t"), pybind11::arg("negative_slope") = 0.2);
  m.def("gatv2_scores_backward_directed",
        [](torch::Tensor grad_logits, torch::Tensor H_dst, torch::Tensor H_src, torch::Tensor att, torch::Tensor row_pointers,
           torch::Tensor column_index, torch::Tensor row_pointers_t, torch::Tensor column_index_t, torch::Tensor entry_index_t,
           double negative_slope) {
          TORCH_CHECK(row_pointers_t.defined() && column_index_t.defined(), "row_pointers_t and column_index_t are required");
          return gatv2_scores_backward_any(grad_logits, H_dst, H_src, att, row_pointers, column_index, row_pointers_t,
                                           column_index_t, entry_index_t, negative_slope);
        },
        "backward of gatv2_scores on any square graph; (row_pointers_t, column_index_t, entry_index_t) from transpose_graph -> "
        "[grad_H_dst, grad_H_src, grad_att] (gfx950)",
        pybind11::arg("grad_logits"), pybind11::arg("H_dst"), pybind11::arg("H_src"), pybind11::arg("att"),
        pybind11::arg("row_pointers"), pybind11::arg("column_index"), pybind11::arg("row_pointers_t"),
        pybind11::arg("column_index_t"), pybind11::arg("entry_index_t"), pybind11::arg("negative_slope") = 0.2);
  m.def("forward_weighted_heads", &spmm_forward_weighted_heads,
        "multi-head edge-weighted aggregation [Z]: values [heads, E], head h weights columns h*Dh ... (h+1)*Dh - 1 (gfx950)");
  m.def("sddmm_heads", &spmm_sddmm_heads,
        "multi-head sampled dense-dense product: float32 [heads, E], one Dh-column slice per head (gfx950)");
  m.def("forward_max", [](torch::Tensor input, torch::Tensor nodePointer, torch::Tensor edgeList, torch::Tensor blockPartition,
                          torch::Tensor edgeToColumn, torch::Tensor edgeToRow, torch::Tensor hybrid_type, torch::Tensor row_nzr,
                          torch::Tensor col_nzr, bool return_arg) {
    return spmm_forward_extremum(input, nodePointer, edgeList, blockPartition, edgeToColumn, edgeToRow, hybrid_type, row_nzr, col_nzr,
                                 return_arg, HCSPMM_REDUCE_MAX);
  }, "max over each row's neighbours -> [Z, arg] ([Z] with return_arg=False); ties to the lowest entry, NaN wins (gfx950)",
        pybind11::arg("input"), pybind11::arg("row_pointers"), pybind11::arg("column_index"), pybind11::arg("blockPartition"),
        pybind11::arg("edgeToColumn"), pybind11::arg("edgeToRow"), pybind11::arg("hybrid_type"), pybind11::arg("row_nzr"),
        pybind11::arg("col_nzr"), pybind11::arg("return_arg") = true);
  m.def("forward_min", [](torch::Tensor input, torch::Tensor nodePointer, torch::Tensor edgeList, torch::Tensor blockPartition,
                          torch::Tensor edgeToColumn, torch::Tensor edgeToRow, torch::Tensor hybrid_type, torch::Tensor row_nzr,
                          torch::Tensor col_nzr, bool return_arg) {
    return spmm_forward_extremum(input, nodePointer, edgeList, blockPartition, edgeToColumn, edgeToRow, hybrid_type, row_nzr, col_nzr,
                                 return_arg, HCSPMM_REDUCE_MIN);
  }, "min over each row's neighbours -> [Z, arg] ([Z] with return_arg=False); ties to the lowest entry, NaN wins (gfx950)",
        pybind11::arg("input"), pybind11::arg("row_pointers"), pybind11::arg("column_index"), pybind11::arg("blockPartition"),
        pybind11::arg("edgeToColumn"), pybind11::arg("edgeToRow"), pybind11::arg("hybrid_type"), pybind11::arg("row_nzr"),
        pybind11::arg("col_nzr"), pybind11::arg("return_arg") = true);
  m.def("forward_extremum_backward", &spmm_forward_extremum_backward,
        "backward of forward_max / forward_min -> grad_X: a square, pattern-symmetric graph with perm = int32 transpose_permutation, "
        "or any square graph's A^T (transpose_graph's tensors and their preprocessing) with perm = entry_index_t (gfx950)");
  m.def("forward_edge_messages", &spmm_forward_edge_messages,
        "edge-feature messages [Z]: Z[r] = sum over the entries e of row r of m(X[col(e)], F[index[e] or e]); op 'mul' x * f, "
        "'add_relu' relu(x + f), 'copy' f (input may be None) (gfx950)",
        pybind11::arg("input"), pybind11::arg("F"), pybind11::arg("row_pointers"), pybind11::arg("column_index"),
        pybind11::arg("blockPartition"), pybind11::arg("edgeToColumn"), pybind11::arg("edgeToRow"), pybind11::arg("hybrid_type"),
        pybind11::arg("row_nzr"), pybind11::arg("col_nzr"), pybind11::arg("op") = "add_relu", pybind11::arg("index") = pybind11::none());
  m.def("edge_messages_grad", &spmm_edge_messages_grad,
        "gradient of forward_edge_messages with respect to F: float32 [E, D] (input / F may be None where the op does not read them) "
        "(gfx950)",
        pybind11::arg("dZ"), pybind11::arg("input"), pybind11::arg("F"), pybind11::arg("row_pointers"), pybind11::arg("column_index"),
        pybind11::arg("op") = "add_relu");
  m.def("sddmm", &spmm_sddmm, "sampled dense-dense product on the stored entries: float32 [E], out[e] = <A[row(e)], B[col(e)]> (gfx950)");
  m.def("edge_softmax", &edge_softmax, "softmax of float32 [E] / [heads, E] logits over each row's stored entries (gfx950)");
  m.def("edge_softmax_backward", &edge_softmax_backward,
        "grad_logits = alpha * (grad_alpha - row sum of alpha * grad_alpha), shapes as edge_softmax (gfx950)");
  m.def("gat_attention", &gat_attention,
        "GAT attention weights: softmax over each row of LeakyReLU(s_dst[row] + s_src[col]), s_* float32 [rows] / [rows, heads] "
        "-> [E] / [heads, E] (gfx950)",
        pybind11::arg("s_dst"), pybind11::arg("s_src"), pybind11::arg("row_pointers"), pybind11::arg("column_index"),
        pybind11::arg("negative_slope") = 0.2);
  m.def("gat_attention_backward", &gat_attention_backward,
        "backward of gat_attention (square, pattern-symmetric graph; perm = transpose_permutation) -> [grad_s_dst, grad_s_src, "
        "grad_scores] (gfx950)",
        pybind11::arg("alpha"), pybind11::arg("grad_alpha"), pybind11::arg("s_dst"), pybind11::arg("s_src"),
        pybind11::arg("row_pointers"), pybind11::arg("column_index"), pybind11::arg("perm"), pybind11::arg("negative_slope") = 0.2);
  m.def("gatv2_scores", &gatv2_scores,
        "GATv2 attention logits: float32 [heads, E], out[h][e] = sum_k att[h][k] * LeakyReLU(H_dst[row(e)][h*Dh + k] + "
        "H_src[col(e)][h*Dh + k]) (gfx950)",
        pybind11::arg("H_dst"), pybind11::arg("H_src"), pybind11::arg("att"), pybind11::arg("row_pointers"),
        pybind11::arg("column_index"), pybind11::arg("negative_slope") = 0.2);
  m.def("gatv2_scores_backward", &gatv2_scores_backward,
        "backward of gatv2_scores (square, pattern-symmetric graph; perm = transpose_permutation) -> [grad_H_dst, grad_H_src, "
        "grad_att] (gfx950)",
        pybind11::arg("grad_logits"), pybind11::arg("H_dst"), pybind11::arg("H_src"), pybind11::arg("att"),
        pybind11::arg("row_pointers"), pybind11::arg("column_index"), pybind11::arg("perm"), pybind11::arg("negative_slope") = 0.2);
  m.def("abi_version", []() { return hcspmm_abi_version(); });
  m.def("loi_reorder", [](torch::Tensor row_pointers, torch::Tensor column_index, int variant) {
    auto rp = row_pointers.to(torch::kCPU, torch::kInt).contiguous();
    auto col = column_index.to(torch::kCPU, torch::kInt).contiguous();
    const int64_t N = rp.numel() - 1, E = col.numel();
    auto perm = torch::empty({N}, torch::kInt), sizes = torch::empty({std::max<int64_t>(N, 1)}, torch::kInt);
    int64_t ng = 0;
    check_rc(hcspmm_loi_reorder_variant(rp.data_ptr<int>(), iptr(col), N, E, variant, mptr(perm), sizes.data_ptr<int>(), &ng),
             "loi_reorder");
    return std::vector<torch::Tensor>{perm, sizes.slice(0, 0, ng).clone()};
  }, "-> [perm (old vertex id at each new position), group sizes]; variant 0 = reorder_plus_new_direct, 1 = reorder_plus_new, "
     "2 / 3 = the windowed reorder_plus_direct / reorder_plus (>= 50 rows, no empty rows)",
        pybind11::arg("row_pointers"), pybind11::arg("column_index"), pybind11::arg("variant") = 0);
  m.def("loi_reorder_fast", [](torch::Tensor row_pointers, torch::Tensor column_index, int batch, int list_cap, int threads) {
    auto rp = row_pointers.to(torch::kCPU, torch::kInt).contiguous();
    auto col = column_index.to(torch::kCPU, torch::kInt).contiguous();
    const int64_t N = rp.numel() - 1, E = col.numel();
    auto perm = torch::empty({N}, torch::kInt), sizes = torch::empty({std::max<int64_t>(N, 1)}, torch::kInt);
    int64_t ng = 0;
    const hcspmm_loi_fast_params params = {batch, list_cap, threads, 0};
    {
      pybind11::gil_scoped_release no_gil;
      check_rc(hcspmm_loi_reorder_fast(rp.data_ptr<int>(), iptr(col), N, E, &params, mptr(perm), sizes.data_ptr<int>(), &ng),
               "loi_reorder_fast");
    }
    return std::vector<torch::Tensor>{perm, sizes.slice(0, 0, ng).clone()};
  }, "the relaxed parallel LOI reorder (hcspmm.h hcspmm_loi_reorder_fast) -> [perm, group sizes]: NOT the reference's permutation "
     "unless batch = 1 and list_cap < 0; deterministic for a given (batch, list_cap) whatever the thread count",
        pybind11::arg("row_pointers"), pybind11::arg("column_index"), pybind11::arg("batch") = 0, pybind11::arg("list_cap") = 0,
        pybind11::arg("threads") = 0);
  m.def("apply_permutation", [](torch::Tensor row_pointers, torch::Tensor column_index, torch::Tensor perm) {
    auto rp = row_pointers.to(torch::kCPU, torch::kInt).contiguous();
    auto col = column_index.to(torch::kCPU, torch::kInt).contiguous();
    auto p = perm.to(torch::kCPU, torch::kInt).contiguous();
    const int64_t N = rp.numel() - 1, E = col.numel();
    TORCH_CHECK(p.numel() == N, "perm must have num_nodes entries");
    auto rp2 = torch::empty({N + 1}, torch::kInt), col2 = torch::empty({E}, torch::kInt);
    check_rc(hcspmm_apply_permutation(rp.data_ptr<int>(), iptr(col), N, E, iptr(p), rp2.data_ptr<int>(), mptr(col2)),
             "apply_permutation");
    return std::vector<torch::Tensor>{rp2, col2};
  }, "relabel a CSR graph with a LOI permutation -> [row_pointers, column_index]");
  m.def("update", [](torch::Tensor X, torch::Tensor W) -> torch::Tensor {
    if (!(X.is_cuda() && W.is_cuda() && X.scalar_type() == torch::kFloat && W.scalar_type() == torch::kFloat && X.dim() == 2 &&
          W.dim() == 2 && X.size(1) == W.size(0) && X.is_contiguous() && X.size(0) > 0 && X.size(1) > 0 && W.size(1) > 0))
      return torch::Tensor();
    auto out = torch::empty({X.size(0), W.size(1)}, X.options());
    const c10::DeviceGuard guard(X.device());
    check_rc(hcspmm_dense_update(X.data_ptr<float>(), W.data_ptr<float>(), W.stride(0), W.stride(1), out.data_ptr<float>(), X.size(0),
                                 (int)X.size(1), (int)W.size(1), (void*)c10::hip::getCurrentHIPStream(X.device().index()).stream()),
             "update");
    return out;
  }, "X * W (the layers' update GEMM; W may be a transposed view); None if the operands are not contiguous fp32 device matrices");
  m.def("weight_grad", [](torch::Tensor A, torch::Tensor B) -> torch::Tensor {
    if (!(A.is_cuda() && B.is_cuda() && A.scalar_type() == torch::kFloat && B.scalar_type() == torch::kFloat &&
          A.dim() == 2 && B.dim() == 2 && A.size(0) == B.size(0) && A.stride(1) == 1 && B.stride(1) == 1 &&
          A.stride(0) >= A.size(1) && B.stride(0) >= B.size(1)))
      return torch::Tensor();
    const int64_t N = A.size(0);
    const int D = (int)A.size(1), H = (int)B.size(1);
    const size_t need = hcspmm_weight_grad_workspace(N, D, H);
    if (need == 0) return torch::Tensor();
    auto ws = torch::empty({(int64_t)(need / 4)}, A.options());
    auto out = torch::empty({(int64_t)D, (int64_t)H}, A.options());
    const c10::DeviceGuard guard(A.device());
    check_rc(hcspmm_weight_grad(A.data_ptr<float>(), A.stride(0), B.data_ptr<float>(), B.stride(0), out.data_ptr<float>(), N,
                                D, H, ws.data_ptr(), need, (void*)c10::hip::getCurrentHIPStream(A.device().index()).stream()),
             "weight_grad");
    return out;
  }, "dW = A^T B for the layers' backward passes (split-K MFMA kernel); None if the shape is unsupported");
  m.def("plan_info", [](torch::Tensor row_nzr) {
    pybind11::dict d;
    hcspmm_plan_header h;
    if (!row_nzr.defined() || row_nzr.numel() < HCSPMM_PLAN_HEADER_WORDS || row_nzr.scalar_type() != torch::kInt) return d;
    auto host = row_nzr.slice(0, 0, HCSPMM_PLAN_HEADER_WORDS).cpu().contiguous();
    std::memcpy(&h, host.data_ptr<int>(), sizeof(h));
    if (h.magic != HCSPMM_PLAN_MAGIC) return d;
    d["n_tasks"] = h.n_tasks; d["n_dense"] = h.n_dense; d["n_split_rows"] = h.n_split_rows;
    d["n_partials"] = h.n_partials; d["nnz_sparse"] = h.nnz_sparse; d["nnz_dense"] = h.nnz_dense;
    d["uniq_dense"] = h.uniq_dense; d["split_threshold"] = h.split_threshold; d["segment_len"] = h.segment_len;
    d["max_dense_k"] = h.max_dense_k; d["n_tiny"] = h.n_tiny; d["n_dense_compact"] = h.n_dense_compact;
    d["n_dense_compact2"] = h.n_dense_compact2; d["num_columns"] = h.num_columns;
    d["panel_cols"] = h.panel_cols; d["n_slices"] = h.n_slices; d["slice_threshold"] = h.slice_threshold; d["n_slice_tasks"] = h.n_slice_tasks;
    d["nnz_sliced"] = h.nnz_sliced; d["n_sliced_rows"] = h.n_sliced_rows; d["total_words"] = h.total_words;
    d["n_sparse_windows"] = h.n_sparse_windows; d["dense_k_sum"] = h.dense_k_sum; d["flags"] = h.flags; d["num_nodes"] = h.num_nodes; d["num_edges"] = h.num_edges;
    d["fingerprint"] = ((uint64_t)h.fingerprint_hi << 32) | h.fingerprint_lo;
    return d;
  }, "fields of the launch plan carried in row_nzr ({} for the reference's [0] placeholder)");
}
```

### include/hcspmm.h

```cpp
#ifndef HCSPMM_H
#define HCSPMM_H

#include <stddef.h>
#include <stdint.h>

#ifdef __cplusplus
extern "C" {
#endif

#define HCSPMM_ABI_VERSION 3

#define HCSPMM_BLK_H 16
#define HCSPMM_BLK_W 8

#define HCSPMM_OK 0
#define HCSPMM_EINVAL (-1)
#define HCSPMM_ENOMEM (-2)
#define HCSPMM_EPLAN (-3)
#define HCSPMM_EHIP (-4)
#define HCSPMM_EWORKSPACE (-5)
#define HCSPMM_ERANGE (-6)

#define HCSPMM_RULE_INTENDED 0
#define HCSPMM_RULE_INTENDED_GUARD 1
#define HCSPMM_RULE_AS_SHIPPED 2
#define HCSPMM_RULE_MI355X 3
#define HCSPMM_RULE_MI355X_WIDE 4

const char* hcspmm_strerror(int code);
int hcspmm_abi_version(void);
int hcspmm_last_hip_error(void);

int hcspmm_preprocess_host(const int32_t* row_pointers_h, const int32_t* column_index_h, int64_t num_nodes,
                           int64_t num_edges, int64_t num_columns, int rule, int num_threads,
                           int32_t* blockPartition_h, int32_t* edgeToColumn_h, int32_t* edgeToRow_h,
                           int32_t* hybrid_type_h);

int hcspmm_edge_to_row_device(const int32_t* row_pointers_d, int64_t num_nodes, int64_t num_edges, int32_t* edgeToRow_d,
                              void* stream);

#define HCSPMM_PLAN_MAGIC 0x48435350
#define HCSPMM_PLAN_VERSION 7
#define HCSPMM_TINY_LEN 2
#define HCSPMM_COMPACT_K 40
#define HCSPMM_COMPACT_WORDS 64
#define HCSPMM_COMPACT2_K 80
#define HCSPMM_COMPACT2_WORDS 128
#define HCSPMM_PLAN_HEADER_WORDS 64

typedef struct hcspmm_plan_header {
  int32_t magic;
  int32_t version;
  int32_t total_words;
  int32_t num_nodes;
  int32_t num_edges;
  int32_t num_windows;
  int32_t split_threshold;
  int32_t segment_len;
  int32_t n_tasks;
  int32_t n_dense;
  int32_t n_split_rows;
  int32_t n_partials;
  int32_t off_tasks;
  int32_t off_dense_index;
  int32_t off_dense_pack;
  int32_t off_fixups;
  int32_t nnz_sparse;
  int32_t nnz_dense;
  int32_t uniq_dense;
  int32_t max_dense_k;
  int32_t n_len_gt[5];
  int32_t n_tiny;
  int32_t n_dense_compact;
  int32_t off_dense_compact;
  int32_t n_dense_compact2;
  int32_t off_dense_compact2;
  int32_t num_columns;
  int32_t n_sparse_windows;
  int32_t off_sparse_windows;
  uint32_t fingerprint_lo;
  uint32_t fingerprint_hi;
  int32_t dense_k_sum;
  int32_t flags;
  int32_t n_slices;
  int32_t slice_threshold;
  int32_t off_slice_table;
  int32_t off_slice_tasks;
  int32_t n_slice_tasks;
  int32_t slice_xcd_tasks;
  int32_t nnz_sliced;
  int32_t n_sliced_rows;
  int32_t panel_cols;
  int32_t reserved[18];
} hcspmm_plan_header;

#define HCSPMM_PLAN_FUSE_IN_LAUNCH 1
#define HCSPMM_PLAN_FUSE_ROWS 2
#define HCSPMM_PLAN_FUSE_NEVER 4

typedef struct hcspmm_plan_params {
  int32_t split_threshold;
  int32_t segment_len;
  int32_t fuse_in_launch;
  int32_t slice_threshold;
  int32_t n_slices;
  int32_t panel_cols;
} hcspmm_plan_params;

int hcspmm_plan_words(const int32_t* row_pointers_h, int64_t num_nodes, int64_t num_edges,
                      const int32_t* blockPartition_h, const int32_t* hybrid_type_h,
                      const hcspmm_plan_params* params, int64_t* words_out);

int hcspmm_plan_build(const int32_t* row_pointers_h, const int32_t* column_index_h, int64_t num_nodes,
                      int64_t num_edges, int64_t num_columns, const int32_t* blockPartition_h,
                      const int32_t* edgeToColumn_h, const int32_t* hybrid_type_h, const hcspmm_plan_params* params,
                      int32_t* plan_h, int64_t words);

int hcspmm_plan_check(const hcspmm_plan_header* header_h, int64_t num_nodes, int64_t num_edges,
                      int64_t plan_words_available);

int hcspmm_graph_fingerprint_host(const int32_t* row_pointers_h, const int32_t* column_index_h, int64_t num_nodes,
                                  int64_t num_edges, uint64_t* fingerprint_out_h);
int hcspmm_graph_fingerprint_device(const int32_t* row_pointers_d, const int32_t* column_index_d, int64_t num_nodes,
                                    int64_t num_edges, uint64_t* fingerprint_out_d, void* stream);

size_t hcspmm_workspace_bytes(const hcspmm_plan_header* header_h, int embedding_dim);

int32_t hcspmm_wide_threshold(const hcspmm_plan_header* header_h, int embedding_dim);

int hcspmm_forward(const float* X_d, float* Z_d, const int32_t* row_pointers_d, const int32_t* column_index_d,
                   const int32_t* blockPartition_d, const int32_t* edgeToColumn_d, const int32_t* edgeToRow_d,
                   const int32_t* hybrid_type_d, const int32_t* plan_d, const hcspmm_plan_header* plan_header_h,
                   int64_t num_nodes, int64_t num_edges, int embedding_dim, void* workspace_d,
                   size_t workspace_bytes, void* stream);

int hcspmm_forward_strided(const float* X_d, int64_t x_rows, int64_t ldx, float* Z_d, int64_t ldz, const int32_t* row_pointers_d,
                           const int32_t* column_index_d, const int32_t* blockPartition_d,
                           const int32_t* edgeToColumn_d, const int32_t* edgeToRow_d, const int32_t* hybrid_type_d,
                           const int32_t* plan_d, const hcspmm_plan_header* plan_header_h, int64_t num_nodes,
                           int64_t num_edges, int embedding_dim, void* workspace_d, size_t workspace_bytes,
                           void* stream);

#define HCSPMM_DTYPE_F32 0
#define HCSPMM_DTYPE_F16 1
#define HCSPMM_DTYPE_BF16 2

int hcspmm_forward_typed(const void* X_d, int64_t x_rows, int64_t ldx, void* Z_d, int64_t ldz, int dtype,
                         const int32_t* row_pointers_d, const int32_t* column_index_d,
                         const int32_t* blockPartition_d, const int32_t* edgeToColumn_d, const int32_t* edgeToRow_d,
                         const int32_t* hybrid_type_d, const int32_t* plan_d, const hcspmm_plan_header* plan_header_h,
                         int64_t num_nodes, int64_t num_edges, int embedding_dim, void* workspace_d,
                         size_t workspace_bytes, void* stream);

int hcspmm_forward_weighted(const void* X_d, int64_t x_rows, int64_t ldx, void* Z_d, int64_t ldz, int dtype,
                            const int32_t* row_pointers_d, const int32_t* column_index_d, const int32_t* blockPartition_d,
                            const int32_t* edgeToColumn_d, const int32_t* edgeToRow_d, const int32_t* hybrid_type_d,
                            const int32_t* plan_d, const hcspmm_plan_header* plan_header_h, int64_t num_nodes,
                            int64_t num_edges, int embedding_dim, void* workspace_d, size_t workspace_bytes, void* stream,
                            const float* values_d);

#define HCSPMM_FP8_E4M3 0
int hcspmm_quantize_fp8(const float* X_d, int64_t rows, int64_t ldx, int embedding_dim, int format,
                        const float* scale_in_d , void* Xq_d, int64_t ldq, float* scale_out_d, void* stream);
int hcspmm_forward_fp8(const void* Xq_d, int64_t x_rows, int64_t ldx, int format, const float* row_scale_d ,
                       const float* values_d , float* Z_d, int64_t ldz, const int32_t* row_pointers_d,
                       const int32_t* column_index_d, const int32_t* blockPartition_d, const int32_t* edgeToColumn_d,
                       const int32_t* edgeToRow_d, const int32_t* hybrid_type_d, const int32_t* plan_d,
                       const hcspmm_plan_header* plan_header_h, int64_t num_nodes, int64_t num_edges, int embedding_dim,
                       void* workspace_d, size_t workspace_bytes, void* stream);
int32_t hcspmm_wide_threshold_fp8(const hcspmm_plan_header* header_h, int embedding_dim);

int hcspmm_forward_weighted_heads(const void* X_d, int64_t x_rows, int64_t ldx, void* Z_d, int64_t ldz, int dtype,
                                  const int32_t* row_pointers_d, const int32_t* column_index_d, const int32_t* blockPartition_d,
                                  const int32_t* edgeToColumn_d, const int32_t* edgeToRow_d, const int32_t* hybrid_type_d,
                                  const int32_t* plan_d, const hcspmm_plan_header* plan_header_h, int64_t num_nodes,
                                  int64_t num_edges, int embedding_dim, void* workspace_d, size_t workspace_bytes, void* stream,
                                  const float* values_d, int heads);

int hcspmm_forward_weighted_indexed(const void* X_d, int64_t x_rows, int64_t ldx, void* Z_d, int64_t ldz, int dtype,
                                    const int32_t* row_pointers_d, const int32_t* column_index_d, const int32_t* blockPartition_d,
                                    const int32_t* edgeToColumn_d, const int32_t* edgeToRow_d, const int32_t* hybrid_type_d,
                                    const int32_t* plan_d, const hcspmm_plan_header* plan_header_h, int64_t num_nodes,
                                    int64_t num_edges, int embedding_dim, void* workspace_d, size_t workspace_bytes, void* stream,
                                    const float* values_d, int heads, const int32_t* value_index_d , int64_t num_values);

#define HCSPMM_REDUCE_MAX 0
#define HCSPMM_REDUCE_MIN 1
size_t hcspmm_extremum_workspace_bytes(const hcspmm_plan_header* header_h, int embedding_dim);
int hcspmm_forward_extremum(const void* X_d, int64_t x_rows, int64_t ldx, void* Z_d, int64_t ldz, int dtype,
                            const int32_t* row_pointers_d, const int32_t* column_index_d, const int32_t* blockPartition_d,
                            const int32_t* edgeToColumn_d, const int32_t* edgeToRow_d, const int32_t* hybrid_type_d,
                            const int32_t* plan_d, const hcspmm_plan_header* plan_header_h, int64_t num_nodes,
                            int64_t num_edges, int embedding_dim, void* workspace_d, size_t workspace_bytes, void* stream,
                            int reduce, int32_t* arg_out_d, int64_t ldarg);

int hcspmm_forward_extremum_backward(const float* grad_Z_d, int64_t ldg, const int32_t* arg_d, int64_t ldarg,
                                     float* grad_X_out_d, int64_t ldgx, const int32_t* row_pointers_d,
                                     const int32_t* column_index_d, const int32_t* blockPartition_d,
                                     const int32_t* edgeToColumn_d, const int32_t* edgeToRow_d, const int32_t* hybrid_type_d,
                                     const int32_t* plan_d, const hcspmm_plan_header* plan_header_h, int64_t num_nodes,
                                     int64_t num_edges, int embedding_dim, const int32_t* transpose_perm_d, void* workspace_d,
                                     size_t workspace_bytes, void* stream);

#define HCSPMM_EDGE_OP_MUL 0
#define HCSPMM_EDGE_OP_ADD_RELU 1
#define HCSPMM_EDGE_OP_COPY 2
int hcspmm_forward_edge_messages(const void* X_d, int64_t x_rows, int64_t ldx, const float* F_d, int64_t f_rows, int64_t ldf,
                                 const int32_t* f_index_d , int op, void* Z_d, int64_t ldz,
                                 const int32_t* row_pointers_d, const int32_t* column_index_d, const int32_t* blockPartition_d,
                                 const int32_t* edgeToColumn_d, const int32_t* edgeToRow_d, const int32_t* hybrid_type_d,
                                 const int32_t* plan_d, const hcspmm_plan_header* plan_header_h, int64_t num_nodes,
                                 int64_t num_edges, int embedding_dim, void* workspace_d, size_t workspace_bytes, void* stream);

int hcspmm_edge_messages_grad(const float* grad_Z_d, int64_t ldg, const float* X_d, int64_t x_rows, int64_t ldx, const float* F_d,
                              int64_t ldf, float* grad_F_out_d, int64_t ldgf, int op, const int32_t* row_pointers_d,
                              const int32_t* column_index_d, int64_t num_nodes, int64_t num_edges, int embedding_dim,
                              void* stream);

#define HCSPMM_NORM_SYM 0
#define HCSPMM_NORM_MEAN 1
int hcspmm_edge_norm_device(const int32_t* row_pointers_d, const int32_t* column_index_d, int64_t num_nodes,
                            int64_t num_edges, int kind, float* values_out_d, void* stream);

int hcspmm_transpose_permutation(const int32_t* row_pointers_h, const int32_t* column_index_h, int64_t num_nodes,
                                 int64_t num_edges, int32_t* perm_out_h);

int hcspmm_transpose_graph(const int32_t* row_pointers_h, const int32_t* column_index_h, int64_t num_rows, int64_t num_cols,
                           int64_t num_edges, int32_t* row_pointers_t_out_h ,
                           int32_t* column_index_t_out_h ,
                           int32_t* entry_index_t_out_h );

int hcspmm_sddmm(const void* A_d, int64_t lda, const void* B_d, int64_t b_rows, int64_t ldb, int dtype, float* out_d,
                 const int32_t* row_pointers_d, const int32_t* column_index_d, const int32_t* plan_d,
                 const hcspmm_plan_header* plan_header_h, int64_t num_nodes, int64_t num_edges, int embedding_dim, void* stream);

int hcspmm_sddmm_heads(const void* A_d, int64_t lda, const void* B_d, int64_t b_rows, int64_t ldb, int dtype, float* out_d,
                       const int32_t* row_pointers_d, const int32_t* column_index_d, const int32_t* plan_d,
                       const hcspmm_plan_header* plan_header_h, int64_t num_nodes, int64_t num_edges, int embedding_dim,
                       void* stream, int heads);

int hcspmm_edge_softmax(const float* logits_d, float* alpha_out_d, const int32_t* row_pointers_d, int64_t num_nodes,
                        int64_t num_edges, int heads, void* stream);

int hcspmm_edge_softmax_backward(const float* alpha_d, const float* grad_alpha_d, float* grad_logits_out_d,
                                 const int32_t* row_pointers_d, int64_t num_nodes, int64_t num_edges, int heads, void* stream);

int hcspmm_gat_attention(const float* s_dst_d, const float* s_src_d, int64_t src_rows, float negative_slope,
                         float* alpha_out_d, const int32_t* row_pointers_d, const int32_t* column_index_d,
                         int64_t num_nodes, int64_t num_edges, int heads, void* stream);

int hcspmm_gat_attention_backward(const float* alpha_d, const float* grad_alpha_d, const float* s_dst_d,
                                  const float* s_src_d, float negative_slope, const int32_t* row_pointers_d,
                                  const int32_t* column_index_d, const int32_t* transpose_perm_d,
                                  int64_t num_nodes, int64_t num_edges, int heads,
                                  float* grad_scores_out_d ,
                                  float* grad_s_dst_out_d , float* grad_s_src_out_d ,
                                  void* stream);

int hcspmm_gat_attention_backward_directed(const float* alpha_d, const float* grad_alpha_d, const float* s_dst_d,
// ... 81 lines not shown
```

Measured before the change: 3758 billion.

## Add stream-phase SpMM path with LDS row accumulators and column-phased edge streams

Adds a new plan section that assigns sparse rows to a fixed set of persistent workgroups by greedy load balancing. Each row gets LDS accumulator slots, and its edges are cut into column-range phases so that all workgroups walk X in the same column order. Edges are packed into 64-entry chunks tagged with slot and start/end flags, and a new kernel consumes these streams in place of the sliced/segmented sparse path. The goal is better L2 reuse of X and less partial-sum traffic through global memory. In exchange it adds plan-build time, plan memory, and padding overhead, and it is enabled automatically only for large sliced graphs.

```diff
diff --git a/hc-spmm_amd/csrc/capi.hip b/hc-spmm_amd/csrc/capi.hip
--- a/hc-spmm_amd/csrc/capi.hip
+++ b/hc-spmm_amd/csrc/capi.hip
@@ -245,6 +245,15 @@
     }
     const int vec = pick_vec(dtype, D, ldx, ldz, X, Z, need ? workspace : nullptr);
     if (fused && (vec != 4 || dtype != HCSPMM_DTYPE_F32)) return HCSPMM_EINVAL;
+    if (ph->n_stream_wgs > 0 && !fused && !values && dtype == HCSPMM_DTYPE_F32 && vec == 4) {
+      a.n_stream_wgs = ph->n_stream_wgs;
+      a.stream_phases = ph->stream_phases;
+      a.stream_slots = ph->stream_slots;
+      a.off_stream_table = ph->off_stream_table;
+      a.off_stream_rowptr = ph->off_stream_rowptr;
+      a.off_stream_rows = ph->off_stream_rows;
+      a.off_stream = ph->off_stream;
+    }
     if (fused && (fused->mode & 2)) {
       e = hcspmm::launch_fused_tiles(a, stream);
       if (e != hipSuccess) return fail_hip(e);
diff --git a/hc-spmm_amd/csrc/plan_host.cpp b/hc-spmm_amd/csrc/plan_host.cpp
--- a/hc-spmm_amd/csrc/plan_host.cpp
+++ b/hc-spmm_amd/csrc/plan_host.cpp
@@ -27,6 +27,7 @@
 struct Resolved {
   int32_t split_threshold, segment_len, fuse_in_launch;
   int32_t slice_mode, slice_threshold, n_slices, panel_cols;
+  int32_t stream_mode, stream_wgs_per_cu;
 };
 
 int env_int(const char* name, int dflt) {
@@ -35,7 +36,7 @@
 }
 
 Resolved resolve(const hcspmm_plan_params* p) {
-  Resolved r{512, 256, 0, kSliceAuto, kSliceAutoThreshold, 8, 0};
+  Resolved r{512, 256, 0, kSliceAuto, kSliceAutoThreshold, 8, 0, 0, 5};
   if (p) {
     if (p->split_threshold > 0) r.split_threshold = p->split_threshold;
     if (p->segment_len > 0) r.segment_len = p->segment_len;
@@ -49,6 +50,10 @@
   else if (thr < 0) r.slice_mode = kSliceOff;
   if (ns > 0) r.n_slices = std::min(64, (ns + 7) / 8 * 8);
   if (p && p->panel_cols != 0) r.panel_cols = p->panel_cols < 0 ? -1 : std::min(1 << 20, (p->panel_cols + 15) / 16 * 16);
+  int sm = p ? p->stream_mode : 0;
+  if (sm == 0) sm = env_int("HCSPMM_STREAM", 0);
+  r.stream_mode = sm < 0 ? -1 : std::min(sm, 64);
+  if (p && p->stream_wgs_per_cu > 0) r.stream_wgs_per_cu = std::min(p->stream_wgs_per_cu, 16);
   return r;
 }
 
@@ -230,6 +235,281 @@
   return HCSPMM_OK;
 }
 
+constexpr int kStreamCUs = 256;
+constexpr int kStreamLdsPerCU = 160 * 1024;
+constexpr int kStreamSlotBytes = 128;
+constexpr int kStreamMaxSlots = 256;
+constexpr int kStreamColBits = 22;
+constexpr int32_t kStreamPadCol = (1 << kStreamColBits) - 1;
+constexpr int kStreamDefaultPhases = 8;
+
+struct StreamShape {
+  int G = 0, P = 0, cap = 0;
+  bool forced = false;
+  int64_t table_words = 0, rowptr_words = 0, rows_words = 0, chunk_budget = 0, extra_words = 0, entries = 0;
+};
+
+StreamShape stream_shape(const Resolved& rp, int64_t N, int64_t nnz_sparse, int64_t base) {
+  StreamShape s;
+  if (rp.stream_mode < 0 || N <= 0 || nnz_sparse <= 0) return s;
+  s.forced = rp.stream_mode > 0;
+  s.entries = nnz_sparse;
+  s.P = s.forced ? rp.stream_mode : kStreamDefaultPhases;
+  s.G = kStreamCUs * rp.stream_wgs_per_cu;
+  s.cap = std::min(kStreamMaxSlots, kStreamLdsPerCU / rp.stream_wgs_per_cu / kStreamSlotBytes);
+  s.table_words = align4((int64_t)s.G * 4 * s.P + 1);
+  s.rowptr_words = align4((int64_t)s.G + 1);
+  s.rows_words = align4(2 * N);
+  const int64_t per_wave_phase = (int64_t)s.G * 4 * s.P;
+  s.chunk_budget = (s.forced ? (nnz_sparse + 7) / 8 : (nnz_sparse * 3 / 2 + 63) / 64) + per_wave_phase;
+  s.extra_words = ((base + 63) & ~int64_t(63)) - base + s.table_words + s.rowptr_words + s.rows_words + 64 + 64 * s.chunk_budget;
+  return s;
+}
+
+bool stream_auto_candidate(const Resolved& rp, const Layout& sliced) {
+  return rp.stream_mode == 0 && rp.slice_mode == kSliceAuto && sliced.nnz_sliced * 20 >= sliced.nnz_sparse &&
+         sliced.nnz_sliced > 0 && sliced.nnz_sparse >= kSliceAutoMinEntries;
+}
+
+struct StreamResult {
+  bool built = false;
+  int32_t slots = 0;
+  int64_t chunks = 0, off_table = 0, off_rowptr = 0, off_rows = 0, off_stream = 0, end = 0;
+};
+
+StreamResult build_stream(const int32_t* rowptr, const int32_t* col, int64_t N, int64_t M, const int32_t* ht,
+                          const StreamShape& sh, int32_t thr, int32_t* plan, int64_t base, int64_t words, int T) {
+  StreamResult res;
+  if (sh.extra_words <= 0 || base + sh.extra_words > words || M - 1 >= kStreamPadCol) return res;
+  static const bool dbg = std::getenv("HCSPMM_PLAN_DEBUG") != nullptr;
+  auto now = [] { return std::chrono::duration<double, std::milli>(std::chrono::steady_clock::now().time_since_epoch()).count(); };
+  double ts[6] = {now(), 0, 0, 0, 0, 0};
+  const int G = sh.G, P = sh.P;
+  const int64_t W = (N + HCSPMM_BLK_H - 1) / HCSPMM_BLK_H;
+  auto sparse_window = [&](int64_t w) {
+    const int64_t r0 = w * HCSPMM_BLK_H, r1 = std::min<int64_t>(r0 + HCSPMM_BLK_H, N);
+    return !(ht[w] != 0 && rowptr[r1] > rowptr[r0]);
+  };
+  int shift = 0;
+  while (((M - 1) >> shift) >= 65536) ++shift;
+  const int64_t nb = ((M - 1) >> shift) + 1;
+  std::vector<std::vector<int64_t>> hist((size_t)T, std::vector<int64_t>((size_t)nb, 0));
+  std::vector<int> unsorted((size_t)T, 0);
+  std::vector<int64_t> nrows_part((size_t)T, 0);
+  parallel_for(T, [&](int t) {
+    int64_t* h = hist[(size_t)t].data();
+    int bad = 0;
+    int64_t nr = 0;
+    for (int64_t w = W * t / T; w < W * (t + 1) / T; ++w) {
+      if (!sparse_window(w)) continue;
+      const int64_t r0 = w * HCSPMM_BLK_H, r1 = std::min<int64_t>(r0 + HCSPMM_BLK_H, N);
+      nr += r1 - r0;
+      for (int64_t r = r0; r < r1; ++r) {
+        const int64_t e0 = rowptr[r], e1 = rowptr[r + 1];
+        for (int64_t e = e0 + 1; e < e1; ++e) bad |= col[e] < col[e - 1];
+        for (int64_t e = e0; e < e1; e += kSliceSample) h[col[e] >> shift]++;
+      }
+    }
+    unsorted[(size_t)t] = bad;
+    nrows_part[(size_t)t] = nr;
+  });
+  int64_t n_rows = 0, total = 0;
+  for (int t = 0; t < T; ++t) {
+    if (unsorted[(size_t)t]) return res;
+    n_rows += nrows_part[(size_t)t];
+  }
+  if (n_rows == 0) return res;
+  for (int64_t b = 0; b < nb; ++b) {
+    for (int t = 1; t < T; ++t) hist[0][(size_t)b] += hist[(size_t)t][(size_t)b];
+    total += hist[0][(size_t)b];
+  }
+  std::vector<int32_t> bounds((size_t)std::max(P - 1, 0), 0);
+  {
+    int64_t run = 0, b = 0;
+    for (int s = 0; s < P - 1; ++s) {
+      const int64_t want = (total * (s + 1) + P - 1) / P;
+      while (b < nb && run + hist[0][(size_t)b] <= want) run += hist[0][(size_t)b++];
+      bounds[(size_t)s] = (int32_t)std::min<int64_t>(M, b << shift);
+    }
+  }
+  ts[1] = now();
+  auto slots_of = [&](int64_t d) { return d > thr ? (int32_t)std::min<int64_t>((d + thr - 1) / thr, sh.cap) : 1; };
+  std::vector<int32_t> order((size_t)n_rows);
+  {
+    constexpr int kKeys = 65536;
+    std::vector<int64_t> cnt((size_t)kKeys + 1, 0);
+    auto key = [&](int64_t r) { return (int64_t)kKeys - 1 - std::min<int64_t>((int64_t)rowptr[r + 1] - rowptr[r], kKeys - 1); };
+    for (int64_t w = 0; w < W; ++w) {
+      if (!sparse_window(w)) continue;
+      for (int64_t r = w * HCSPMM_BLK_H; r < std::min<int64_t>((w + 1) * HCSPMM_BLK_H, N); ++r) cnt[(size_t)key(r) + 1]++;
+    }
+    for (int k = 0; k < kKeys; ++k) cnt[(size_t)k + 1] += cnt[(size_t)k];
+    const int64_t n_top = cnt[1];
+    for (int64_t w = 0; w < W; ++w) {
+      if (!sparse_window(w)) continue;
+      for (int64_t r = w * HCSPMM_BLK_H; r < std::min<int64_t>((w + 1) * HCSPMM_BLK_H, N); ++r) order[(size_t)cnt[(size_t)key(r)]++] = (int32_t)r;
+    }
+    std::stable_sort(order.begin(), order.begin() + n_top, [&](int32_t a, int32_t b) {
+      return (int64_t)rowptr[a + 1] - rowptr[a] > (int64_t)rowptr[b + 1] - rowptr[b];
+    });
+  }
+  std::vector<int32_t> wg_of((size_t)n_rows);
+  std::vector<int64_t> wg_first((size_t)G + 1, 0);
+  {
+    typedef std::pair<int64_t, int32_t> Item;
+    std::vector<Item> heap;
+    heap.reserve((size_t)G);
+    for (int g = 0; g < G; ++g) heap.emplace_back(0, g);
+    auto cmp = [](const Item& a, const Item& b) { return a > b; };
+    std::vector<int32_t> used((size_t)G, 0);
+    std::vector<Item> aside;
+    for (int64_t i = 0; i < n_rows; ++i) {
+      const int64_t r = order[(size_t)i], d = (int64_t)rowptr[r + 1] - rowptr[r];
+      const int32_t m = slots_of(d);
+      aside.clear();
+      int32_t g = -1;
+      while (!heap.empty()) {
+        std::pop_heap(heap.begin(), heap.end(), cmp);
+        const Item it = heap.back();
+        heap.pop_back();
+        if (used[(size_t)it.second] + m <= sh.cap) {
+          g = it.second;
+          used[(size_t)g] += m;
+          if (used[(size_t)g] < sh.cap) {
+            heap.emplace_back(it.first + d + 2, g);
+            std::push_heap(heap.begin(), heap.end(), cmp);
+          }
+          break;
+        }
+        aside.push_back(it);
+      }
+      for (const Item& it : aside) {
+        heap.push_back(it);
+        std::push_heap(heap.begin(), heap.end(), cmp);
+      }
+      if (g < 0) return res;
+      wg_of[(size_t)i] = g;
+      wg_first[(size_t)g + 1]++;
+    }
+    for (int g = 0; g < G; ++g) {
+      wg_first[(size_t)g + 1] += wg_first[(size_t)g];
+      res.slots = std::max(res.slots, used[(size_t)g]);
+    }
+  }
+  std::vector<int32_t> wg_rows((size_t)n_rows);
+  {
+    std::vector<int64_t> at(wg_first.begin(), wg_first.end() - 1);
+    for (int64_t i = 0; i < n_rows; ++i) wg_rows[(size_t)at[(size_t)wg_of[(size_t)i]]++] = order[(size_t)i];
+  }
+  ts[2] = now();
+  std::vector<std::vector<int32_t>> buf((size_t)G);
+  std::vector<int32_t> nchunks((size_t)G * 4 * (size_t)P, 0);
+  res.off_table = align4(base);
+  res.off_rowptr = res.off_table + sh.table_words;
+  res.off_rows = res.off_rowptr + sh.rowptr_words;
+  res.off_stream = (res.off_rows + sh.rows_words + 63) & ~int64_t(63);
+  int32_t* rowtab = plan + res.off_rows;
+  parallel_for(T, [&](int t) {
+    struct VRow { int32_t row_i, k, m, slot; };
+    struct Run { int32_t len, slot, first; };
+    std::vector<int32_t> cuts;
+    std::vector<VRow> wave_rows[4];
+    std::vector<Run> runs;
+    std::vector<int> sub_of;
+    for (int g = (int)((int64_t)G * t / T); g < (int)((int64_t)G * (t + 1) / T); ++g) {
+      const int64_t i0 = wg_first[(size_t)g], nr = wg_first[(size_t)g + 1] - i0;
+      if (nr == 0) continue;
+      cuts.resize((size_t)nr * ((size_t)P + 1));
+      for (int w = 0; w < 4; ++w) wave_rows[w].clear();
+      int64_t wave_load[4] = {0, 0, 0, 0};
+      int32_t slot = 0;
+      for (int64_t i = 0; i < nr; ++i) {
+        const int64_t r = wg_rows[(size_t)(i0 + i)], d = (int64_t)rowptr[r + 1] - rowptr[r];
+        slice_cuts(col, rowptr[r], d, bounds.data(), P, cuts.data() + (size_t)i * ((size_t)P + 1));
+        const int32_t m = slots_of(d);
+        rowtab[2 * (i0 + i) + 0] = (int32_t)r;
+        rowtab[2 * (i0 + i) + 1] = slot | (m << 16);
+        for (int32_t k = 0; k < m; ++k) {
+          int w = 0;
+          for (int x = 1; x < 4; ++x) if (wave_load[x] < wave_load[w]) w = x;
+          wave_load[w] += d / m + 2;
+          wave_rows[w].push_back(VRow{(int32_t)i, k, m, slot + k});
+        }
+        slot += m;
+      }
+      std::vector<int32_t>& out = buf[(size_t)g];
+      out.clear();
+      out.reserve((size_t)(wave_load[0] + wave_load[1] + wave_load[2] + wave_load[3]) * 5 / 4 + 64 * 4 * (size_t)P);
+      for (int w = 0; w < 4; ++w) {
+        for (int p = 0; p < P; ++p) {
+          runs.clear();
+          for (const VRow& v : wave_rows[w]) {
+            const int32_t* c = cuts.data() + (size_t)v.row_i * ((size_t)P + 1);
+            const int64_t a = c[p], n = (int64_t)c[p + 1] - a;
+            const int64_t lo = a + n * v.k / v.m, hi = a + n * (v.k + 1) / v.m;
+            if (hi > lo) runs.push_back(Run{(int32_t)(hi - lo), v.slot, (int32_t)(rowptr[wg_rows[(size_t)(i0 + v.row_i)]] + lo)});
+          }
+          if (runs.empty()) continue;
+          std::stable_sort(runs.begin(), runs.end(), [](const Run& a, const Run& b) { return a.len > b.len; });
+          size_t fill[8] = {0, 0, 0, 0, 0, 0, 0, 0};
+          sub_of.resize(runs.size());
+          for (size_t i = 0; i < runs.size(); ++i) {
+            int q = 0;
+            for (int x = 1; x < 8; ++x) if (fill[x] < fill[q]) q = x;
+            sub_of[i] = q;
+            fill[q] += (size_t)runs[i].len;
+          }
+          size_t longest = 0;
+          for (int q = 0; q < 8; ++q) longest = std::max(longest, fill[q]);
+          const size_t nc = (longest + 7) / 8;
+          nchunks[((size_t)g * 4 + (size_t)w) * (size_t)P + (size_t)p] = (int32_t)nc;
+          const size_t o = out.size();
+          out.resize(o + 64 * nc, kStreamPadCol);
+          for (int q = 0; q < 8; ++q) fill[q] = 0;
+          for (size_t i = 0; i < runs.size(); ++i) {
+            const Run& rn = runs[i];
+            const int q = sub_of[i];
+            const uint32_t tag = (uint32_t)rn.slot << kStreamColBits;
+            size_t k = fill[q];
+            for (int32_t j = 0; j < rn.len; ++j, ++k)
+              out[o + (k >> 3) * 64 + (size_t)q * 8 + (k & 7)] =
+                  (int32_t)((uint32_t)col[rn.first + j] | tag | (j == 0 ? 1u << 30 : 0u) | (j == rn.len - 1 ? 1u << 31 : 0u));
+            fill[q] = k;
+          }
+        }
+      }
+    }
+  });
+  ts[3] = now();
+  int32_t* table = plan + res.off_table;
+  int64_t run = 0;
+  for (size_t i = 0; i < nchunks.size(); ++i) {
+    table[i] = (int32_t)run;
+    run += nchunks[i];
+  }
+  if (run > sh.chunk_budget || (!sh.forced && 64 * run > sh.entries * 3 / 2)) return res;
+  table[nchunks.size()] = (int32_t)run;
+  for (int64_t i = (int64_t)nchunks.size() + 1; i < sh.table_words; ++i) table[i] = 0;
+  int32_t* rp_out = plan + res.off_rowptr;
+  for (int64_t g = 0; g < sh.rowptr_words; ++g) rp_out[g] = g <= G ? (int32_t)wg_first[(size_t)g] : 0;
+  for (int64_t i = 2 * n_rows; i < res.off_stream - res.off_rows; ++i) rowtab[i] = 0;
+  for (int64_t i = base; i < res.off_table; ++i) plan[i] = 0;
+  int32_t* sout = plan + res.off_stream;
+  parallel_for(T, [&](int t) {
+    for (int g = (int)((int64_t)G * t / T); g < (int)((int64_t)G * (t + 1) / T); ++g)
+      if (!buf[(size_t)g].empty())
+        std::memcpy(sout + 64 * (int64_t)table[(size_t)g * 4 * (size_t)P], buf[(size_t)g].data(), sizeof(int32_t) * buf[(size_t)g].size());
+  });
+  ts[4] = now();
+  if (dbg)
+    std::fprintf(stderr, "plan_build: stream: sorted? + phase boundaries %.2f | deal %.2f | streams %.2f | copy %.2f ms\n", ts[1] - ts[0],
+                 ts[2] - ts[1], ts[3] - ts[2], ts[4] - ts[3]);
+  res.chunks = run;
+  res.end = res.off_stream + 64 * run;
+  res.built = true;
+  return res;
+}
+
 }
 
 extern "C" int hcspmm_plan_words(const int32_t* rowptr, int64_t N, int64_t E, const int32_t* bp, const int32_t* ht,
@@ -251,6 +531,9 @@
     if (rc != HCSPMM_OK) return rc;
     total = std::max(total, Ls.total);
   }
+  if (rp.stream_mode > 0 || (rp.slice_mode != kSliceOff && stream_auto_candidate(rp, Ls)))
+    total += stream_shape(rp, N, rp.slice_mode != kSliceOff ? Ls.nnz_sparse : L.nnz_sparse, total).extra_words;
+  if (total > INT32_MAX) return HCSPMM_ERANGE;
   *words_out = total;
   return HCSPMM_OK;
 }
@@ -301,7 +584,7 @@
   PoolScope scope(plan_threads((N + HCSPMM_BLK_H - 1) / HCSPMM_BLK_H));
   static const bool dbg = std::getenv("HCSPMM_PLAN_DEBUG") != nullptr;
   auto now = [] { return std::chrono::duration<double, std::milli>(std::chrono::steady_clock::now().time_since_epoch()).count(); };
-  double tp[8] = {now(), 0, 0, 0, 0, 0, 0, 0};
+  double tp[9] = {now(), 0, 0, 0, 0, 0, 0, 0, 0};
   uint64_t fingerprint = 0;
   {
     const int frc = fingerprint_and_check(rowptr, col, N, E, M, &fingerprint);
@@ -594,11 +877,20 @@
     uniq_total += uniq_part[(size_t)t];
   }
 
+  tp[6] = now();
+  StreamResult sr;
+  StreamShape ss;
+  const int32_t stream_thr = slicing ? rp.slice_threshold : rp.split_threshold;
+  if (rp.stream_mode > 0 || (rp.stream_mode == 0 && rp.slice_mode == kSliceAuto && slicing && L.nnz_sparse >= kSliceAutoMinEntries)) {
+    ss = stream_shape(rp, N, L.nnz_sparse, L.total);
+    sr = build_stream(rowptr, col, N, M, ht, ss, stream_thr, plan, L.total, words, T);
+  }
+
   hcspmm_plan_header h;
   std::memset(&h, 0, sizeof(h));
   h.magic = HCSPMM_PLAN_MAGIC;
   h.version = HCSPMM_PLAN_VERSION;
-  h.total_words = (int32_t)L.total;
+  h.total_words = (int32_t)(sr.built ? sr.end : L.total);
   h.num_nodes = (int32_t)N;
   h.num_edges = (int32_t)E;
   h.num_windows = (int32_t)W;
@@ -638,13 +930,24 @@
   h.nnz_sliced = slicing ? (int32_t)L.nnz_sliced : 0;
   h.n_sliced_rows = slicing ? (int32_t)L.n_sliced_rows : 0;
   h.panel_cols = rp.panel_cols;
+  if (sr.built) {
+    h.n_stream_wgs = ss.G;
+    h.stream_phases = ss.P;
+    h.stream_slots = sr.slots;
+    h.stream_threshold = stream_thr;
+    h.off_stream_table = (int32_t)sr.off_table;
+    h.off_stream_rowptr = (int32_t)sr.off_rowptr;
+    h.off_stream_rows = (int32_t)sr.off_rows;
+    h.off_stream = (int32_t)sr.off_stream;
+    h.stream_chunks = (int32_t)sr.chunks;
+  }
   static_assert(sizeof(hcspmm_plan_header) == HCSPMM_PLAN_HEADER_WORDS * 4, "header size");
   std::memcpy(plan, &h, sizeof(h));
   if (dbg) {
-    tp[6] = now();
+    tp[7] = now();
     std::fprintf(stderr, "plan_build: T=%d: fingerprint + range check %.2f | layout %.2f | clear + slice boundaries %.2f | task pass 1 (count) %.2f | "
-                         "task pass 2 (write) %.2f | dense packs %.2f | total %.2f ms\n",
-                 T, tp[1] - tp[0], tp[2] - tp[1], tp[3] - tp[2], tp[4] - tp[3], tp[5] - tp[4], tp[6] - tp[5], tp[6] - tp[0]);
+                         "task pass 2 (write) %.2f | dense packs %.2f | stream %.2f | total %.2f ms\n",
+                 T, tp[1] - tp[0], tp[2] - tp[1], tp[3] - tp[2], tp[4] - tp[3], tp[5] - tp[4], tp[6] - tp[5], tp[7] - tp[6], tp[7] - tp[0]);
   }
   return HCSPMM_OK;
 }
@@ -687,6 +990,22 @@
   } else if (h->n_slice_tasks != 0 || h->slice_xcd_tasks != 0) {
     return HCSPMM_EPLAN;
   }
+  if (h->n_stream_wgs < 0) return HCSPMM_EPLAN;
+  if (h->n_stream_wgs > 0) {
+    const int64_t sections_end = h->n_slices > 0 ? h->off_slice_tasks + 4 * (int64_t)h->n_slice_tasks
+                                                  : h->off_sparse_windows + (int64_t)h->n_sparse_windows;
+    const int64_t entries = (int64_t)h->n_stream_wgs * 4 * h->stream_phases;
+    if (h->stream_phases <= 0 || h->stream_phases > 64 || h->stream_slots <= 0 || h->stream_slots > 256 || h->stream_threshold <= 0 ||
+        h->stream_chunks < 0 || h->num_columns >= (1 << 22))
+      return HCSPMM_EPLAN;
+    if (h->off_stream_table < sections_end || (h->off_stream_table & 3)) return HCSPMM_EPLAN;
+    if (h->off_stream_rowptr < h->off_stream_table + entries + 1 || (h->off_stream_rowptr & 3)) return HCSPMM_EPLAN;
+    if (h->off_stream_rows < h->off_stream_rowptr + (int64_t)h->n_stream_wgs + 1 || (h->off_stream_rows & 3)) return HCSPMM_EPLAN;
+    if (h->off_stream < h->off_stream_rows || (h->off_stream & 63)) return HCSPMM_EPLAN;
+    if (h->total_words < h->off_stream + 64 * (int64_t)h->stream_chunks) return HCSPMM_EPLAN;
+  } else if (h->stream_phases != 0 || h->stream_slots != 0 || h->stream_chunks != 0) {
+    return HCSPMM_EPLAN;
+  }
   if (words_available > 0 && h->total_words > words_available) return HCSPMM_EPLAN;
   if ((int64_t)h->nnz_sparse + h->nnz_dense != E) return HCSPMM_EPLAN;
   return HCSPMM_OK;
diff --git a/hc-spmm_amd/csrc/spmm_impl.h b/hc-spmm_amd/csrc/spmm_impl.h
--- a/hc-spmm_amd/csrc/spmm_impl.h
+++ b/hc-spmm_amd/csrc/spmm_impl.h
@@ -2,6 +2,8 @@
 #include <hip/hip_runtime.h>
 #include <stdint.h>
 #include <stdlib.h>
+
+#include <type_traits>
 
 #include "hcspmm.h"
 #include "spmm_kernels.h"
@@ -862,6 +864,12 @@
     if (dense_wgs > cap) dense_wgs = cap;
   }
   b.fused_dense_wgs = (int)dense_wgs;
+  const bool streamed = a.n_stream_wgs > 0;
+  if (streamed) {
+    if (!(std::is_same<E, F32>::value && VEC == 4) || a.fused) return hipErrorInvalidValue;
+    b.sparse_wgs = 0;
+    b.tiny_kernel_wgs = 0;
+  }
   const long long grid = (long long)b.sparse_wgs + dense_wgs;
   if (grid > 0x7fffffffLL) return hipErrorInvalidValue;
   if (grid > 0) {
@@ -881,6 +889,7 @@
   }
   hipError_t e = hipGetLastError();
   if (e != hipSuccess) return e;
+  if (streamed) return launch_stream_f32(b, stream);
   if (b.tiny_kernel_wgs > 0) {
     hipLaunchKernelGGL((tiny_kernel<E, L, VEC>), dim3((unsigned)(b.tiny_kernel_wgs * n_col_panels)), dim3(kThreads), 0, stream, b);
     e = hipGetLastError();
diff --git a/hc-spmm_amd/csrc/spmm_kernels.h b/hc-spmm_amd/csrc/spmm_kernels.h
--- a/hc-spmm_amd/csrc/spmm_kernels.h
+++ b/hc-spmm_amd/csrc/spmm_kernels.h
@@ -35,6 +35,8 @@
   };
   long long w_ldr, w_ldc;
   float* out;
+  int n_stream_wgs, stream_phases, stream_slots;
+  int off_stream_table, off_stream_rowptr, off_stream_rows, off_stream;
 };
 
 struct TilesArgs {
@@ -69,6 +71,7 @@
 };
 
 hipError_t launch_plan_f32(const PlanArgs& a, int vec, hipStream_t stream);
+hipError_t launch_stream_f32(const PlanArgs& a, hipStream_t stream);
 bool plan_own_tiny_launch(int n_tiny, int fused);
 hipError_t launch_window_f32(const WindowArgs& a, int vec, hipStream_t stream);
 hipError_t launch_plan_f16(const PlanArgs& a, int vec, hipStream_t stream);
diff --git a/hc-spmm_amd/csrc/spmm_stream.hip b/hc-spmm_amd/csrc/spmm_stream.hip
--- /dev/null
+++ b/hc-spmm_amd/csrc/spmm_stream.hip
@@ -0,0 +1,92 @@
+#include <type_traits>
+
+#include "spmm_impl.h"
+
+namespace hcspmm {
+
+constexpr int kStreamL = 8;
+constexpr int kStreamPanel = 32;
+constexpr unsigned kStreamColMask = (1u << 22) - 1u;
+
+#ifndef HCSPMM_STREAM_MIN_WAVES
+#define HCSPMM_STREAM_MIN_WAVES 5
+#endif
+
+__global__ __launch_bounds__(kThreads, HCSPMM_STREAM_MIN_WAVES) void stream_phase_kernel(PlanArgs a) {
+  typedef Lane<F32, 4> Ln;
+  typedef Ln::acc_t acc_t;
+  extern __shared__ __attribute__((aligned(16))) float s_acc[];
+  const float* X = reinterpret_cast<const float*>(a.X);
+  float* Z = reinterpret_cast<float*>(a.Z);
+  const int lane = threadIdx.x & 63;
+  const int wave = __builtin_amdgcn_readfirstlane(threadIdx.x >> 6);
+  const int wg = (int)blockIdx.x;
+  cint_p rowptr = (cint_p)(a.plan + a.off_stream_rowptr);
+  const int r0 = rowptr[wg], nrows = rowptr[wg + 1] - r0;
+  if (nrows == 0) return;
+  cint_p table = (cint_p)(a.plan + a.off_stream_table);
+  const int ch0 = table[(wg * kWaves + wave) * a.stream_phases], ch1 = table[(wg * kWaves + wave + 1) * a.stream_phases];
+  const int* stream = a.plan + a.off_stream;
+  const int* rows = a.plan + a.off_stream_rows + 2 * (size_t)r0;
+  const int s = lane & (kStreamL - 1), gbase = lane & ~(kStreamL - 1);
+  acc_t* mine = reinterpret_cast<acc_t*>(s_acc) + s;
+
+  for (int i = threadIdx.x; i < a.stream_slots * kStreamL; i += kThreads) reinterpret_cast<acc_t*>(s_acc)[i] = azero<4>();
+  __syncthreads();
+  for (int c0 = 0; c0 < a.D; c0 += kStreamPanel) {
+    const int cend = min(a.D, c0 + kStreamPanel);
+    const bool cok = c0 + s * 4 < cend;
+    const int c = cok ? lane_col<4>(c0 + s * 4, cend) : 0;
+    acc_t acc = azero<4>();
+    int next = ch0 < ch1 ? stream[(size_t)ch0 * 64 + lane] : (int)kStreamColMask;
+    for (int ch = ch0; ch < ch1; ++ch) {
+      const unsigned mine_w = (unsigned)next;
+      unsigned w[8];
+      Ln::raw_t v[8];
+#pragma unroll
+      for (int u = 0; u < 8; ++u) w[u] = (unsigned)__shfl((int)mine_w, gbase + u, 64);
+      if (ch + 1 < ch1) next = stream[(size_t)(ch + 1) * 64 + lane];
+#pragma unroll
+      for (int u = 0; u < 8; ++u) {
+        const unsigned col = w[u] & kStreamColMask;
+        v[u] = Ln::load(X + (size_t)(col == kStreamColMask ? 0u : col) * a.ldx + c);
+      }
+#pragma unroll
+      for (int u = 0; u < 8; ++u) {
+        const bool first = (w[u] >> 30) & 1u, last = (w[u] >> 31) != 0u;
+        acc_t* slot = mine + ((w[u] >> 22) & 0xffu) * kStreamL;
+        if (__builtin_amdgcn_ballot_w64(first) != 0ull) {
+          if (first) acc = *slot;
+        }
+        if (!(cok && (w[u] & kStreamColMask) != kStreamColMask)) v[u] = Ln::zero();
+        Ln::add(acc, v[u]);
+        if (__builtin_amdgcn_ballot_w64(last) != 0ull) {
+          if (last) *slot = acc;
+        }
+      }
+    }
+    __syncthreads();
+    for (int i = wave * (64 / kStreamL) + (lane >> 3); i < nrows; i += kWaves * (64 / kStreamL)) {
+      const int row = rows[2 * i], sm = rows[2 * i + 1];
+      acc_t* slot = mine + (sm & 0xffff) * kStreamL;
+      const int m = sm >> 16;
+      acc_t sum = slot[0];
+      slot[0] = azero<4>();
+      for (int k = 1; k < m; ++k) {
+        sum += slot[k * kStreamL];
+        slot[k * kStreamL] = azero<4>();
+      }
+      if (cok) Ln::store(Z + (size_t)row * a.ldz + c, sum);
+    }
+    __syncthreads();
+  }
+}
+
+hipError_t launch_stream_f32(const PlanArgs& a, hipStream_t stream) {
+  if (a.n_stream_wgs <= 0 || a.stream_slots <= 0 || a.stream_slots > 256) return hipErrorInvalidValue;
+  const size_t lds = (size_t)a.stream_slots * kStreamPanel * sizeof(float);
+  hipLaunchKernelGGL(stream_phase_kernel, dim3((unsigned)a.n_stream_wgs), dim3(kThreads), lds, stream, a);
+  return hipGetLastError();
+}
+
+}
diff --git a/hc-spmm_amd/hcspmm/__init__.py b/hc-spmm_amd/hcspmm/__init__.py
--- a/hc-spmm_amd/hcspmm/__init__.py
+++ b/hc-spmm_amd/hcspmm/__init__.py
@@ -226,14 +226,15 @@
 
 def build_plan(row_pointers, column_index, blockPartition, edgeToColumn, hybrid_type, device=None,
                split_threshold=0, segment_len=0, num_columns=None, fuse_in_launch=False, slice_threshold=0, n_slices=0,
-               panel_cols=0):
+               panel_cols=0, stream_mode=0, stream_wgs_per_cu=0):
     L = lib()
     rp_h, col_h = _i32_host(row_pointers), _i32_host(column_index)
     bp_h, e2c_h, ht_h = _i32_host(blockPartition), _i32_host(edgeToColumn), _i32_host(hybrid_type)
     N, E = rp_h.numel() - 1, col_h.numel()
     params = PlanParams(int(split_threshold), int(segment_len), int(fuse_in_launch), int(slice_threshold), int(n_slices),
-                        int(panel_cols)) \
-        if (split_threshold or segment_len or fuse_in_launch or slice_threshold or n_slices or panel_cols) else _PLAN_PARAMS
+                        int(panel_cols), int(stream_mode), int(stream_wgs_per_cu)) \
+        if (split_threshold or segment_len or fuse_in_launch or slice_threshold or n_slices or panel_cols or stream_mode
+            or stream_wgs_per_cu) else _PLAN_PARAMS
     words = ctypes.c_int64(0)
     check(L.hcspmm_plan_words(_ptr(rp_h), N, E, _ptr(bp_h), _ptr(ht_h), ctypes.byref(params), ctypes.byref(words)))
     plan = torch.empty(max(int(words.value), Header.WORDS), dtype=torch.int32)
diff --git a/hc-spmm_amd/hcspmm/capi.py b/hc-spmm_amd/hcspmm/capi.py
--- a/hc-spmm_amd/hcspmm/capi.py
+++ b/hc-spmm_amd/hcspmm/capi.py
@@ -30,7 +30,12 @@
                                                                                   ("off_slice_table", ctypes.c_int32), ("off_slice_tasks", ctypes.c_int32),
                                                                                   ("n_slice_tasks", ctypes.c_int32), ("slice_xcd_tasks", ctypes.c_int32),
                                                                                   ("nnz_sliced", ctypes.c_int32), ("n_sliced_rows", ctypes.c_int32),
-                                                                                  ("panel_cols", ctypes.c_int32), ("reserved", ctypes.c_int32 * 18)]
+                                                                                  ("panel_cols", ctypes.c_int32), ("n_stream_wgs", ctypes.c_int32),
+                                                                                  ("stream_phases", ctypes.c_int32), ("stream_slots", ctypes.c_int32),
+                                                                                  ("stream_threshold", ctypes.c_int32), ("off_stream_table", ctypes.c_int32),
+                                                                                  ("off_stream_rowptr", ctypes.c_int32), ("off_stream_rows", ctypes.c_int32),
+                                                                                  ("off_stream", ctypes.c_int32), ("stream_chunks", ctypes.c_int32),
+                                                                                  ("reserved", ctypes.c_int32 * 9)]
 
     @property
     def fingerprint(self):
@@ -39,7 +44,8 @@
 
 class PlanParams(ctypes.Structure):
     _fields_ = [("split_threshold", ctypes.c_int32), ("segment_len", ctypes.c_int32), ("fuse_in_launch", ctypes.c_int32),
-                ("slice_threshold", ctypes.c_int32), ("n_slices", ctypes.c_int32), ("panel_cols", ctypes.c_int32)]
+                ("slice_threshold", ctypes.c_int32), ("n_slices", ctypes.c_int32), ("panel_cols", ctypes.c_int32),
+                ("stream_mode", ctypes.c_int32), ("stream_wgs_per_cu", ctypes.c_int32)]
 
 
 _vp, _i64, _int, _sz = ctypes.c_void_p, ctypes.c_int64, ctypes.c_int, ctypes.c_size_t
diff --git a/hc-spmm_amd/hybrid_kernel/hybrid_all.cpp b/hc-spmm_amd/hybrid_kernel/hybrid_all.cpp
--- a/hc-spmm_amd/hybrid_kernel/hybrid_all.cpp
+++ b/hc-spmm_amd/hybrid_kernel/hybrid_all.cpp
@@ -18,7 +18,7 @@
   CHECK_CONTIGUOUS(x)
 
 int g_rule = HCSPMM_RULE_MI355X;
-hcspmm_plan_params g_params = {0, 0, 0, 0, 0, 0};
+hcspmm_plan_params g_params = {0, 0, 0, 0, 0, 0, 0, 0};
 
 void check_rc(int rc, const char* what) {
   TORCH_CHECK(rc == HCSPMM_OK, "HCSPMM.", what, ": ", hcspmm_strerror(rc), " [code ", rc, ", hipError_t ",
@@ -889,12 +889,15 @@
 
 torch::Tensor build_plan(torch::Tensor row_pointers, torch::Tensor column_index, torch::Tensor blockPartition,
                          torch::Tensor edgeToColumn, torch::Tensor hybrid_type, int split_threshold, int segment_len,
-                         int64_t num_columns, int fuse_in_launch, int slice_threshold, int n_slices, int panel_cols) {
+                         int64_t num_columns, int fuse_in_launch, int slice_threshold, int n_slices, int panel_cols,
+                         int stream_mode, int stream_wgs_per_cu) {
   auto rp = to_host_i32(row_pointers), col = to_host_i32(column_index), bp = to_host_i32(blockPartition),
        e2c = to_host_i32(edgeToColumn), ht = to_host_i32(hybrid_type);
   const int64_t N = rp.numel() - 1, E = col.numel();
-  hcspmm_plan_params pp = (split_threshold || segment_len || fuse_in_launch || slice_threshold || n_slices || panel_cols)
-                              ? hcspmm_plan_params{split_threshold, segment_len, fuse_in_launch, slice_threshold, n_slices, panel_cols}
+  hcspmm_plan_params pp = (split_threshold || segment_len || fuse_in_launch || slice_threshold || n_slices || panel_cols ||
+                           stream_mode || stream_wgs_per_cu)
+                              ? hcspmm_plan_params{split_threshold, segment_len, fuse_in_launch, slice_threshold, n_slices, panel_cols,
+                                                   stream_mode, stream_wgs_per_cu}
                               : g_params;
   int64_t words = 0;
   check_rc(hcspmm_plan_words(rp.data_ptr<int>(), N, E, iptr(bp), iptr(ht), &pp, &words), "build_plan(plan size)");
@@ -941,7 +944,8 @@
         pybind11::arg("row_pointers"), pybind11::arg("column_index"), pybind11::arg("blockPartition"),
         pybind11::arg("edgeToColumn"), pybind11::arg("hybrid_type"), pybind11::arg("split_threshold") = 0,
         pybind11::arg("segment_len") = 0, pybind11::arg("num_columns") = -1, pybind11::arg("fuse_in_launch") = 0,
-        pybind11::arg("slice_threshold") = 0, pybind11::arg("n_slices") = 0, pybind11::arg("panel_cols") = 0);
+        pybind11::arg("slice_threshold") = 0, pybind11::arg("n_slices") = 0, pybind11::arg("panel_cols") = 0,
+        pybind11::arg("stream_mode") = 0, pybind11::arg("stream_wgs_per_cu") = 0);
   m.def("wide_threshold", [](torch::Tensor row_nzr, int embedding_dim, int dtype) {
     hcspmm_plan_header h;
     bool has = false;
@@ -1218,6 +1222,8 @@
     d["n_dense_compact2"] = h.n_dense_compact2; d["num_columns"] = h.num_columns;
     d["panel_cols"] = h.panel_cols; d["n_slices"] = h.n_slices; d["slice_threshold"] = h.slice_threshold; d["n_slice_tasks"] = h.n_slice_tasks;
     d["nnz_sliced"] = h.nnz_sliced; d["n_sliced_rows"] = h.n_sliced_rows; d["total_words"] = h.total_words;
+    d["n_stream_wgs"] = h.n_stream_wgs; d["stream_phases"] = h.stream_phases; d["stream_slots"] = h.stream_slots;
+    d["stream_threshold"] = h.stream_threshold; d["stream_chunks"] = h.stream_chunks;
     d["n_sparse_windows"] = h.n_sparse_windows; d["dense_k_sum"] = h.dense_k_sum; d["flags"] = h.flags; d["num_nodes"] = h.num_nodes; d["num_edges"] = h.num_edges;
     d["fingerprint"] = ((uint64_t)h.fingerprint_hi << 32) | h.fingerprint_lo;
     return d;
diff --git a/include/hcspmm.h b/include/hcspmm.h
--- a/include/hcspmm.h
+++ b/include/hcspmm.h
@@ -91,7 +91,16 @@
   int32_t nnz_sliced;
   int32_t n_sliced_rows;
   int32_t panel_cols;
-  int32_t reserved[18];
+  int32_t n_stream_wgs;
+  int32_t stream_phases;
+  int32_t stream_slots;
+  int32_t stream_threshold;
+  int32_t off_stream_table;
+  int32_t off_stream_rowptr;
+  int32_t off_stream_rows;
+  int32_t off_stream;
+  int32_t stream_chunks;
+  int32_t reserved[9];
 } hcspmm_plan_header;
 
 #define HCSPMM_PLAN_FUSE_IN_LAUNCH 1
@@ -105,6 +114,8 @@
   int32_t slice_threshold;
   int32_t n_slices;
   int32_t panel_cols;
+  int32_t stream_mode;
+  int32_t stream_wgs_per_cu;
 } hcspmm_plan_params;
 
 int hcspmm_plan_words(const int32_t* row_pointers_h, int64_t num_nodes, int64_t num_edges,
```

Result: slower. 3555 billion (-5.4%).
